# pr0g/ToyMeshPathTracer

Hardware: AMD Instinct MI355X
Metric: MRays/s on sponza.obj 1920x1080 64spp at 1/2/4/8 GPUs; %HBM roofline (higher is better)
Workload: dtype f32

## Files before the change

### include/tmpt.h

```cpp
#ifndef TMPT_H
#define TMPT_H

#include <stdint.h>

#ifdef __cplusplus
extern "C" {
#endif

#define TMPT_ABI_VERSION 9

typedef struct tmpt_scene tmpt_scene;

typedef struct {
    float origin[3], lower_left[3], horizontal[3], vertical[3], u[3], v[3], w[3];
    float lens_radius;
} tmpt_camera;

enum { TMPT_SEED_ROW = 0, TMPT_SEED_PIXEL = 1, TMPT_SEED_SAMPLE = 2 };

enum {
    TMPT_ENGINE_WAVEFRONT = 0,
    TMPT_ENGINE_MEGAKERNEL = 1,
    TMPT_ENGINE_PERSISTENT = 2
};

enum {
    TMPT_FLAG_OUT_DEVICE = 1,
    TMPT_FLAG_COUNT_VISITS = 2,
    TMPT_FLAG_WAIT_STREAM = 4,
    TMPT_FLAG_REQUIRE_RCCL = 8
};

typedef struct {
    int32_t width, height, spp;
    int32_t seed_mode;
    int32_t band_rows;
    int32_t shard, num_shards;
    int32_t engine;
    int32_t flags;
    int32_t spp_begin, spp_count;
    int32_t reserved0;
    uint64_t wait_stream;
    int32_t reserved[2];
} tmpt_render_desc;

typedef struct {
    double render_ms;
    double extend_ms, shadow_ms;
    uint64_t extend_rays, shadow_rays;
    int64_t extend_launches, shadow_launches, iterations;
    uint64_t node_visits, tri_tests;
    uint64_t shadow_node_visits, shadow_tri_tests;
    double build_ms;
    int32_t bvh_nodes, bvh_depth, n_tris, device;
    int32_t bvh4_nodes, bvh4_depth, leaf_max, builder_iters;
    int32_t octree_nodes, octree_leaves;
    int64_t octree_refs;
    double octree_build_ms;
    uint64_t tie_queries, root_misses;
    int32_t row_engine;
    int32_t stream_fallbacks;
    int32_t octree_depth;
    int32_t tie_rule;
    int64_t chain_pixels;
    int64_t redo_samples;
    int64_t redo_late;
    uint64_t crack_queries;
    int32_t octree_flat;
    int32_t redo_launches;
    double redo_ms;
    uint64_t redo_rays;
    int32_t tie_path;
    int32_t reserved_stats;
} tmpt_stats;

typedef struct {
    float    normal[3];
    float    depth;
    float    direct;
    int32_t  tri_id;
    uint32_t hits;
    uint32_t lit;
} tmpt_aov_pixel;

typedef struct {
    int32_t width, height, spp;
    int32_t levels;
    int32_t normal_exp;
    int32_t flags;
    float sigma_depth;
    float sigma_direct;
    uint64_t wait_stream;
    int32_t reserved[4];
} tmpt_denoise_desc;


int tmpt_load_obj(const char* path, float** out_tris, int32_t* out_n, float out_bmin[3],
                  float out_bmax[3]);
void tmpt_free(void* p);

int tmpt_camera_init(tmpt_camera* cam, const float look_from[3], const float look_at[3],
                     const float vup[3], float vfov, float aspect, float aperture,
                     float focus_dist);
int tmpt_camera_for_scene(tmpt_camera* cam, const float bmin[3], const float bmax[3],
                          int32_t width, int32_t height, int32_t is_sponza);


int tmpt_device_count(void);

int tmpt_scene_create(const float* tris, int32_t n, int32_t device, tmpt_scene** out);

int tmpt_scene_create_ex(const float* tris, int32_t n, int32_t device, const char* options, tmpt_scene** out);
int tmpt_scene_set_option(tmpt_scene* scene, const char* key, double value);
int tmpt_scene_get_option(const tmpt_scene* scene, const char* key, double* value);
int tmpt_scene_build_octree(tmpt_scene* scene, const float bmin[3], const float bmax[3]);
int tmpt_octree_bounds(const float bmin[3], const float bmax[3], float box[6]);
int tmpt_octree_digest(const float* tris, int32_t n, const float bmin[3], const float bmax[3], uint64_t out[5]);
int tmpt_octree_flags(const float* tris, int32_t n, const float bmin[3], const float bmax[3], const float* rays,
                      const float* t, const int32_t* ids, int64_t n_rays, uint8_t* flags, float grid[13]);
int tmpt_scene_destroy(tmpt_scene* scene);

int tmpt_scene_hit(const tmpt_scene* scene, const float* rays, int64_t n, float tmin, float tmax,
                   int32_t any_hit, float* hits, int32_t* ids);
int tmpt_scene_hit_ranged(const tmpt_scene* scene, const float* rays8, int64_t n, int32_t any_hit,
                          float* hits, int32_t* ids);

int tmpt_render(tmpt_scene* scene, const tmpt_camera* cam, const tmpt_render_desc* desc,
                uint8_t* rgba_out, uint64_t* ray_count);
int tmpt_render_aov(tmpt_scene* scene, const tmpt_camera* cam, const tmpt_render_desc* desc,
                    tmpt_aov_pixel* out, uint64_t* ray_count);
int tmpt_render_radiance(tmpt_scene* scene, const tmpt_camera* cam, const tmpt_render_desc* desc,
                         float* rgba32f_out, uint8_t* rgba8_out, uint64_t* ray_count);
int tmpt_denoise(tmpt_scene* scene, const tmpt_denoise_desc* desc, const float* rgba32f_in,
                 const tmpt_aov_pixel* aov, float* rgba32f_out, uint8_t* rgba8_out);
int tmpt_render_multi(const float* tris, int32_t n, const float* octree_box ,
                      const tmpt_camera* cam, const tmpt_render_desc* desc, const int32_t* devices,
                      int32_t ndevices, uint8_t* rgba_full, uint64_t* ray_count, double* seconds);

int32_t tmpt_tile_rows(const tmpt_render_desc* desc);
int32_t tmpt_tile_row_to_y(const tmpt_render_desc* desc, int32_t r);

int tmpt_get_stats(const tmpt_scene* scene, tmpt_stats* out);

int tmpt_write_png(const char* path, const uint8_t* rgba, int32_t width, int32_t height);

int tmpt_unit_sincos(int32_t device, uint32_t key0, uint32_t n, float* out);

int tmpt_fastdiv(uint32_t divisor, const uint32_t* x, uint64_t n, uint32_t* out, uint32_t mul_shift[2]);

int tmpt_scene_dump_bvh(const tmpt_scene* scene, int32_t layout, uint32_t* nodes, uint64_t node_words,
                        uint32_t* tris, uint64_t tri_words, int32_t info[8]);
int tmpt_radix_sort(const tmpt_scene* scene, uint32_t* keys, uint32_t* vals, int64_t n, int32_t bits);

const char* tmpt_last_error(void);
int tmpt_abi_version(void);

#ifdef __cplusplus
}
#endif
#endif
```

### toymeshpathtracer_amd/__init__.py

```python
from __future__ import annotations

import ctypes
import os
from dataclasses import dataclass
from typing import Optional, Tuple

import numpy as np

__all__ = [
    "Camera", "Scene", "Hit", "RenderStats", "load_scene", "write_png", "device_count",
    "SEED_ROW", "SEED_PIXEL", "SEED_SAMPLE", "ENGINE_WAVEFRONT", "ENGINE_MEGAKERNEL", "ENGINE_PERSISTENT", "lib_path", "TmptError",
    "tile_rows", "tile_row_to_y", "render_multi", "octree_bounds", "octree_digest", "octree_flags",
    "AOV_DTYPE",
]

SEED_ROW, SEED_PIXEL, SEED_SAMPLE = 0, 1, 2
ENGINE_WAVEFRONT, ENGINE_MEGAKERNEL, ENGINE_PERSISTENT = 0, 1, 2
FLAG_OUT_DEVICE, FLAG_COUNT_VISITS, FLAG_WAIT_STREAM, FLAG_REQUIRE_RCCL = 1, 2, 4, 8

AOV_DTYPE = np.dtype([("normal", np.float32, (3,)), ("depth", np.float32), ("direct", np.float32),
                      ("tri_id", np.int32), ("hits", np.uint32), ("lit", np.uint32)])

_HERE = os.path.dirname(os.path.abspath(__file__))
lib_path = os.environ.get("TMPT_LIB_PATH") or os.path.join(_HERE, "_lib", "libtmpt.so")


class TmptError(RuntimeError):
    pass


if not os.path.exists(lib_path):
    raise ImportError(
        f"libtmpt.so not built ({lib_path}); run `python -c 'import __graft_entry__ as g; g.build()'` "
        "or `make -C toymeshpathtracer_amd/csrc`. There is no CPU fallback.")

try:
    if os.environ.get("TMPT_NO_TORCH") == "1":
        raise ImportError("TMPT_NO_TORCH")
    import torch
except Exception:
    torch = None

_lib = ctypes.CDLL(lib_path)

_f32p = ctypes.POINTER(ctypes.c_float)
_i32p = ctypes.POINTER(ctypes.c_int32)
_u8p = ctypes.POINTER(ctypes.c_uint8)
_u64p = ctypes.POINTER(ctypes.c_uint64)


class _Camera(ctypes.Structure):
    _fields_ = [("origin", ctypes.c_float * 3), ("lower_left", ctypes.c_float * 3),
                ("horizontal", ctypes.c_float * 3), ("vertical", ctypes.c_float * 3),
                ("u", ctypes.c_float * 3), ("v", ctypes.c_float * 3), ("w", ctypes.c_float * 3),
                ("lens_radius", ctypes.c_float)]


class _Desc(ctypes.Structure):
    _fields_ = [("width", ctypes.c_int32), ("height", ctypes.c_int32), ("spp", ctypes.c_int32),
                ("seed_mode", ctypes.c_int32), ("band_rows", ctypes.c_int32),
                ("shard", ctypes.c_int32), ("num_shards", ctypes.c_int32),
                ("engine", ctypes.c_int32), ("flags", ctypes.c_int32),
                ("spp_begin", ctypes.c_int32), ("spp_count", ctypes.c_int32),
                ("reserved0", ctypes.c_int32), ("wait_stream", ctypes.c_uint64),
                ("reserved", ctypes.c_int32 * 2)]


class _DenoiseDesc(ctypes.Structure):
    _fields_ = [("width", ctypes.c_int32), ("height", ctypes.c_int32), ("spp", ctypes.c_int32),
                ("levels", ctypes.c_int32), ("normal_exp", ctypes.c_int32), ("flags", ctypes.c_int32),
                ("sigma_depth", ctypes.c_float), ("sigma_direct", ctypes.c_float),
                ("wait_stream", ctypes.c_uint64), ("reserved", ctypes.c_int32 * 4)]


class _Stats(ctypes.Structure):
    _fields_ = [("render_ms", ctypes.c_double), ("extend_ms", ctypes.c_double),
                ("shadow_ms", ctypes.c_double), ("extend_rays", ctypes.c_uint64),
                ("shadow_rays", ctypes.c_uint64), ("extend_launches", ctypes.c_int64),
                ("shadow_launches", ctypes.c_int64), ("iterations", ctypes.c_int64),
                ("node_visits", ctypes.c_uint64), ("tri_tests", ctypes.c_uint64),
                ("shadow_node_visits", ctypes.c_uint64), ("shadow_tri_tests", ctypes.c_uint64),
                ("build_ms", ctypes.c_double), ("bvh_nodes", ctypes.c_int32),
                ("bvh_depth", ctypes.c_int32), ("n_tris", ctypes.c_int32),
                ("device", ctypes.c_int32), ("bvh4_nodes", ctypes.c_int32),
                ("bvh4_depth", ctypes.c_int32), ("leaf_max", ctypes.c_int32),
                ("builder_iters", ctypes.c_int32), ("octree_nodes", ctypes.c_int32),
                ("octree_leaves", ctypes.c_int32), ("octree_refs", ctypes.c_int64),
                ("octree_build_ms", ctypes.c_double), ("tie_queries", ctypes.c_uint64),
                ("root_misses", ctypes.c_uint64), ("row_engine", ctypes.c_int32),
                ("stream_fallbacks", ctypes.c_int32), ("octree_depth", ctypes.c_int32),
                ("tie_rule", ctypes.c_int32), ("chain_pixels", ctypes.c_int64),
                ("redo_samples", ctypes.c_int64), ("redo_late", ctypes.c_int64),
                ("crack_queries", ctypes.c_uint64), ("octree_flat", ctypes.c_int32),
                ("redo_launches", ctypes.c_int32), ("redo_ms", ctypes.c_double),
                ("redo_rays", ctypes.c_uint64), ("tie_path", ctypes.c_int32), ("reserved_stats", ctypes.c_int32)]


def _sig(name, res, args):
    fn = getattr(_lib, name)
    fn.restype = res
    fn.argtypes = args
    return fn


_load_obj = _sig("tmpt_load_obj", ctypes.c_int, [ctypes.c_char_p, ctypes.POINTER(_f32p), _i32p, _f32p, _f32p])
_free = _sig("tmpt_free", None, [ctypes.c_void_p])
_cam_init = _sig("tmpt_camera_init", ctypes.c_int, [ctypes.POINTER(_Camera), _f32p, _f32p, _f32p,
                                                     ctypes.c_float, ctypes.c_float, ctypes.c_float,
                                                     ctypes.c_float])
_cam_scene = _sig("tmpt_camera_for_scene", ctypes.c_int, [ctypes.POINTER(_Camera), _f32p, _f32p,
                                                          ctypes.c_int32, ctypes.c_int32, ctypes.c_int32])
_dev_count = _sig("tmpt_device_count", ctypes.c_int, [])
_scene_create = _sig("tmpt_scene_create", ctypes.c_int, [_f32p, ctypes.c_int32, ctypes.c_int32,
                                                         ctypes.POINTER(ctypes.c_void_p)])
_scene_create_ex = _sig("tmpt_scene_create_ex", ctypes.c_int, [_f32p, ctypes.c_int32, ctypes.c_int32,
                                                               ctypes.c_char_p, ctypes.POINTER(ctypes.c_void_p)])
_set_option = _sig("tmpt_scene_set_option", ctypes.c_int, [ctypes.c_void_p, ctypes.c_char_p, ctypes.c_double])
_get_option = _sig("tmpt_scene_get_option", ctypes.c_int, [ctypes.c_void_p, ctypes.c_char_p,
                                                           ctypes.POINTER(ctypes.c_double)])
_scene_destroy = _sig("tmpt_scene_destroy", ctypes.c_int, [ctypes.c_void_p])
_scene_hit = _sig("tmpt_scene_hit", ctypes.c_int, [ctypes.c_void_p, _f32p, ctypes.c_int64,
                                                   ctypes.c_float, ctypes.c_float, ctypes.c_int32,
                                                   _f32p, _i32p])
_scene_hit_ranged = _sig("tmpt_scene_hit_ranged", ctypes.c_int, [ctypes.c_void_p, _f32p, ctypes.c_int64,
                                                                 ctypes.c_int32, _f32p, _i32p])
_render = _sig("tmpt_render", ctypes.c_int, [ctypes.c_void_p, ctypes.POINTER(_Camera),
                                             ctypes.POINTER(_Desc), ctypes.c_void_p, _u64p])
_render_aov = _sig("tmpt_render_aov", ctypes.c_int, [ctypes.c_void_p, ctypes.POINTER(_Camera),
                                                     ctypes.POINTER(_Desc), ctypes.c_void_p, _u64p])
_render_radiance = _sig("tmpt_render_radiance", ctypes.c_int, [ctypes.c_void_p, ctypes.POINTER(_Camera),
                                                               ctypes.POINTER(_Desc), ctypes.c_void_p,
                                                               ctypes.c_void_p, _u64p])
_denoise = _sig("tmpt_denoise", ctypes.c_int, [ctypes.c_void_p, ctypes.POINTER(_DenoiseDesc), ctypes.c_void_p,
                                               ctypes.c_void_p, ctypes.c_void_p, ctypes.c_void_p])
_build_octree = _sig("tmpt_scene_build_octree", ctypes.c_int, [ctypes.c_void_p, _f32p, _f32p])
_octree_bounds = _sig("tmpt_octree_bounds", ctypes.c_int, [_f32p, _f32p, _f32p])
_octree_digest = _sig("tmpt_octree_digest", ctypes.c_int, [_f32p, ctypes.c_int32, _f32p, _f32p, _u64p])
_octree_flags = _sig("tmpt_octree_flags", ctypes.c_int, [_f32p, ctypes.c_int32, _f32p, _f32p, _f32p, _f32p, _i32p,
                                                         ctypes.c_int64, ctypes.c_void_p, _f32p])
_render_multi = _sig("tmpt_render_multi", ctypes.c_int,
                     [_f32p, ctypes.c_int32, _f32p, ctypes.POINTER(_Camera), ctypes.POINTER(_Desc),
                      ctypes.POINTER(ctypes.c_int32), ctypes.c_int32, ctypes.c_void_p, _u64p,
                      ctypes.POINTER(ctypes.c_double)])
_tile_rows = _sig("tmpt_tile_rows", ctypes.c_int32, [ctypes.POINTER(_Desc)])
_tile_row_to_y = _sig("tmpt_tile_row_to_y", ctypes.c_int32, [ctypes.POINTER(_Desc), ctypes.c_int32])
_stats = _sig("tmpt_get_stats", ctypes.c_int, [ctypes.c_void_p, ctypes.POINTER(_Stats)])
_write_png = _sig("tmpt_write_png", ctypes.c_int, [ctypes.c_char_p, _u8p, ctypes.c_int32, ctypes.c_int32])
_last_error = _sig("tmpt_last_error", ctypes.c_char_p, [])
_abi = _sig("tmpt_abi_version", ctypes.c_int, [])
_unit_sincos = _sig("tmpt_unit_sincos", ctypes.c_int, [ctypes.c_int32, ctypes.c_uint32, ctypes.c_uint32,
                                                       ctypes.c_void_p])
EXPORTS = ("tmpt_load_obj", "tmpt_free", "tmpt_camera_init", "tmpt_camera_for_scene",
           "tmpt_device_count", "tmpt_scene_create", "tmpt_scene_create_ex", "tmpt_scene_set_option",
           "tmpt_scene_get_option", "tmpt_scene_destroy", "tmpt_scene_hit", "tmpt_scene_hit_ranged",
           "tmpt_render", "tmpt_render_multi", "tmpt_tile_rows", "tmpt_tile_row_to_y", "tmpt_get_stats",
           "tmpt_write_png", "tmpt_last_error", "tmpt_abi_version", "tmpt_unit_sincos",
           "tmpt_scene_build_octree", "tmpt_octree_bounds", "tmpt_octree_digest",
           "tmpt_octree_flags", "tmpt_render_aov", "tmpt_render_radiance", "tmpt_denoise", "tmpt_fastdiv",
           "tmpt_scene_dump_bvh", "tmpt_radix_sort")


def _check(rc: int, what: str) -> None:
    if rc != 0:
        raise TmptError(f"{what} failed ({rc}): {_last_error().decode(errors='replace')}")


def _fp(a: np.ndarray):
    return a.ctypes.data_as(_f32p)


def unit_sincos(key0: int, n: int, device: int = 0) -> np.ndarray:
    out = np.empty((n, 2), dtype=np.float32)
    _check(_unit_sincos(device, key0, n, out.ctypes.data), "tmpt_unit_sincos")
    return out


def fastdiv(divisor: int, x: np.ndarray):
    fn = _sig("tmpt_fastdiv", ctypes.c_int, [ctypes.c_uint32, ctypes.c_void_p, ctypes.c_uint64, ctypes.c_void_p,
                                             ctypes.c_void_p])
    x = np.ascontiguousarray(x, dtype=np.uint32)
    out = np.empty_like(x)
    ms = np.zeros(2, dtype=np.uint32)
    _check(fn(divisor, x.ctypes.data, x.size, out.ctypes.data, ms.ctypes.data), "tmpt_fastdiv")
    return out, (int(ms[0]), int(ms[1]))


def device_count() -> int:
    return int(_dev_count())


def abi_version() -> int:
    return int(_abi())


def load_scene(path: str) -> Tuple[np.ndarray, np.ndarray, np.ndarray]:
    p = _f32p()
    n = ctypes.c_int32()
    bmin = np.zeros(3, np.float32)
    bmax = np.zeros(3, np.float32)
    _check(_load_obj(path.encode(), ctypes.byref(p), ctypes.byref(n), _fp(bmin), _fp(bmax)),
           f"load_scene({path!r})")
    try:
        tris = np.ctypeslib.as_array(p, shape=(n.value * 9,)).copy().reshape(n.value, 3, 3)
    finally:
        _free(p)
    return tris, bmin, bmax


def octree_bounds(bmin, bmax) -> Tuple[np.ndarray, np.ndarray]:
    lo, hi = np.asarray(bmin, np.float32), np.asarray(bmax, np.float32)
    box = np.zeros(6, np.float32)
    _check(_octree_bounds(_fp(lo), _fp(hi), _fp(box)), "octree_bounds")
    return box[:3].copy(), box[3:].copy()


def octree_digest(tris: np.ndarray, box_min, box_max) -> dict:
    t = np.ascontiguousarray(np.asarray(tris, np.float32).reshape(-1, 9))
    lo, hi = np.asarray(box_min, np.float32), np.asarray(box_max, np.float32)
    out = (ctypes.c_uint64 * 5)()
    _check(_octree_digest(_fp(t), t.shape[0], _fp(lo), _fp(hi), out), "octree_digest")
    return dict(zip(("nodes", "leaves", "refs", "depth", "digest"), (int(v) for v in out)))


def octree_flags(tris: np.ndarray, box_min, box_max, rays, t, ids):
    tr = np.ascontiguousarray(np.asarray(tris, np.float32).reshape(-1, 9))
    lo, hi = np.asarray(box_min, np.float32), np.asarray(box_max, np.float32)
    r = np.ascontiguousarray(np.asarray(rays, np.float32)[:, :6])
    tt = np.ascontiguousarray(np.asarray(t, np.float32))
    ii = np.ascontiguousarray(np.asarray(ids, np.int32))
    out = np.zeros(r.shape[0], np.uint8)
    grid = np.zeros(13, np.float32)
    _check(_octree_flags(_fp(tr), tr.shape[0], _fp(lo), _fp(hi), _fp(r), _fp(tt), ii.ctypes.data_as(_i32p),
                         r.shape[0], out.ctypes.data, _fp(grid)), "octree_flags")
    return out, grid


@dataclass
class Camera:
    origin: np.ndarray
    lower_left: np.ndarray
    horizontal: np.ndarray
    vertical: np.ndarray
    u: np.ndarray
    v: np.ndarray
    w: np.ndarray
    lens_radius: float

    @staticmethod
    def _from_c(c: _Camera) -> "Camera":
        a = lambda f: np.array(list(f), np.float32)
        return Camera(a(c.origin), a(c.lower_left), a(c.horizontal), a(c.vertical), a(c.u),
                      a(c.v), a(c.w), float(c.lens_radius))

    def _to_c(self) -> _Camera:
        c = _Camera()
        for name in ("origin", "lower_left", "horizontal", "vertical", "u", "v", "w"):
            getattr(c, name)[:] = [float(x) for x in np.asarray(getattr(self, name), np.float32)]
        c.lens_radius = self.lens_radius
        return c

    @staticmethod
    def create(look_from, look_at, vup, vfov: float, aspect: float, aperture: float,
               focus_dist: float) -> "Camera":
        c = _Camera()
        lf, la, up = (np.asarray(x, np.float32) for x in (look_from, look_at, vup))
        _check(_cam_init(ctypes.byref(c), _fp(lf), _fp(la), _fp(up), vfov, aspect, aperture,
                         focus_dist), "Camera")
        return Camera._from_c(c)

    @staticmethod
    def for_scene(bmin, bmax, width: int, height: int, is_sponza: bool = False) -> "Camera":
        c = _Camera()
        lo, hi = np.asarray(bmin, np.float32), np.asarray(bmax, np.float32)
        _check(_cam_scene(ctypes.byref(c), _fp(lo), _fp(hi), width, height, int(is_sponza)),
               "Camera.for_scene")
        return Camera._from_c(c)

    def as_array(self) -> np.ndarray:
        return np.concatenate([self.origin, self.lower_left, self.horizontal, self.vertical,
                               self.u, self.v, self.w, [self.lens_radius]]).astype(np.float32)


@dataclass
class Hit:
    pos: np.ndarray
    normal: np.ndarray
    t: float


@dataclass
class RenderStats:
    render_ms: float
    extend_ms: float
    shadow_ms: float
    extend_rays: int
    shadow_rays: int
    extend_launches: int
    shadow_launches: int
    iterations: int
    node_visits: int
    tri_tests: int
    shadow_node_visits: int
    shadow_tri_tests: int
    build_ms: float
    bvh_nodes: int
    bvh_depth: int
    n_tris: int
    device: int
    bvh4_nodes: int
    bvh4_depth: int
    leaf_max: int
    builder_iters: int
# ... 96 lines not shown
    def __exit__(self, *exc):
        self.close()

    def hit_scene_batch(self, rays: np.ndarray, t_min: Optional[float] = None, t_max: Optional[float] = None,
                        any_hit: bool = False) -> Tuple[np.ndarray, np.ndarray]:
        rays = np.asarray(rays, np.float32)
        if (t_min is None) != (t_max is None):
            raise ValueError("hit_scene_batch: give both t_min and t_max, or neither (ranged rays [n,8])")
        ranged = t_min is None and t_max is None
        rays = np.ascontiguousarray(rays.reshape(-1, 8 if ranged else 6))
        n = rays.shape[0]
        hits = np.zeros((n, 7), np.float32)
        ids = np.full(n, -1, np.int32)
        if ranged:
            _check(_scene_hit_ranged(self._h, _fp(rays), n, int(any_hit), _fp(hits), ids.ctypes.data_as(_i32p)),
                   "hit_scene")
        else:
            _check(_scene_hit(self._h, _fp(rays), n, t_min, t_max, int(any_hit), _fp(hits),
                              ids.ctypes.data_as(_i32p)), "hit_scene")
        return ids, hits

    def hit_scene(self, orig, direction, t_min: float, t_max: float) -> Tuple[int, Optional[Hit]]:
        ids, hits = self.hit_scene_batch(np.concatenate([orig, direction])[None], t_min, t_max)
        if ids[0] < 0:
            return -1, None
        h = hits[0]
        return 1, Hit(h[0:3].copy(), h[3:6].copy(), float(h[6]))

    def trace_image(self, camera: Camera, width: int, height: int, spp: int,
                    seed_mode: int = SEED_ROW, engine: int = ENGINE_PERSISTENT, band_rows: int = 0,
                    shard: int = 0, num_shards: int = 1, count_visits: bool = False,
                    out=None, spp_begin: int = 0, spp_count: int = 0,
                    wait_stream="current") -> Tuple[np.ndarray, int]:
        if out is None:
            ws = None
        elif isinstance(wait_stream, str):
            ws = _current_stream(self.device)
        else:
            ws = wait_stream
        d = _desc(width, height, spp, seed_mode, band_rows, shard, num_shards, engine,
                  (FLAG_COUNT_VISITS if count_visits else 0) | (FLAG_OUT_DEVICE if out is not None else 0),
                  spp_begin, spp_count, ws)
        rows = int(_tile_rows(ctypes.byref(d)))
        rays = ctypes.c_uint64()
        cam = camera._to_c()
        if out is not None:
            _check(_render(self._h, ctypes.byref(cam), ctypes.byref(d), ctypes.c_void_p(int(out)),
                           ctypes.byref(rays)), "trace_image")
            return None, int(rays.value)
        img = np.zeros((rows, width, 4), np.uint8)
        _check(_render(self._h, ctypes.byref(cam), ctypes.byref(d), img.ctypes.data_as(ctypes.c_void_p),
                       ctypes.byref(rays)), "trace_image")
        return img, int(rays.value)

    def trace_progressive(self, camera: Camera, width: int, height: int, spp: int, passes,
                          band_rows: int = 0, shard: int = 0, num_shards: int = 1, seed_mode: int = SEED_PIXEL):
        if isinstance(passes, int):
            passes = [min(passes, spp - b) for b in range(0, spp, passes)]
        if sum(passes) != spp or min(passes) < 1:
            raise ValueError("passes must be positive and sum to spp")
        done = 0
        for n in passes:
            img, rays = self.trace_image(camera, width, height, spp, seed_mode=seed_mode,
                                         engine=ENGINE_PERSISTENT, band_rows=band_rows, shard=shard,
                                         num_shards=num_shards, spp_begin=done, spp_count=n)
            done += n
            yield done, img, rays

    def trace_aov(self, camera: Camera, width: int, height: int, spp: int, band_rows: int = 0,
                  shard: int = 0, num_shards: int = 1, out=None, wait_stream="current"):
        if out is None:
            ws = None
        elif isinstance(wait_stream, str):
            ws = _current_stream(self.device)
        else:
            ws = wait_stream
        d = _desc(width, height, spp, SEED_SAMPLE, band_rows, shard, num_shards, ENGINE_PERSISTENT,
                  FLAG_OUT_DEVICE if out is not None else 0, 0, 0, ws)
        rows = int(_tile_rows(ctypes.byref(d)))
        rays = ctypes.c_uint64()
        cam = camera._to_c()
        if out is not None:
            _check(_render_aov(self._h, ctypes.byref(cam), ctypes.byref(d), ctypes.c_void_p(int(out)),
                               ctypes.byref(rays)), "trace_aov")
            return None, int(rays.value)
        rec = np.zeros((rows, width), AOV_DTYPE)
        _check(_render_aov(self._h, ctypes.byref(cam), ctypes.byref(d), rec.ctypes.data_as(ctypes.c_void_p),
                           ctypes.byref(rays)), "trace_aov")
        return rec, int(rays.value)

    def trace_radiance(self, camera: Camera, width: int, height: int, spp: int, seed_mode: int = SEED_SAMPLE,
                       band_rows: int = 0, shard: int = 0, num_shards: int = 1, out=None, wait_stream="current"):
        if out is None:
            ws = None
        elif isinstance(wait_stream, str):
            ws = _current_stream(self.device)
        else:
            ws = wait_stream
        d = _desc(width, height, spp, seed_mode, band_rows, shard, num_shards, ENGINE_PERSISTENT,
                  FLAG_OUT_DEVICE if out is not None else 0, 0, 0, ws)
        rows = int(_tile_rows(ctypes.byref(d)))
        rays = ctypes.c_uint64()
        cam = camera._to_c()
        if out is not None:
            f32, u8 = out if isinstance(out, (tuple, list)) else (out, None)
            _check(_render_radiance(self._h, ctypes.byref(cam), ctypes.byref(d), ctypes.c_void_p(int(f32)),
                                    None if u8 is None else ctypes.c_void_p(int(u8)), ctypes.byref(rays)),
                   "trace_radiance")
            return None, None, int(rays.value)
        rad = np.zeros((rows, width, 4), np.float32)
        img = np.zeros((rows, width, 4), np.uint8)
        _check(_render_radiance(self._h, ctypes.byref(cam), ctypes.byref(d), rad.ctypes.data_as(ctypes.c_void_p),
                                img.ctypes.data_as(ctypes.c_void_p), ctypes.byref(rays)), "trace_radiance")
        return rad, img, int(rays.value)

    def denoise(self, radiance, aov, spp: int, levels: int = 0, normal_exp: int = -1, sigma_depth: float = 0.0,
                sigma_direct: float = 0.0, out=None, width: Optional[int] = None, height: Optional[int] = None,
                wait_stream="current"):
        dev = isinstance(radiance, int)
        d = _DenoiseDesc()
        if dev:
            if width is None or height is None or out is None:
                raise ValueError("denoise: device pointers need width, height and out")
            h, w = int(height), int(width)
        else:
            radiance = np.ascontiguousarray(radiance, np.float32)
            aov = np.ascontiguousarray(aov, AOV_DTYPE)
            h, w = radiance.shape[:2]
            if radiance.shape != (h, w, 4) or aov.shape != (h, w):
                raise ValueError("denoise: radiance [h, w, 4] and aov [h, w] of one whole frame")
        d.width, d.height, d.spp, d.levels, d.normal_exp = w, h, spp, levels, normal_exp
        d.sigma_depth, d.sigma_direct = sigma_depth, sigma_direct
        if dev:
            d.flags = FLAG_OUT_DEVICE
            ws = _current_stream(self.device) if isinstance(wait_stream, str) else wait_stream
            if ws is not None:
                d.flags |= FLAG_WAIT_STREAM
                d.wait_stream = int(ws)
            f32, u8 = out
            _check(_denoise(self._h, ctypes.byref(d), ctypes.c_void_p(radiance), ctypes.c_void_p(int(aov)),
                            None if f32 is None else ctypes.c_void_p(int(f32)),
                            None if u8 is None else ctypes.c_void_p(int(u8))), "denoise")
            return None, None
        res = np.zeros((h, w, 4), np.float32) if out is None else out
        if not (isinstance(res, np.ndarray) and res.dtype == np.float32 and res.shape == (h, w, 4)
                and res.flags.c_contiguous):
            raise ValueError("denoise: out must be a contiguous float32 array [h, w, 4] (it may be radiance itself)")
        img = np.zeros((h, w, 4), np.uint8)
        _check(_denoise(self._h, ctypes.byref(d), radiance.ctypes.data_as(ctypes.c_void_p),
                        aov.ctypes.data_as(ctypes.c_void_p), res.ctypes.data_as(ctypes.c_void_p),
                        img.ctypes.data_as(ctypes.c_void_p)), "denoise")
        return res, img

    def dump_bvh(self, layout: str = "aos") -> dict:
        if layout not in ("aos", "soa"):
            raise ValueError("dump_bvh: layout is 'aos' or 'soa'")
        fn = _sig("tmpt_scene_dump_bvh", ctypes.c_int, [ctypes.c_void_p, ctypes.c_int32, ctypes.c_void_p,
                                                        ctypes.c_uint64, ctypes.c_void_p, ctypes.c_uint64, _i32p])
        info = np.zeros(8, np.int32)
        lay = int(layout == "soa")
        _check(fn(self._h, lay, None, 0, None, 0, info.ctypes.data_as(_i32p)), "dump_bvh")
        nodes = np.zeros((int(info[1]), 16), np.uint32)
        tris = np.zeros((int(info[0]) + 1, 12), np.uint32)
        _check(fn(self._h, lay, nodes.ctypes.data, nodes.size, tris.ctypes.data, tris.size,
                  info.ctypes.data_as(_i32p)), "dump_bvh")
        keys = ("n", "n_nodes4", "depth4", "leaf_max", "count_shift", "link_bits", "builder_iters", "soa")
        return {"nodes": nodes, "tris": tris, "info": dict(zip(keys, (int(v) for v in info)))}

    def radix_sort(self, keys, vals, bits: int = 32):
        fn = _sig("tmpt_radix_sort", ctypes.c_int, [ctypes.c_void_p, ctypes.c_void_p, ctypes.c_void_p,
                                                    ctypes.c_int64, ctypes.c_int32])
        k = np.array(keys, dtype=np.uint32).reshape(-1)
        v = np.array(vals, dtype=np.uint32).reshape(-1)
        if k.shape != v.shape:
            raise ValueError("radix_sort: keys and vals of one length")
        _check(fn(self._h, k.ctypes.data, v.ctypes.data, k.size, bits), "radix_sort")
        return k, v

    def stats(self) -> RenderStats:
        s = _Stats()
        _check(_stats(self._h, ctypes.byref(s)), "stats")
        return RenderStats(*[getattr(s, f) for f, _ in _Stats._fields_ if not f.startswith("reserved")])


def render_multi(tris: np.ndarray, camera: "Camera", width: int, height: int, spp: int, devices,
                 seed_mode: int = SEED_PIXEL, engine: int = ENGINE_PERSISTENT,
                 require_rccl: bool = False, bounds=None) -> Tuple[np.ndarray, int, float]:
    t = np.ascontiguousarray(np.asarray(tris, np.float32).reshape(-1, 9))
    devs = (ctypes.c_int32 * len(devices))(*devices)
    img = np.zeros((height, width, 4), np.uint8)
    rays = ctypes.c_uint64()
    secs = ctypes.c_double()
    d = _desc(width, height, spp, seed_mode, 0, 0, 1, engine, FLAG_REQUIRE_RCCL if require_rccl else 0)
    cam = camera._to_c()
    box = None if bounds is None else np.concatenate(octree_bounds(*bounds)).astype(np.float32)
    _check(_render_multi(t.ctypes.data_as(_f32p), t.shape[0], None if box is None else _fp(box),
                         ctypes.byref(cam), ctypes.byref(d), devs,
                         len(devices), img.ctypes.data_as(ctypes.c_void_p), ctypes.byref(rays),
                         ctypes.byref(secs)), "render_multi")
    return img, int(rays.value), float(secs.value)


def write_png(path: str, rgba: np.ndarray) -> None:
    rgba = np.ascontiguousarray(rgba, np.uint8)
    h, w = rgba.shape[:2]
    _check(_write_png(path.encode(), rgba.ctypes.data_as(_u8p), w, h), "write_png")
```

### toymeshpathtracer_amd/csrc/tmpt_api.cpp

```cpp
#include <dlfcn.h>
#include <hip/hip_runtime.h>
#include <rccl/rccl.h>
#include <string.h>

#include <algorithm>
#include <new>
#include <chrono>
#include <string>
#include <thread>
#include <vector>

#include "tmpt.h"
#include "tmpt_internal.h"
#include "tmpt_traverse.h"
#include "tmpt_render.h"

namespace tmpt {

static thread_local std::string g_last_error;
void set_error(const std::string& msg) { g_last_error = msg; }
const char* last_error() { return g_last_error.c_str(); }

int load_obj(const char* path, std::vector<float>& tris, f3& bmin, f3& bmax);
void camera_init(tmpt_camera* cam, f3 lookFrom, f3 lookAt, f3 vup, float vfov, float aspect,
                 float aperture, float focusDist);
void camera_for_scene(tmpt_camera* cam, f3 sceneMin, f3 sceneMax, int w, int h, bool sponza);
int write_png(const char* path, const uint8_t* rgba, int w, int h);
int render(Scene& s, const tmpt_camera* cam, const tmpt_render_desc* d, uint32_t* d_out,
           uint64_t* ray_count, float4* d_sums = nullptr);
int intersect_batch(Scene& s, const float* d_rays, int64_t n, float tmin, float tmax, bool any, bool ranged,
                    float* d_hits, int32_t* d_ids);

__global__ void k_unit_sincos(uint32_t key0, uint32_t n, float2* out)
{
    const uint32_t i = blockIdx.x * blockDim.x + threadIdx.x;
    if (i >= n) return;
    float c, s;
    glibc_sincosf_unit(unit_angle((key0 + i) & 0xFFFFFFu), c, s);
    out[i] = make_float2(c, s);
}

__global__ void k_assemble_rows(const uint32_t* __restrict__ gathered, int32_t nd, int32_t max_rows, int32_t W,
                                int32_t H, uint32_t* __restrict__ frame)
{
    const int64_t i = (int64_t)blockIdx.x * 256 + threadIdx.x;
    if (i >= (int64_t)W * H) return;
    const int32_t y = (int32_t)(i / W), x = (int32_t)(i - (int64_t)y * W);
    frame[i] = gathered[((int64_t)(y % nd) * max_rows + y / nd) * W + x];
}

struct Rccl {
    ncclResult_t (*comm_init_all)(ncclComm_t*, int, const int*) = nullptr;
    ncclResult_t (*comm_destroy)(ncclComm_t) = nullptr;
    ncclResult_t (*gather)(const void*, void*, size_t, ncclDataType_t, int, ncclComm_t, hipStream_t) = nullptr;
    ncclResult_t (*reduce)(const void*, void*, size_t, ncclDataType_t, ncclRedOp_t, int, ncclComm_t,
                           hipStream_t) = nullptr;
    ncclResult_t (*group_start)() = nullptr;
    ncclResult_t (*group_end)() = nullptr;
    const char* (*error_string)(ncclResult_t) = nullptr;
    bool ok = false;
};

const Rccl& rccl()
{
    static Rccl r = []() {
        Rccl x;
        void* h = dlopen("librccl.so.1", RTLD_NOW | RTLD_GLOBAL);
        if (!h) h = dlopen("/opt/rocm/lib/librccl.so.1", RTLD_NOW | RTLD_GLOBAL);
        if (!h) return x;
        x.comm_init_all = (decltype(x.comm_init_all))dlsym(h, "ncclCommInitAll");
        x.comm_destroy = (decltype(x.comm_destroy))dlsym(h, "ncclCommDestroy");
        x.gather = (decltype(x.gather))dlsym(h, "ncclGather");
        x.reduce = (decltype(x.reduce))dlsym(h, "ncclReduce");
        x.group_start = (decltype(x.group_start))dlsym(h, "ncclGroupStart");
        x.group_end = (decltype(x.group_end))dlsym(h, "ncclGroupEnd");
        x.error_string = (decltype(x.error_string))dlsym(h, "ncclGetErrorString");
        x.ok = x.comm_init_all && x.comm_destroy && x.gather && x.reduce && x.group_start && x.group_end &&
               x.error_string;
        return x;
    }();
    return r;
}

namespace {
struct OptionDef {
    const char* name;
    bool build;
    double lo, hi;
    int Options::*i;
    float Options::*f;
    double Options::*d;
};
const OptionDef kOptions[] = {
    {"builder", true, 0, 1, &Options::builder, nullptr, nullptr},
    {"layout", true, 0, 1, &Options::layout, nullptr, nullptr},
    {"leaf_max", true, 1, kLeafMaxTris, &Options::leaf_max, nullptr, nullptr},
    {"collapse", true, 0, 1, &Options::collapse, nullptr, nullptr},
    {"ploc_radius", true, 1, 256, &Options::ploc_radius, nullptr, nullptr},
    {"sah_c_leaf", true, 0, 1e6, nullptr, &Options::sah_c_leaf, nullptr},
    {"sah_c_tri", true, 0, 1e6, nullptr, &Options::sah_c_tri, nullptr},
    {"sample_block", false, 0, 1024, &Options::sample_block, nullptr, nullptr},
    {"sample_tail", false, -1, 64, &Options::sample_tail, nullptr, nullptr},
    {"sbuf_max", false, 0, 1e18, nullptr, nullptr, &Options::sbuf_max},
    {"sbuf_pair", false, 0, 1, &Options::sbuf_pair, nullptr, nullptr},
    {"pilot", false, -1, 512, &Options::pilot, nullptr, nullptr},
    {"help", false, -1, 1, &Options::help, nullptr, nullptr},
    {"pair", false, -1, 63, &Options::pair, nullptr, nullptr},
    {"balance", false, 0, 1, &Options::balance, nullptr, nullptr},
    {"dprio", false, 0, 1, &Options::dprio, nullptr, nullptr},
    {"wave_cap", false, 0, 64, &Options::wave_cap, nullptr, nullptr},
    {"pixel_chains", false, -1, 1024, &Options::pixel_chains, nullptr, nullptr},
    {"tie_defer", false, -1, 1, &Options::tie_defer, nullptr, nullptr},
    {"redo_cap", false, 0, 1 << 30, &Options::redo_cap, nullptr, nullptr},
    {"redo_inline", false, 0, 1, &Options::redo_inline, nullptr, nullptr},
    {"redo_lanes", false, 1, 64, &Options::redo_lanes, nullptr, nullptr},
    {"path_waves", false, 0, 5, &Options::path_waves, nullptr, nullptr},
    {"top_walk", false, -1, 8, &Options::top_walk, nullptr, nullptr},
    {"shadow_order", false, -1, 2, &Options::shadow_order, nullptr, nullptr},
    {"pop_cull", false, -1, 1, &Options::pop_cull, nullptr, nullptr},
    {"pop_key_cap", false, -1, kPopKeyMax, &Options::pop_key_cap, nullptr, nullptr},
    {"rowspec", false, 0, 1, &Options::rowspec, nullptr, nullptr},
    {"rowspec_wmax", false, 0, 16384, &Options::rowspec_wmax, nullptr, nullptr},
    {"rowspec_windows", false, 0, 32, &Options::rowspec_windows, nullptr, nullptr},
    {"rowspec_spread", false, -1, 100, nullptr, &Options::rowspec_spread, nullptr},
    {"rowspec_groups", false, 1, kRowSpecMaxGroups, &Options::rowspec_groups, nullptr, nullptr},
    {"rowspec_noshadow", false, 0, 1, &Options::rowspec_noshadow, nullptr, nullptr},
    {"rowspec_chase", false, 0, 1, &Options::rowspec_chase, nullptr, nullptr},
    {"rowspec_stream", false, 0, 1, &Options::rowspec_stream, nullptr, nullptr},
    {"rowstream_dynamic", false, 0, 1, &Options::rowstream_dynamic, nullptr, nullptr},
    {"row_flag_leaves", false, 0, 1, &Options::row_flag_leaves, nullptr, nullptr},
    {"row_occ", false, 0, 5, &Options::row_occ, nullptr, nullptr},
    {"wf_bins", false, 1, 8, &Options::wf_bins, nullptr, nullptr},
    {"rowstream_test_abort", false, 0, 1, &Options::rowstream_test_abort, nullptr, nullptr},
    {"tie_rule", false, 0, 1, &Options::tie_rule, nullptr, nullptr},
    {"aov_group", false, 0, 16, &Options::aov_group, nullptr, nullptr},
    {"denoise_lds", false, -1, 1, &Options::denoise_lds, nullptr, nullptr},
};

const OptionDef* find_option(const char* key)
{
    for (const OptionDef& d : kOptions)
        if (strcmp(d.name, key) == 0) return &d;
    return nullptr;
}
}

int options_set(Options& o, const char* key, double v, bool allow_build)
{
    const OptionDef* d = key ? find_option(key) : nullptr;
    if (!d) {
        set_error(std::string("unknown option '") + (key ? key : "(null)") + "'");
        return -22;
    }
    if (d->build && !allow_build) {
        set_error(std::string("option '") + key + "' is a build option: give it to tmpt_scene_create_ex");
        return -22;
    }
    if (!(v >= d->lo && v <= d->hi)) {
        set_error(std::string("option '") + key + "' out of range [" + std::to_string(d->lo) + ", " +
                  std::to_string(d->hi) + "]");
        return -22;
    }
    if (d->i) {
        if (v != (double)(long long)v) {
            set_error(std::string("option '") + key + "' takes an integer");
            return -22;
        }
        if ((strcmp(key, "row_occ") == 0 || strcmp(key, "path_waves") == 0) && v != 0 && v != 4 && v != 5) {
            set_error(std::string("option '") + key + "' takes 0 (auto), 4 or 5");
            return -22;
        }
        if (strcmp(key, "aov_group") == 0 && v > 0 && ((long long)v & ((long long)v - 1)) != 0) {
            set_error(std::string("option '") + key + "' out of range: 0 (auto), 1, 2, 4, 8 or 16");
            return -22;
        }
        if ((strcmp(key, "sample_block") == 0 || strcmp(key, "wf_bins") == 0) && v > 0 &&
            ((long long)v & ((long long)v - 1)) != 0) {
            set_error(std::string("option '") + key + "' must be a power of two");
            return -22;
        }
        o.*(d->i) = (int)v;
    } else if (d->f) {
        o.*(d->f) = (float)v;
    } else {
        o.*(d->d) = v;
    }
    return 0;
}

int options_get(const Options& o, const char* key, double* v)
{
    const OptionDef* d = key ? find_option(key) : nullptr;
    if (!d) {
        set_error(std::string("unknown option '") + (key ? key : "(null)") + "'");
        return -22;
    }
    *v = d->i ? (double)(o.*(d->i)) : d->f ? (double)(o.*(d->f)) : o.*(d->d);
    return 0;
}

int options_parse(Options& o, const char* text, bool allow_build)
{
    if (!text) return 0;
    std::string t(text);
    size_t pos = 0;
    while (pos <= t.size()) {
        size_t end = t.find(',', pos);
        if (end == std::string::npos) end = t.size();
        std::string item = t.substr(pos, end - pos);
        pos = end + 1;
        item.erase(0, item.find_first_not_of(" \t"));
        item.erase(item.find_last_not_of(" \t") + 1);
        if (item.empty()) continue;
        const size_t eq = item.find('=');
        if (eq == std::string::npos) {
            set_error("option '" + item + "' has no value (key=value)");
            return -22;
        }
        std::string key = item.substr(0, eq), val = item.substr(eq + 1);
        key.erase(key.find_last_not_of(" \t") + 1);
        val.erase(0, val.find_first_not_of(" \t"));
        if (key == "builder" && (val == "ploc" || val == "lbvh")) val = val == "lbvh" ? "1" : "0";
        if (key == "collapse" && (val == "greedy" || val == "sah")) val = val == "sah" ? "1" : "0";
        if (key == "tie_rule" && (val == "visit" || val == "index")) val = val == "index" ? "1" : "0";
        if (key == "layout" && (val == "aos" || val == "soa")) val = val == "soa" ? "1" : "0";
        char* endp = nullptr;
        const double v = strtod(val.c_str(), &endp);
        if (val.empty() || !endp || *endp != '\0') {
            set_error("option '" + key + "': bad value '" + val + "'");
            return -22;
        }
        if (int rc = options_set(o, key.c_str(), v, allow_build)) return rc;
    }
    return 0;
}

}

struct tmpt_scene {
    tmpt::Scene s;
};

using namespace tmpt;

#define TMPT_GUARD_BEGIN try {
#define TMPT_GUARD_END                                  \
    }                                                   \
    catch (const std::bad_alloc&) {                     \
        set_error("out of host memory");                \
        return -1;                                      \
    }                                                   \
    catch (...) {                                       \
        set_error("unexpected C++ exception");          \
        return -1;                                      \
    }

namespace {
// ... 17 lines not shown
    if (n == 0) return 0;
    if (device < 0) {
        for (uint32_t i = 0; i < n; ++i)
            glibc_sincosf_unit(unit_angle((key0 + i) & 0xFFFFFFu), out[2 * (size_t)i], out[2 * (size_t)i + 1]);
        return 0;
    }
    int ndev = 0;
    TMPT_HIP(hipGetDeviceCount(&ndev));
    if (device >= ndev) return bad("tmpt_unit_sincos: no such device");
    TMPT_HIP(hipSetDevice(device));
    float2* d = nullptr;
    TMPT_HIP(hipMalloc(&d, sizeof(float2) * (size_t)n));
    k_unit_sincos<<<(n + 255u) / 256u, 256>>>(key0, n, d);
    hipError_t e = hipGetLastError();
    if (e == hipSuccess) e = hipMemcpy(out, d, sizeof(float2) * (size_t)n, hipMemcpyDeviceToHost);
    (void)hipFree(d);
    if (e != hipSuccess) {
        set_error(std::string("tmpt_unit_sincos: ") + hipGetErrorString(e));
        return -1;
    }
    return 0;
    TMPT_GUARD_END
}

int tmpt_fastdiv(uint32_t divisor, const uint32_t* x, uint64_t n, uint32_t* out, uint32_t mul_shift[2])
{
    TMPT_GUARD_BEGIN
    if (divisor == 0u || divisor >= (1u << 31)) return bad("tmpt_fastdiv: divisor out of range (1 .. 2^31 - 1)");
    if ((!x || !out) && n) return bad("tmpt_fastdiv: null argument");
    const FastDiv f = fastdiv_make(divisor);
    if (mul_shift) {
        mul_shift[0] = f.mul;
        mul_shift[1] = f.shift;
    }
    for (uint64_t i = 0; i < n; ++i) {
        if (x[i] >= (1u << 31)) return bad("tmpt_fastdiv: dividend out of range (below 2^31)");
        out[i] = fastdiv(x[i], f);
    }
    return 0;
    TMPT_GUARD_END
}

int tmpt_load_obj(const char* path, float** out_tris, int32_t* out_n, float out_bmin[3],
                  float out_bmax[3])
{
    TMPT_GUARD_BEGIN
    if (!path || !out_tris || !out_n) return bad("tmpt_load_obj: null argument");
    std::vector<float> tris;
    f3 bmin, bmax;
    int rc = load_obj(path, tris, bmin, bmax);
    if (rc) return rc;
    float* p = (float*)malloc(tris.size() * sizeof(float));
    if (!p) return bad("tmpt_load_obj: out of memory");
    memcpy(p, tris.data(), tris.size() * sizeof(float));
    *out_tris = p;
    *out_n = (int32_t)(tris.size() / 9);
    if (out_bmin) { out_bmin[0] = bmin.x; out_bmin[1] = bmin.y; out_bmin[2] = bmin.z; }
    if (out_bmax) { out_bmax[0] = bmax.x; out_bmax[1] = bmax.y; out_bmax[2] = bmax.z; }
    return 0;
    TMPT_GUARD_END
}

int tmpt_camera_init(tmpt_camera* cam, const float lf[3], const float la[3], const float up[3],
                     float vfov, float aspect, float aperture, float focus_dist)
{
    if (!cam || !lf || !la || !up) return bad("tmpt_camera_init: null argument");
    camera_init(cam, mk(lf[0], lf[1], lf[2]), mk(la[0], la[1], la[2]), mk(up[0], up[1], up[2]),
                vfov, aspect, aperture, focus_dist);
    return 0;
}

int tmpt_camera_for_scene(tmpt_camera* cam, const float bmin[3], const float bmax[3],
                          int32_t width, int32_t height, int32_t is_sponza)
{
    if (!cam || !bmin || !bmax) return bad("tmpt_camera_for_scene: null argument");
    if (width < 1 || height < 1) return bad("tmpt_camera_for_scene: bad size");
    camera_for_scene(cam, mk(bmin[0], bmin[1], bmin[2]), mk(bmax[0], bmax[1], bmax[2]), width,
                     height, is_sponza != 0);
    return 0;
}

int tmpt_device_count(void)
{
    int n = 0;
    if (hipGetDeviceCount(&n) != hipSuccess) return 0;
    return n;
}

int tmpt_scene_create(const float* tris, int32_t n, int32_t device, tmpt_scene** out)
{
    return tmpt_scene_create_ex(tris, n, device, nullptr, out);
}

int tmpt_scene_create_ex(const float* tris, int32_t n, int32_t device, const char* options, tmpt_scene** out)
{
    TMPT_GUARD_BEGIN
    if (!out || n < 0 || (n > 0 && !tris)) return bad("tmpt_scene_create: bad arguments");
    *out = nullptr;
    (void)hipGetLastError();
    Options opt;
    if (int rc = options_parse(opt, options, true)) {
        set_error(std::string("tmpt_scene_create: ") + last_error());
        return rc;
    }
    int ndev = 0;
    TMPT_HIP(hipGetDeviceCount(&ndev));
    if (device < 0 || device >= ndev) return bad("tmpt_scene_create: no such device");
    TMPT_HIP(hipSetDevice(device));
    tmpt_scene* h = new tmpt_scene();
    Scene& s = h->s;
    s.opt = opt;
    s.device = device;
    s.n = n;
    auto fail = [&](int rc) {
        tmpt_scene_destroy(h);
        return rc;
    };
    if (hipStreamCreateWithFlags(&s.stream, hipStreamNonBlocking) != hipSuccess)
        return fail((set_error("hipStreamCreate failed"), -1));
    float* d_tris = nullptr;
    if (n > 0) {
        if (hipMalloc(&d_tris, sizeof(float) * 9 * (size_t)n) != hipSuccess)
            return fail((set_error("tmpt_scene_create: out of device memory"), -1));
        if (hipMemcpy(d_tris, tris, sizeof(float) * 9 * (size_t)n, hipMemcpyHostToDevice) != hipSuccess) {
            (void)hipFree(d_tris);
            return fail((set_error("tmpt_scene_create: upload failed"), -1));
        }
    }
    s.tris_host.assign(tris, tris + 9 * (size_t)n);
    int rc = build_lbvh(s, d_tris);
    if (d_tris) (void)hipFree(d_tris);
    if (rc) return fail(rc);
    *out = h;
    return 0;
    TMPT_GUARD_END
}

int tmpt_scene_destroy(tmpt_scene* h)
{
    if (!h) return 0;
    Scene& s = h->s;
    (void)hipSetDevice(s.device);
    if (s.stream) (void)hipStreamSynchronize(s.stream);
    for (auto& st : s.rs_stream)
        if (st) (void)hipStreamSynchronize(st);
    if (s.nodes4) (void)hipFree(s.nodes4);
    if (s.oct) (void)hipFree(s.oct);
    if (s.oct_refs) (void)hipFree(s.oct_refs);
    if (s.oct_view) (void)hipFree(s.oct_view);
    if (s.soa_buf) (void)hipFree(s.soa_buf);
    if (s.prog) (void)hipFree(s.prog);
    if (s.jt) (void)hipFree(s.jt);
    if (s.sbuf) (void)hipFree(s.sbuf);
    if (s.redo) (void)hipFree(s.redo);
    if (s.redo_state) (void)hipFree(s.redo_state);
    if (s.jt2) (void)hipFree(s.jt2);
    if (s.rs_buf) (void)hipFree(s.rs_buf);
    for (auto& st : s.rs_stream)
        if (st) (void)hipStreamDestroy(st);
    for (auto& ev : s.rs_event)
        if (ev) (void)hipEventDestroy(ev);
    if (s.rs_host) (void)hipHostFree(s.rs_host);
    if (s.rs_list) (void)hipFree(s.rs_list);
    if (s.rss_buf) (void)hipFree(s.rss_buf);
    if (s.rss_tab) (void)hipFree(s.rss_tab);
    if (s.rss_host) (void)hipHostFree(s.rss_host);
    if (s.wait_ev) (void)hipEventDestroy(s.wait_ev);
    if (s.counters) (void)hipFree(s.counters);
    if (s.chk) (void)hipFree(s.chk);
    if (s.counters_host) (void)hipHostFree(s.counters_host);
    for (auto e : s.render_ev)
        if (e) (void)hipEventDestroy(e);
    if (s.tri_pre) (void)hipFree(s.tri_pre);
    if (s.tri_orig) (void)hipFree(s.tri_orig);
    if (s.ws) (void)hipFree(s.ws);
    for (auto e : s.path_ev)
        if (e) (void)hipEventDestroy(e);
    if (s.stream) (void)hipStreamDestroy(s.stream);
    delete h;
    return 0;
}

int tmpt_scene_build_octree(tmpt_scene* h, const float bmin[3], const float bmax[3])
{
    TMPT_GUARD_BEGIN
    if (!h || !bmin || !bmax) return bad("tmpt_scene_build_octree: null argument");
    Scene& s = h->s;
    if ((int64_t)s.tris_host.size() != 9 * (int64_t)s.n) return bad("tmpt_scene_build_octree: no triangle copy");
    TMPT_HIP(hipSetDevice(s.device));
    const auto t0 = std::chrono::steady_clock::now();
    OctreeHost t;
    build_octree(s.tris_host.data(), s.n, bmin, bmax, t);
    if (t.refs.size() >= (size_t)INT32_MAX || t.nodes.size() >= (size_t)INT32_MAX)
        return bad("tmpt_scene_build_octree: octree too large");
    OctNode* d_nodes = nullptr;
    int32_t* d_refs = nullptr;
    const size_t nb = t.nodes.size() * sizeof(OctNode), rb = std::max<size_t>(1, t.refs.size()) * sizeof(int32_t);
    if (hipMalloc(&d_nodes, nb) != hipSuccess || hipMalloc(&d_refs, rb) != hipSuccess ||
        hipMemcpy(d_nodes, t.nodes.data(), nb, hipMemcpyHostToDevice) != hipSuccess ||
        (t.refs.size() && hipMemcpy(d_refs, t.refs.data(), t.refs.size() * sizeof(int32_t), hipMemcpyHostToDevice) !=
                              hipSuccess)) {
        if (d_nodes) (void)hipFree(d_nodes);
        if (d_refs) (void)hipFree(d_refs);
        return (set_error("tmpt_scene_build_octree: out of device memory"), -1);
    }
    if (ensure_counters(s)) {
        (void)hipFree(d_nodes);
        (void)hipFree(d_refs);
        return -1;
    }
    if (s.stream) (void)hipStreamSynchronize(s.stream);
    if (!s.oct_view && hipMalloc(&s.oct_view, sizeof(OctView)) != hipSuccess) {
        (void)hipFree(d_nodes);
        (void)hipFree(d_refs);
        return (set_error("tmpt_scene_build_octree: out of device memory"), -1);
    }
    OctGrid grid;
    octree_grid(t, bmin, bmax, grid);
    std::vector<uint8_t> flat;
    const int32_t n_flat = octree_flat_triangles(s.tris_host.data(), s.n, grid, flat);
    if (mark_flat_triangles(s, flat)) {
        (void)hipFree(d_nodes);
        (void)hipFree(d_refs);
        return -1;
    }
    const OctView ov{d_nodes, d_refs, (int32_t)t.nodes.size(), n_flat, s.ties, grid, (int64_t)t.refs.size()};
    if (hipMemcpy(s.oct_view, &ov, sizeof(ov), hipMemcpyHostToDevice) != hipSuccess) {
        (void)hipFree(d_nodes);
        (void)hipFree(d_refs);
        std::vector<uint8_t> old_flat((size_t)s.n, 0);
        if (s.oct) (void)octree_flat_triangles(s.tris_host.data(), s.n, s.oct_grid, old_flat);
        (void)mark_flat_triangles(s, old_flat);
        return (set_error("tmpt_scene_build_octree: upload failed"), -1);
    }
    if (s.oct) (void)hipFree(s.oct);
    if (s.oct_refs) (void)hipFree(s.oct_refs);
    s.oct = d_nodes;
    s.oct_refs = d_refs;
    s.n_oct = (int32_t)t.nodes.size();
    s.n_oct_refs = (int64_t)t.refs.size();
    s.oct_leaves = t.leaves;
    s.oct_depth = t.depth;
    s.oct_flat = n_flat;
    s.oct_grid = grid;
    for (int c = 0; c < 3; ++c) {
        s.oct_lo[c] = bmin[c];
        s.oct_hi[c] = bmax[c];
    }
    s.oct_build_ms = std::chrono::duration<double, std::milli>(std::chrono::steady_clock::now() - t0).count();
    return 0;
    TMPT_GUARD_END
}

int tmpt_octree_bounds(const float bmin[3], const float bmax[3], float box[6])
{
    if (!bmin || !bmax || !box) return bad("tmpt_octree_bounds: null argument");
    const f3 lo = mk(bmin[0], bmin[1], bmin[2]), hi = mk(bmax[0], bmax[1], bmax[2]);
    const f3 extra = (hi - lo) * 0.7f;
    const f3 a = lo - extra, b = hi + extra;
    box[0] = a.x, box[1] = a.y, box[2] = a.z, box[3] = b.x, box[4] = b.y, box[5] = b.z;
    return 0;
}

int tmpt_octree_digest(const float* tris, int32_t n, const float bmin[3], const float bmax[3], uint64_t out[5])
{
    TMPT_GUARD_BEGIN
    if (n < 0 || (n > 0 && !tris) || !bmin || !bmax || !out) return bad("tmpt_octree_digest: bad arguments");
    OctreeHost t;
    build_octree(tris, n, bmin, bmax, t);
    out[0] = t.nodes.size();
    out[1] = (uint64_t)t.leaves;
    out[2] = t.refs.size() - (uint64_t)t.leaves;
    out[3] = (uint64_t)t.depth;
    out[4] = octree_digest(t);
    return 0;
    TMPT_GUARD_END
}

int tmpt_octree_flags(const float* tris, int32_t n, const float bmin[3], const float bmax[3], const float* rays,
                      const float* t, const int32_t* ids, int64_t n_rays, uint8_t* flags, float grid[13])
{
    TMPT_GUARD_BEGIN
    if (n < 0 || (n > 0 && !tris) || !bmin || !bmax || n_rays < 0 || (n_rays > 0 && (!rays || !t || !ids || !flags)))
        return bad("tmpt_octree_flags: bad arguments");
    OctreeHost oh;
    build_octree(tris, n, bmin, bmax, oh);
    OctGrid g;
    octree_grid(oh, bmin, bmax, g);
    std::vector<uint8_t> flat;
    octree_flat_triangles(tris, n, g, flat);
    for (int64_t i = 0; i < n_rays; ++i) {
        const float* r = rays + 6 * i;
        const int32_t id = ids[i];
        uint8_t f = 0;
        if (id >= 0 && id < n)
            f = (uint8_t)(flat[(size_t)id] | (octree_crack(g, mk(r[0], r[1], r[2]), mk(r[3], r[4], r[5]), t[i]) ? 2 : 0));
        flags[i] = f;
    }
    if (grid) {
        for (int k = 0; k < 3; ++k) {
            grid[k] = g.r0[k];
            grid[3 + k] = g.inv_cell[k];
            grid[6 + k] = g.cell[k];
            grid[9 + k] = g.band[k];
        }
        grid[12] = g.reach;
    }
    return 0;
    TMPT_GUARD_END
}

int tmpt_scene_set_option(tmpt_scene* h, const char* key, double value)
{
    TMPT_GUARD_BEGIN
    if (!h) return bad("tmpt_scene_set_option: null scene");
    return options_set(h->s.opt, key, value, false);
    TMPT_GUARD_END
}

int tmpt_scene_get_option(const tmpt_scene* h, const char* key, double* value)
{
    TMPT_GUARD_BEGIN
    if (!h || !value) return bad("tmpt_scene_get_option: null argument");
    if (key && strcmp(key, "pop_key_bits") == 0) {
        *value = (double)pop_key_bits(h->s.link_bits, h->s.opt.pop_key_cap);
        return 0;
    }
    return options_get(h->s.opt, key, value);
    TMPT_GUARD_END
}

namespace {
int scene_hit(const tmpt_scene* hc, const float* rays, int64_t n, float tmin, float tmax, bool ranged,
              int32_t any_hit, float* hits, int32_t* ids)
{
    if (!hc || n < 0 || (n > 0 && (!rays || !hits || !ids))) return bad("tmpt_scene_hit: bad arguments");
    if (n == 0) return 0;
    const size_t rs = ranged ? 32 : 24;
    Scene& s = const_cast<tmpt_scene*>(hc)->s;
    TMPT_HIP(hipSetDevice(s.device));
    float *d_rays = nullptr, *d_hits = nullptr;
    int32_t* d_ids = nullptr;
    auto cleanup = [&]() {
        if (d_rays) (void)hipFree(d_rays);
        if (d_hits) (void)hipFree(d_hits);
        if (d_ids) (void)hipFree(d_ids);
    };
    if (hipMalloc(&d_rays, rs * (size_t)n) != hipSuccess || hipMalloc(&d_hits, 28 * (size_t)n) != hipSuccess ||
        hipMalloc(&d_ids, 4 * (size_t)n) != hipSuccess) {
        cleanup();
        return bad("tmpt_scene_hit: out of device memory");
    }
    int rc = 0;
    if (hipMemcpy(d_rays, rays, rs * (size_t)n, hipMemcpyHostToDevice) != hipSuccess ||
        hipMemcpy(d_hits, hits, 28 * (size_t)n, hipMemcpyHostToDevice) != hipSuccess)
        rc = (set_error("tmpt_scene_hit: upload failed"), -1);
    if (!rc) rc = intersect_batch(s, d_rays, n, tmin, tmax, any_hit != 0, ranged, d_hits, d_ids);
    if (!rc && (hipStreamSynchronize(s.stream) != hipSuccess ||
                hipMemcpy(hits, d_hits, 28 * (size_t)n, hipMemcpyDeviceToHost) != hipSuccess ||
                hipMemcpy(ids, d_ids, 4 * (size_t)n, hipMemcpyDeviceToHost) != hipSuccess))
        rc = (set_error("tmpt_scene_hit: kernel or readback failed"), -1);
    if (!rc) {
        s.tie_queries = s.counters_host[kTieCounter];
        s.root_misses = s.counters_host[kTieCounter + 1];
        s.crack_queries = s.counters_host[kCrackCounter];
    }
    if (!rc) rc = check_report(s, "tmpt_scene_hit");
    cleanup();
    return rc;
}
}

int tmpt_scene_hit(const tmpt_scene* hc, const float* rays, int64_t n, float tmin, float tmax,
                   int32_t any_hit, float* hits, int32_t* ids)
{
    TMPT_GUARD_BEGIN
    return scene_hit(hc, rays, n, tmin, tmax, false, any_hit, hits, ids);
    TMPT_GUARD_END
}

int tmpt_scene_hit_ranged(const tmpt_scene* hc, const float* rays8, int64_t n, int32_t any_hit, float* hits,
                          int32_t* ids)
{
    TMPT_GUARD_BEGIN
    return scene_hit(hc, rays8, n, 0.0f, 0.0f, true, any_hit, hits, ids);
    TMPT_GUARD_END
}

int32_t tmpt_tile_rows(const tmpt_render_desc* d)
{
    if (!d || d->height < 1) return 0;
    int band = d->band_rows > 0 ? d->band_rows : d->height;
    int ns = d->num_shards > 1 ? d->num_shards : 1;
    int sh = ns > 1 ? d->shard : 0;
    int nbands = (d->height + band - 1) / band;
    int rows = 0;
    for (int b = sh; b < nbands; b += ns) rows += std::min(band, d->height - b * band);
    return rows;
}

int32_t tmpt_tile_row_to_y(const tmpt_render_desc* d, int32_t r)
{
    int band = d->band_rows > 0 ? d->band_rows : d->height;
    int ns = d->num_shards > 1 ? d->num_shards : 1;
    int sh = ns > 1 ? d->shard : 0;
    int lb = r / band;
    return (lb * ns + sh) * band + (r - lb * band);
}

int tmpt_render(tmpt_scene* h, const tmpt_camera* cam, const tmpt_render_desc* d,
                uint8_t* rgba_out, uint64_t* ray_count)
{
    TMPT_GUARD_BEGIN
    if (!h || !cam || !d || !rgba_out) return bad("tmpt_render: null argument");
    if (d->width < 1 || d->width > 10000) return bad("tmpt_render: invalid width");
    if (d->height < 1 || d->height > 10000) return bad("tmpt_render: invalid height");
    if (d->spp < 1 || d->spp > 1024) return bad("tmpt_render: invalid samplesPerPixel");
    if (d->seed_mode != TMPT_SEED_ROW && d->seed_mode != TMPT_SEED_PIXEL && d->seed_mode != TMPT_SEED_SAMPLE)
        return bad("tmpt_render: invalid seed_mode");
    if (d->engine != TMPT_ENGINE_WAVEFRONT && d->engine != TMPT_ENGINE_MEGAKERNEL &&
        d->engine != TMPT_ENGINE_PERSISTENT)
        return bad("tmpt_render: invalid engine");
    if (d->num_shards > 1 && (d->shard < 0 || d->shard >= d->num_shards))
        return bad("tmpt_render: invalid shard");
    if (d->spp_begin < 0 || d->spp_begin >= d->spp || d->spp_count < 0 ||
        d->spp_count > d->spp - d->spp_begin)
        return bad("tmpt_render: invalid spp_begin / spp_count");
    const bool progressive = d->spp_begin > 0 || (d->spp_count > 0 && d->spp_count < d->spp);
    if (progressive && (d->engine != TMPT_ENGINE_PERSISTENT || d->seed_mode == TMPT_SEED_ROW))
        return bad("tmpt_render: progressive spp needs the persistent engine and pixel or sample seeding");
    (void)hipGetLastError();
    Scene& s = h->s;
    TMPT_HIP(hipSetDevice(s.device));
    const int32_t rows = tmpt_tile_rows(d);
    const size_t bytes = (size_t)rows * (size_t)d->width * 4;
    const bool dev_out = (d->flags & TMPT_FLAG_OUT_DEVICE) != 0;
    uint32_t* d_out = nullptr;
    if (dev_out) d_out = (uint32_t*)rgba_out;
    else if (bytes && hipMalloc(&d_out, bytes) != hipSuccess) return bad("tmpt_render: out of device memory");
    int rc = render(s, cam, d, d_out, ray_count);
    if (!rc) rc = check_report(s, "tmpt_render");
    if (!rc && !dev_out && bytes) {
        if (hipMemcpy(rgba_out, d_out, bytes, hipMemcpyDeviceToHost) != hipSuccess)
            rc = (set_error("tmpt_render: readback failed"), -1);
    }
    if (!dev_out && d_out) (void)hipFree(d_out);
    return rc;
    TMPT_GUARD_END
}

int tmpt_render_aov(tmpt_scene* h, const tmpt_camera* cam, const tmpt_render_desc* d, tmpt_aov_pixel* out,
                    uint64_t* ray_count)
{
    TMPT_GUARD_BEGIN
    if (!h || !cam || !d || !out) return bad("tmpt_render_aov: null argument");
    if (d->width < 1 || d->width > 10000) return bad("tmpt_render_aov: invalid width");
    if (d->height < 1 || d->height > 10000) return bad("tmpt_render_aov: invalid height");
    if (d->spp < 1 || d->spp > 1024) return bad("tmpt_render_aov: invalid samplesPerPixel");
    if (d->seed_mode != TMPT_SEED_SAMPLE)
        return bad("tmpt_render_aov: seed_mode must be TMPT_SEED_SAMPLE (the only seeding where a camera ray is a "
                   "function of pixel and sample)");
    if (d->spp_begin != 0 || d->spp_count != 0)
        return bad("tmpt_render_aov: spp_begin / spp_count must be 0 (the pass is not progressive)");
    if (d->flags & TMPT_FLAG_COUNT_VISITS) return bad("tmpt_render_aov: TMPT_FLAG_COUNT_VISITS is not supported");
    if (d->num_shards > 1 && (d->shard < 0 || d->shard >= d->num_shards))
        return bad("tmpt_render_aov: invalid shard");
    const bool dev_out = (d->flags & TMPT_FLAG_OUT_DEVICE) != 0;
    if (dev_out && (reinterpret_cast<uintptr_t>(out) & 15u) != 0)
        return bad("tmpt_render_aov: a device output must be 16-byte aligned");
    (void)hipGetLastError();
    Scene& s = h->s;
    TMPT_HIP(hipSetDevice(s.device));
    const size_t bytes = (size_t)tmpt_tile_rows(d) * (size_t)d->width * sizeof(tmpt_aov_pixel);
    tmpt_aov_pixel* d_out = nullptr;
    if (dev_out) d_out = out;
    else if (bytes && hipMalloc(&d_out, bytes) != hipSuccess) return bad("tmpt_render_aov: out of device memory");
    int rc = render_aov(s, cam, d, d_out, ray_count);
    if (!rc) rc = check_report(s, "tmpt_render_aov");
    if (!rc && !dev_out && bytes) {
        if (hipMemcpy(out, d_out, bytes, hipMemcpyDeviceToHost) != hipSuccess)
            rc = (set_error("tmpt_render_aov: readback failed"), -1);
    }
    if (!dev_out && d_out) (void)hipFree(d_out);
    return rc;
    TMPT_GUARD_END
}

int tmpt_render_radiance(tmpt_scene* h, const tmpt_camera* cam, const tmpt_render_desc* d, float* rgba32f_out,
                         uint8_t* rgba8_out, uint64_t* ray_count)
{
    TMPT_GUARD_BEGIN
    if (!h || !cam || !d || !rgba32f_out) return bad("tmpt_render_radiance: null argument");
    if (d->width < 1 || d->width > 10000) return bad("tmpt_render_radiance: invalid width");
    if (d->height < 1 || d->height > 10000) return bad("tmpt_render_radiance: invalid height");
    if (d->spp < 1 || d->spp > 1024) return bad("tmpt_render_radiance: invalid samplesPerPixel");
    if (d->seed_mode != TMPT_SEED_PIXEL && d->seed_mode != TMPT_SEED_SAMPLE)
        return bad("tmpt_render_radiance: seed_mode must be TMPT_SEED_PIXEL or TMPT_SEED_SAMPLE (row seeding keeps no "
                   "float sum per pixel)");
    if (d->engine != TMPT_ENGINE_PERSISTENT)
        return bad("tmpt_render_radiance: engine must be TMPT_ENGINE_PERSISTENT");
    if (d->spp_begin != 0 || d->spp_count != 0)
        return bad("tmpt_render_radiance: spp_begin / spp_count must be 0 (whole renders only)");
    if (d->flags & TMPT_FLAG_COUNT_VISITS)
        return bad("tmpt_render_radiance: TMPT_FLAG_COUNT_VISITS is not supported");
    if (d->num_shards > 1 && (d->shard < 0 || d->shard >= d->num_shards))
        return bad("tmpt_render_radiance: invalid shard");
    const bool dev_out = (d->flags & TMPT_FLAG_OUT_DEVICE) != 0;
    if (dev_out && (reinterpret_cast<uintptr_t>(rgba32f_out) & 15u) != 0)
        return bad("tmpt_render_radiance: a device rgba32f_out must be 16-byte aligned");
    (void)hipGetLastError();
    Scene& s = h->s;
    TMPT_HIP(hipSetDevice(s.device));
    const size_t px = (size_t)tmpt_tile_rows(d) * (size_t)d->width;
    float4* d_f = dev_out ? reinterpret_cast<float4*>(rgba32f_out) : nullptr;
    uint32_t* d_8 = dev_out ? reinterpret_cast<uint32_t*>(rgba8_out) : nullptr;
    void *own_f = nullptr, *own_8 = nullptr;
    auto cleanup = [&]() {
        if (own_f) (void)hipFree(own_f);
        if (own_8) (void)hipFree(own_8);
    };
    if (px && ((!d_f && hipMalloc(&own_f, px * sizeof(float4)) != hipSuccess) ||
               (!d_8 && hipMalloc(&own_8, px * 4) != hipSuccess))) {
        cleanup();
        return bad("tmpt_render_radiance: out of device memory");
    }
    if (own_f) d_f = static_cast<float4*>(own_f);
    if (own_8) d_8 = static_cast<uint32_t*>(own_8);
    int rc = render(s, cam, d, d_8, ray_count, d_f);
    if (!rc) rc = check_report(s, "tmpt_render_radiance");
    if (!rc && !dev_out && px) {
        if (hipMemcpy(rgba32f_out, d_f, px * sizeof(float4), hipMemcpyDeviceToHost) != hipSuccess ||
            (rgba8_out && hipMemcpy(rgba8_out, d_8, px * 4, hipMemcpyDeviceToHost) != hipSuccess))
            rc = (set_error("tmpt_render_radiance: readback failed"), -1);
    }
    cleanup();
    return rc;
    TMPT_GUARD_END
}

int tmpt_denoise(tmpt_scene* h, const tmpt_denoise_desc* d, const float* rgba32f_in, const tmpt_aov_pixel* aov,
                 float* rgba32f_out, uint8_t* rgba8_out)
{
    TMPT_GUARD_BEGIN
    if (!d) return bad("tmpt_denoise: null descriptor");
    if (d->width < 1 || d->width > 10000) return bad("tmpt_denoise: invalid width");
    if (d->height < 1 || d->height > 10000) return bad("tmpt_denoise: invalid height");
    if (d->spp < 1 || d->spp > 1024) return bad("tmpt_denoise: invalid samplesPerPixel");
    if (d->levels < 0 || d->levels > 6) return bad("tmpt_denoise: levels out of range (1..6, 0 = 5)");
    if (d->normal_exp < -1 || d->normal_exp > 8) return bad("tmpt_denoise: normal_exp out of range (0..8, -1 = 5)");
    if (!(d->sigma_depth >= 0.0f) || !(d->sigma_depth <= 3.0e38f))
        return bad("tmpt_denoise: sigma_depth must be finite and not negative (0 = auto)");
    if (!(d->sigma_direct >= 0.0f) || !(d->sigma_direct <= 3.0e38f))
        return bad("tmpt_denoise: sigma_direct must be finite and not negative (0 = default)");
    if (d->flags & ~(TMPT_FLAG_OUT_DEVICE | TMPT_FLAG_WAIT_STREAM)) return bad("tmpt_denoise: unknown flag");
    if (!rgba32f_out && !rgba8_out) return bad("tmpt_denoise: no output (rgba32f_out and rgba8_out are both null)");
    if (!h || !rgba32f_in || !aov) return bad("tmpt_denoise: null argument");
    const bool dev = (d->flags & TMPT_FLAG_OUT_DEVICE) != 0;
    if (dev && (((reinterpret_cast<uintptr_t>(rgba32f_in) | reinterpret_cast<uintptr_t>(aov) |
                  reinterpret_cast<uintptr_t>(rgba32f_out)) & 15u) != 0 ||
                (reinterpret_cast<uintptr_t>(rgba8_out) & 3u) != 0))
        return bad("tmpt_denoise: device pointers must be 16-byte aligned (rgba8_out: 4)");
    tmpt_denoise_desc r = *d;
    if (r.levels == 0) r.levels = 5;
    if (r.normal_exp < 0) r.normal_exp = 5;
    if (r.sigma_depth == 0.0f) r.sigma_depth = 1.0f / (float)r.height;
    if (r.sigma_direct == 0.0f) r.sigma_direct = 0.05f;
    (void)hipGetLastError();
    Scene& s = h->s;
    TMPT_HIP(hipSetDevice(s.device));
    const size_t n = (size_t)r.width * (size_t)r.height;
    const float4* d_in = reinterpret_cast<const float4*>(rgba32f_in);
    const tmpt_aov_pixel* d_aov = aov;
    float4* d_o32 = reinterpret_cast<float4*>(rgba32f_out);
    uint32_t* d_o8 = reinterpret_cast<uint32_t*>(rgba8_out);
    void *own_in = nullptr, *own_aov = nullptr, *own_8 = nullptr;
    auto cleanup = [&]() {
        if (own_in) (void)hipFree(own_in);
        if (own_aov) (void)hipFree(own_aov);
        if (own_8) (void)hipFree(own_8);
    };
    if (!dev) {
        if (hipMalloc(&own_in, n * sizeof(float4)) != hipSuccess ||
            hipMalloc(&own_aov, n * sizeof(tmpt_aov_pixel)) != hipSuccess ||
            (rgba8_out && hipMalloc(&own_8, n * 4) != hipSuccess)) {
            cleanup();
            return bad("tmpt_denoise: out of device memory");
        }
        if (hipMemcpy(own_in, rgba32f_in, n * sizeof(float4), hipMemcpyHostToDevice) != hipSuccess ||
            hipMemcpy(own_aov, aov, n * sizeof(tmpt_aov_pixel), hipMemcpyHostToDevice) != hipSuccess) {
            cleanup();
            return (set_error("tmpt_denoise: upload failed"), -1);
        }
        d_in = static_cast<const float4*>(own_in);
        d_aov = static_cast<const tmpt_aov_pixel*>(own_aov);
        d_o32 = rgba32f_out ? static_cast<float4*>(own_in) : nullptr;
        d_o8 = static_cast<uint32_t*>(own_8);
    }
    int rc = denoise(s, &r, d_in, d_aov, d_o32, d_o8);
    if (!rc && !dev) {
        if ((rgba32f_out && hipMemcpy(rgba32f_out, d_o32, n * sizeof(float4), hipMemcpyDeviceToHost) != hipSuccess) ||
            (rgba8_out && hipMemcpy(rgba8_out, d_o8, n * 4, hipMemcpyDeviceToHost) != hipSuccess))
            rc = (set_error("tmpt_denoise: readback failed"), -1);
    }
    cleanup();
    return rc;
    TMPT_GUARD_END
}

int tmpt_render_multi(const float* tris, int32_t n, const float* octree_box, const tmpt_camera* cam,
                      const tmpt_render_desc* desc, const int32_t* devices, int32_t ndevices, uint8_t* rgba_full,
                      uint64_t* ray_count, double* seconds)
{
    TMPT_GUARD_BEGIN
    if (!cam || !desc || !devices || ndevices < 1 || !rgba_full || (n > 0 && !tris))
        return bad("tmpt_render_multi: bad arguments");
    if (desc->width < 1 || desc->width > 10000 || desc->height < 1 || desc->height > 10000)
        return bad("tmpt_render_multi: invalid width / height");
    const int nd = ndevices;
    const int W = desc->width, H = desc->height;
    bool unique = true;
    for (int g = 0; g < nd; ++g)
        for (int k = 0; k < g; ++k) unique = unique && devices[g] != devices[k];
    const bool use_rccl = unique && rccl().ok;
    if ((desc->flags & TMPT_FLAG_REQUIRE_RCCL) && !use_rccl)
        return bad(unique ? "tmpt_render_multi: RCCL (librccl.so.1) not available"
                          : "tmpt_render_multi: RCCL needs distinct devices (a device is listed twice)");
    std::vector<tmpt_scene*> scenes((size_t)nd, nullptr);
    std::vector<int> rcs((size_t)nd, 0);
    std::vector<std::string> errs((size_t)nd);
    const int max_rows = (H + nd - 1) / nd;
    const size_t tile_bytes = (size_t)max_rows * (size_t)W * 4;
    std::vector<uint8_t*> d_tile((size_t)nd, nullptr);
    std::vector<uint64_t*> d_rays((size_t)nd, nullptr);
    std::vector<hipStream_t> streams((size_t)nd, nullptr);
    uint8_t* d_gather = nullptr;
    uint32_t* d_frame = nullptr;
    uint64_t* d_total = nullptr;
// ... 223 lines not shown
```

### toymeshpathtracer_amd/csrc/tmpt_internal.h

```cpp
#pragma once

#include <hip/hip_runtime.h>
#include <stdint.h>

#include <string>
#include <vector>

#include "tmpt_math.h"

namespace tmpt {

struct alignas(16) Bvh4Node {
    float4 a;
    uint4 b;
    uint4 c;
    int4 d;
};
static_assert(sizeof(Bvh4Node) == 64, "BVH4Q node is one half cache line");

constexpr int kLeafMaxTris = 16;

constexpr int kPopKeyMin = 9;
constexpr int kPopKeyMax = 16;
TMPT_HD constexpr int bits_for(uint32_t v)
// ... 24 lines not shown
{
    return 0x80000000u | ((count - 1u) << count_shift) | first;
}
TMPT_HD constexpr uint32_t leaf_first(uint32_t link, int count_shift) { return link & ((1u << count_shift) - 1u); }
TMPT_HD constexpr uint32_t leaf_count(uint32_t link, int count_shift)
{
    return ((link >> count_shift) & (uint32_t)(kLeafMaxTris - 1)) + 1u;
}
TMPT_HD constexpr uint32_t entry_pack(uint32_t link, uint32_t key_f32, uint32_t key_mask)
{
    return (key_f32 & key_mask) | link;
}
TMPT_HD constexpr uint32_t entry_key(uint32_t e, uint32_t key_mask) { return e & key_mask; }
TMPT_HD constexpr uint32_t entry_link(uint32_t e, uint32_t key_mask) { return e ^ (e & key_mask); }

namespace link_checks {
constexpr LinkLayout kBench = link_layout(66453u, 2, 16700u);
static_assert(kBench.count_shift == 17 && kBench.link_bits == 18, "bench scene: 18-bit links");
static_assert(pop_key_bits(kBench.link_bits, -1) == 13 && pop_key_mask(13) == 0x7FFC0000u, "bench scene: bits 30..18");
static_assert(pop_key_bits(kBench.link_bits, 9) == 9 && pop_key_mask(9) == 0x7FC00000u, "capped key");
static_assert(pop_key_bits(kBench.link_bits, 0) == 0 && pop_key_bits(kBench.link_bits, 8) == 0 &&
                  pop_key_mask(0) == 0u, "no key below 9 bits");
static_assert(link_layout(66453u, 16, 9000u).link_bits == 21 && pop_key_bits(21, -1) == 10, "leaf_max 16");
static_assert(link_layout(1u << 21, 2, 1u << 20).link_bits == 23 && pop_key_bits(23, -1) == 0, "2^21 triangles");
static_assert(link_layout(1u << 21, 1, 1u << 21).link_bits == 22 && pop_key_bits(22, -1) == 9, "2^21, leaf_max 1");
static_assert(pop_key_bits(link_layout(12u, 2, 5u).link_bits, -1) == 16 && pop_key_mask(16) == 0x7FFF8000u, "cap 16");
static_assert(link_layout(3u, 1, 1000u).link_bits == 10, "node index decides");
static_assert(link_layout((1u << 27) - 1u, 16, 1u << 26).link_bits == 31, "2^27 - 1 triangles still fit");
constexpr uint32_t kLeaf = leaf_link(2u, 66452u, kBench.count_shift), kMask = pop_key_mask(13);
constexpr uint32_t kTn = 0x4129999Au;
static_assert(leaf_first(kLeaf, kBench.count_shift) == 66452u && leaf_count(kLeaf, kBench.count_shift) == 2u,
              "leaf decode");
static_assert(entry_link(entry_pack(kLeaf, kTn, kMask), kMask) == kLeaf, "leaf link survives its key");
static_assert(entry_link(entry_pack(16699u, kTn, kMask), kMask) == 16699u, "node link survives its key");
static_assert(entry_key(entry_pack(kLeaf, kTn, kMask), kMask) == 0x41280000u, "key = tn truncated (10.5 <= 10.6)");
static_assert(entry_key(entry_pack(kLeaf, 0x7F800000u, kMask), kMask) == 0x7F800000u, "+inf stays +inf");
static_assert(entry_pack(kLeaf, kTn, 0u) == kLeaf && entry_key(kLeaf, 0u) == 0u, "no key field: plain links");
}

struct FastDiv {
    uint32_t mul, shift;
};
inline FastDiv fastdiv_make(uint32_t d)
{
    const uint32_t l = (uint32_t)bits_for(d > 1u ? d - 1u : 0u);
    const uint64_t p = 1ull << (31u + l);
    return FastDiv{(uint32_t)((p + d - 1u) / d), l};
}
TMPT_HD uint32_t fastdiv(uint32_t x, FastDiv f)
{
#if defined(__HIP_DEVICE_COMPILE__)
    return __umulhi(x << 1, f.mul) >> f.shift;
#else
    return (uint32_t)(((uint64_t)(x << 1) * f.mul) >> 32) >> f.shift;
#endif
}

constexpr int kTopNodes = 120;
constexpr int kTopNodes5 = 80;

struct alignas(16) TriPre {
    float4 a;
    float4 b;
    float4 c;
};
struct alignas(16) TriOrig {
    float4 a;
    float4 b;
    float4 c;
};

struct alignas(16) OctNode {
    float4 lo;
    float4 hi;
};
static_assert(sizeof(OctNode) == 32, "octree node: two dwordx4 loads");

struct OctGrid {
    float reach;
    float drift[3];
    float r0[3];
    float inv_cell[3];
    float cell[3];
    float band[3];
};

struct OctView {
    const OctNode* nodes;
    const int32_t* refs;
    int32_t n;
    int32_t flat;
    unsigned long long* ties;
    OctGrid grid;
    int64_t n_refs;
};

constexpr uint32_t kChkNode = 1u, kChkLeaf = 2u, kChkStack = 4u, kChkOctSkip = 8u, kChkOctRef = 16u,
                   kChkTri = 32u;
constexpr int kCheckError = -30;

struct OctreeHost {
    std::vector<OctNode> nodes;
    std::vector<int32_t> refs;
    int32_t leaves = 0, depth = 0;
};

void build_octree(const float* tris9, int32_t n, const float bmin[3], const float bmax[3], OctreeHost& out);
uint64_t octree_digest(const OctreeHost& t);
void octree_grid(const OctreeHost& t, const float bmin[3], const float bmax[3], OctGrid& g);
int32_t octree_flat_triangles(const float* tris9, int32_t n, const OctGrid& g, std::vector<uint8_t>& flat);

struct SoaScene {
    const uint4* __restrict__ na = nullptr;
    const uint4* __restrict__ nb = nullptr;
    const uint2* __restrict__ nc = nullptr;
    const int4* __restrict__ nd = nullptr;
    const float4* __restrict__ ta = nullptr;
    const float4* __restrict__ tb = nullptr;
    const float2* __restrict__ tc = nullptr;
};

constexpr float kBoxPadRel = 1e-5f;
constexpr float kTfarSlack = 1.00001f;

constexpr int kStackTotal = 128;

constexpr int kShadowOrderDefault = 2;
constexpr int kPopCullSample = 1, kPopCullPixel = 1, kPopCullRow = 1;

constexpr int kRowSpecMaxGroups = 8;
constexpr int kRenderCounters = 48;
constexpr int kWalkCounter = 42;
constexpr int kCamCounter = 44;
constexpr int kTopCounter = 32;
constexpr int kTieCounter = 24;
constexpr int kCrackCounter = 30;
constexpr int kRedoRaysCounter = 31;
constexpr int kRedoCounter = 26;

struct Options {
    int builder = 0;
    int layout = 0;
    int leaf_max = 2;
    int collapse = 0;
    int ploc_radius = 32;
    float sah_c_leaf = 0.7f, sah_c_tri = 0.5f;
    int sample_block = 0;
    int rowstream_dynamic = 1;
    int row_flag_leaves = 1;
    int row_occ = 0;
    int sample_tail = -1;
    double sbuf_max = 0.0;
    int sbuf_pair = 1;
    int pilot = -1;
    int help = -1;
    int pair = -1;
    int balance = 1;
    int dprio = 1;
    int wave_cap = 0;
    int pixel_chains = -1;
    int rowspec = 1;
    int rowspec_wmax = 0;
    int rowspec_windows = 0;
    float rowspec_spread = -1.0f;
    int rowspec_groups = 2;
    int rowspec_noshadow = 1;
    int rowspec_chase = 1;
    int rowspec_stream = 1;
    int rowstream_test_abort = 0;
    int wf_bins = 1;
    int tie_rule = 0;
    int tie_defer = -1;
    int redo_cap = 0;
    int redo_lanes = 4;
    int path_waves = 0;
    int redo_inline = 1;
    int top_walk = -1;
    int shadow_order = -1;
    int pop_cull = -1;
    int pop_key_cap = -1;
    int aov_group = 0;
    int denoise_lds = -1;
};
int options_parse(Options& o, const char* text, bool allow_build);
int options_set(Options& o, const char* key, double value, bool allow_build);
int options_get(const Options& o, const char* key, double* value);

struct Scene {
    int device = 0;
    int32_t n = 0;
    int32_t n_nodes = 0;
    int32_t max_depth = 0;
    Bvh4Node* nodes4 = nullptr;
    int32_t n_nodes4 = 0, depth4 = 0, leaf_max = 0, ploc_iters = 0;
    int32_t count_shift = 0, link_bits = 31;
    TriPre* tri_pre = nullptr;
    TriOrig* tri_orig = nullptr;
    void* soa_buf = nullptr;
    SoaScene soa;
    std::vector<float> tris_host;
    OctNode* oct = nullptr;
    int32_t* oct_refs = nullptr;
    OctView* oct_view = nullptr;
    int32_t n_oct = 0, oct_leaves = 0, oct_depth = 0;
    int32_t oct_flat = 0;
    OctGrid oct_grid{};
    int64_t n_oct_refs = 0;
    double oct_build_ms = 0.0;
    float oct_lo[3] = {0, 0, 0}, oct_hi[3] = {0, 0, 0};
    unsigned long long* ties = nullptr;
    uint64_t tie_queries = 0, root_misses = 0, crack_queries = 0;
    int32_t row_engine = 0, stream_fallbacks = 0;
    int64_t chain_pixels = 0;
    Options opt;
    hipEvent_t wait_ev = nullptr;
    unsigned long long* counters = nullptr;
    unsigned long long* counters_host = nullptr;
    uint32_t* chk = nullptr;
    hipEvent_t render_ev[2] = {nullptr, nullptr};
    hipStream_t stream = nullptr;
    double build_ms = 0.0;
    void* ws = nullptr;
    size_t ws_bytes = 0;
    float4* prog = nullptr;
    size_t prog_slots = 0;
    int32_t prog_key[7] = {0, 0, 0, 0, 0, 0, -1};
    uint64_t prog_cam = 0;
    uint32_t* jt = nullptr;
    int32_t jt_spp = 0;
    float4* sbuf = nullptr;
    size_t sbuf_bytes = 0;
    uint2* redo = nullptr;
    uint32_t redo_cap = 0;
    float4* redo_state = nullptr;
    int64_t redo_samples = 0;
    int64_t redo_late = 0;
    int32_t redo_launches = 0;
    int32_t tie_path = 0;
    bool row_render = false;
    bool pixel_render = false;
    double redo_ms = 0.0;
    uint64_t redo_rays = 0;
    uint32_t* jt2 = nullptr;
    int32_t jt2_n = 0;
    void* rs_buf = nullptr;
    size_t rs_bytes = 0;
    hipStream_t rs_stream[kRowSpecMaxGroups] = {};
    hipEvent_t rs_event[kRowSpecMaxGroups + 1] = {};
    uint32_t* rs_host = nullptr;
    void* rs_list = nullptr;
    size_t rs_list_bytes = 0;
    void* rss_buf = nullptr;
    size_t rss_bytes = 0;
    uint32_t* rss_tab = nullptr;
    uint32_t* rss_host = nullptr;
    int path_launches = 1;
    hipEvent_t path_ev[4] = {nullptr, nullptr, nullptr, nullptr};
    double render_ms = 0.0;
    double extend_ms = 0.0;
    double shadow_ms = 0.0;
    uint64_t extend_rays = 0, shadow_rays = 0;
    int64_t extend_launches = 0, shadow_launches = 0, iterations = 0;
    uint64_t node_visits = 0, tri_tests = 0;
    uint64_t shadow_node_visits = 0, shadow_tri_tests = 0;
};

void set_error(const std::string& msg);
const char* last_error();

#define TMPT_HIP(call)                                                                  \
    do {                                                                                \
        hipError_t e_ = (call);                                                         \
        if (e_ != hipSuccess) {                                                         \
            ::tmpt::set_error(std::string(#call) + ": " + hipGetErrorString(e_));       \
            return -1;                                                                  \
        }                                                                               \
    } while (0)

int build_lbvh(Scene& s, const float* d_tris9);
int build_soa(Scene& s);
int mark_flat_triangles(Scene& s, const std::vector<uint8_t>& flat);
int ensure_counters(Scene& s);
int check_report(Scene& s, const char* what);
void sample_jump_tables(int32_t spp, std::vector<uint32_t>& tab);
int radix_sort_pairs(uint32_t* keys, uint32_t* vals, uint32_t* tkeys, uint32_t* tvals, int32_t n,
                     int bits, uint32_t* hist, hipStream_t st);
size_t radix_sort_hist_words(int32_t n);
constexpr int32_t kRadixSortHookMax = 1 << 22;
int dump_bvh(Scene& s, bool soa, uint32_t* nodes, uint32_t* tris);
int radix_sort_host(Scene& s, uint32_t* keys, uint32_t* vals, int32_t n, int bits);

TMPT_HD float4 f4(float x, float y, float z, float w) { return make_float4(x, y, z, w); }

}
```

### toymeshpathtracer_amd/csrc/tmpt_path.h

```cpp
#pragma once

#include "tmpt_render.h"

namespace tmpt {

#ifndef TMPT_RSS_T
#define TMPT_RSS_T 8
#endif
constexpr int kRssT = TMPT_RSS_T;
static_assert(kRssT >= 4 && kRssT <= 31, "the worker's pick key holds the slot in 5 bits");
constexpr uint32_t kRssM24 = 0xFFFFFFu;
struct RsStream {
    unsigned long long* __restrict__ slots;
    unsigned long long* __restrict__ res;
    unsigned long long* __restrict__ chainpos;
    uint32_t* __restrict__ list;
    uint32_t* __restrict__ rowrays;
    uint32_t* __restrict__ lo;
    uint32_t* __restrict__ ctl;
    const uint32_t* __restrict__ anchors;
    const uint32_t* __restrict__ t1;
    const uint32_t* __restrict__ t2;
    uint32_t na, R, rmask;
    uint32_t jlimit;
    int nrows, nchase, nw;
    float spread;
    float room_lanes;
    uint32_t dyn;
    uint32_t watchdog;
    int test_abort;
};

__device__ __forceinline__ uint32_t rss_state(const RsStream& S, int row, uint32_t j)
{
    uint32_t s = S.anchors[(size_t)row * S.na + (j >> 14)];
    s = sample_seed(S.t2, (j >> 7) & 127u, s);
    return sample_seed(S.t1, j & 127u, s);
}

struct PathCtl {
    uint32_t* heads;
    uint32_t nchunks;
    uint32_t* simd_reg;
    uint32_t* claim;
    uint32_t nsimd, wps;
    int64_t P;
    const uint32_t* __restrict__ order;
    uint32_t* __restrict__ cost_out;
    float dprio[3];
    const uint32_t* __restrict__ dprio_cost;
    uint32_t lane_cap;
    uint32_t chunk;
    uint32_t nblk, blk;
    FastDiv div_nblk, div_blk;
    uint32_t blk0;
    uint32_t ua;
    float4* __restrict__ sbuf;
    uint32_t sb_ss, sb_sp;
    uint32_t pair;
    const uint32_t* __restrict__ upix;
    const uint32_t* __restrict__ ustate;
    float4* __restrict__ rs_out;
    uint32_t* __restrict__ rs_end;
    const uint32_t* __restrict__ p_dev;
    int rs_noshadow;
    const uint32_t* __restrict__ uslot;
    RsStream rss;
    uint2* __restrict__ redo;
    float4* __restrict__ redo_state;
    uint32_t redo_cap;
    uint32_t redo_inline;
    uint32_t redo_lanes;
    uint32_t oct_shadow;
    uint32_t top_walk;
};

struct PathVariant {
    bool count;
    int sl, steps, shade_min, occ;
    int prof;
    int help;
    int samp;
    bool soa;
    int ties;
    bool sums;
};

constexpr int kPathSL = 16, kPathSL5 = 12;

#ifndef TMPT_PATH_STEPS
#define TMPT_PATH_STEPS 16
#endif
#ifndef TMPT_PIX_STEPS
#define TMPT_PIX_STEPS 24
#endif
#ifndef TMPT_ROW_STEPS
#define TMPT_ROW_STEPS 16
#endif
#ifndef TMPT_ROW_SHADE_MIN
#define TMPT_ROW_SHADE_MIN 24
#endif
#ifndef TMPT_SHADE_MIN
#define TMPT_SHADE_MIN 16
#endif
#ifndef TMPT_SPARSE
#define TMPT_SPARSE 2
#endif
#ifndef TMPT_RS_OCC
#define TMPT_RS_OCC 5
#endif
constexpr int kSampleSteps = TMPT_PATH_STEPS, kShadeMin = TMPT_SHADE_MIN, kSparse = TMPT_SPARSE;
constexpr int kPixSteps = TMPT_PIX_STEPS;
constexpr int kRowSteps = TMPT_ROW_STEPS, kRowShadeMin = TMPT_ROW_SHADE_MIN;
constexpr int kRowIterSteps = 16, kRowIterShadeMin = 16;
constexpr int kRsOcc3 = TMPT_RS_OCC;
constexpr int path_tail(int samp) { return samp <= 1 ? kSparse : 2; }

using PathFn = void (*)(SceneView, RenderArgs, PathCtl, uint32_t*, uint32_t*, unsigned long long*);

PathFn path_kernel(const PathVariant& v);
int find_path_kernel(const PathVariant& v, const char* who, PathFn& fn);

struct PixelChains {
    const uint32_t* cpix;
    const float4* cinit;
    int n, smp0, cspp;
};

uint32_t top_walk_cap(const Options& o, int seeding);
uint32_t oct_shadow_check(const Scene& s);

void launch_resolve_px(hipStream_t stream, const float4* sbuf, int64_t P, int32_t spp, float spp_recip,
                       uint32_t* out);

#ifdef TMPT_EXP_WAVETIME
constexpr int kWaveTimeMax = 16384;
bool wavetime_get(unsigned long long* w);
bool rowtime_get(unsigned long long* r, unsigned long long* cl);
void wavetime_put(const unsigned long long* w);
void rowtime_put(const unsigned long long* r);
#endif

}
```

### toymeshpathtracer_amd/csrc/tmpt_render.hip

```cpp
#include <hip/hip_runtime.h>

#include <stdio.h>
#include <stdlib.h>
#include <string.h>

#include <algorithm>
#include <chrono>
#include <cmath>
#include <string>
#include <utility>
#include <vector>

#include "tmpt_lane_path.h"
#include "tmpt_path.h"

namespace tmpt {

#ifdef TMPT_EXP_WAVETIME
__device__ unsigned long long g_wavetime[3 * kWaveTimeMax];
__device__ unsigned long long g_rowtime[kWaveTimeMax];
__device__ unsigned long long g_claimtime[kWaveTimeMax];
bool wavetime_get(unsigned long long* w)
{
    return hipMemcpyFromSymbol(w, HIP_SYMBOL(g_wavetime), 3 * kWaveTimeMax * 8) == hipSuccess;
// ... 203 lines not shown
                               ((hw >> 8) & 15u)) * 4u) + ((hw >> 4) & 3u);
        r = hw & 15u;
        if (atomicAdd(&reg[2 * key], 1u) == 0) {
            d = atomicAdd(&reg[2 * kSimdKeys], 1u);
            __hip_atomic_store(&reg[2 * key + 1], d + 1u, __ATOMIC_RELAXED, __HIP_MEMORY_SCOPE_AGENT);
        } else {
            uint32_t v;
            while ((v = __hip_atomic_load(&reg[2 * key + 1], __ATOMIC_RELAXED, __HIP_MEMORY_SCOPE_AGENT)) == 0u)
                __builtin_amdgcn_s_sleep(2);
            d = v - 1u;
        }
    }
    return make_uint2((uint32_t)__shfl((int)r, 0), (uint32_t)__shfl((int)d, 0));
}

__device__ __forceinline__ unsigned long long rss_ld(const unsigned long long* p)
{
    return __hip_atomic_load(p, __ATOMIC_RELAXED, __HIP_MEMORY_SCOPE_AGENT);
}
__device__ __forceinline__ uint32_t rss_ld32(const uint32_t* p)
{
    return __hip_atomic_load(p, __ATOMIC_RELAXED, __HIP_MEMORY_SCOPE_AGENT);
}
__device__ __forceinline__ unsigned long long rss_win(uint32_t p, uint32_t q, uint32_t hi)
{
    return ((unsigned long long)(p + 1u) << 48) | ((unsigned long long)q << 24) | hi;
}

template <int BLOCK>
__device__ void rss_chaser(const RenderArgs& a, const RsStream& S, int wave)
{
    const int row = wave * 64 + lane_id();
    const bool mine = row < S.nrows;
    const uint32_t W = (uint32_t)a.W, spp = (uint32_t)a.spp, T = (uint32_t)kRssT;
    uint32_t c = 0, x = 0, k = 0, pdraws = 0, rays = 0, erays = 0, planned = 0;
    uint32_t n_wait = 0, n_ext = 0, n_pre = 0, n_sweep = 0;
    uint32_t stuck = 0;
    float mean = 17.0f;
    float spread = S.spread;
    uint32_t nw = (uint32_t)S.nw;
    bool done = !mine, err = false;
    unsigned long long* slot = S.slots + (size_t)(mine ? row : 0) * (T + 1u);
    uint32_t* lo = S.lo + (size_t)(mine ? row : 0) * T;
    const unsigned long long* res = S.res + (size_t)(mine ? row : 0) * T * S.R;
    const uint32_t cap_span = S.R - 64u;
    auto plan = [&](uint32_t q) {
        const float E = (float)spp * mean * 0.5f, rest = (float)(spp - k) * mean * 0.5f;
        const float i = (float)(q - x);
        const float P = (float)c + rest + (i - 1.0f) * E;
        const float lo_f = fmaxf((float)c, P - spread * sqrtf(i) * E);
        const float hi_f = P + E + spread * sqrtf(i + 1.0f) * E + 2.0f;
        const uint32_t l = (uint32_t)lo_f, h = min((uint32_t)hi_f, c + cap_span);
        lo[q % T] = l;
        __hip_atomic_exchange(&slot[q % T], rss_win(q, min(l, h), h), __ATOMIC_RELAXED, __HIP_MEMORY_SCOPE_AGENT);
    };
    if (mine) {
        const float E = (float)spp * mean * 0.5f;
        const uint32_t h = min((uint32_t)(E + S.spread * E) + 2u, cap_span);
        lo[0] = 0;
        __hip_atomic_exchange(&slot[0], rss_win(0, 0, h), __ATOMIC_RELAXED, __HIP_MEMORY_SCOPE_AGENT);
        planned = 0;
        while (planned + 1u < min(W, (uint32_t)S.nw)) plan(++planned);
    }
    for (;;) {
        bool moved = false;
        if (!done) {
            for (int it = 0; it < 64; ++it) {
                const unsigned long long w = rss_ld(res + (size_t)(x % T) * S.R + (c & S.rmask));
                if ((w >> 28) != (((unsigned long long)(x + 1u) << 24) | c)) {
                    if (++stuck < 3u) break;
                    stuck = 0;
                    const unsigned long long sw = rss_ld(&slot[x % T]);
                    const uint32_t q = (uint32_t)(sw >> 24) & kRssM24, hi = (uint32_t)sw & kRssM24;
                    const uint32_t l = lo[x % T];
                    const uint32_t rest = (uint32_t)((float)(spp - k) * mean * 0.65f) + 16u;
                    ++n_wait;
                    if (c < l) {
                        ++n_pre;
                        __hip_atomic_exchange(&slot[T], rss_win(x, c, min(l, c + cap_span)), __ATOMIC_RELAXED,
                                              __HIP_MEMORY_SCOPE_AGENT);
                        lo[x % T] = c;
                    } else if (c >= hi) {
                        ++n_ext;
                        __hip_atomic_exchange(&slot[x % T], rss_win(x, c, c + min(rest, cap_span)),
                                              __ATOMIC_RELAXED, __HIP_MEMORY_SCOPE_AGENT);
                    }
                    (void)q;
                    break;
                }
                stuck = 0;
                const uint32_t draws = (uint32_t)w & 0x3FFFu;
                rays += (uint32_t)(w >> 14) & 31u;
                erays += (uint32_t)(w >> 19) & 15u;
                pdraws += draws;
                S.list[((size_t)row * W + x) * spp + k] = c;
                c += draws >> 1;
                moved = true;
                if (c + cap_span >= S.jlimit) {
                    err = true;
                    done = true;
                    break;
                }
                if (++k == spp) {
                    mean = (float)pdraws / (float)k;
                    k = 0;
                    pdraws = 0;
                    if (++x == W) {
                        done = true;
                        break;
                    }
                    if (S.dyn) {
                        const uint32_t live = (uint32_t)S.nrows - min((uint32_t)S.nrows, rss_ld32(&S.ctl[0]));
                        const float room = S.room_lanes / (float)max(live, 1u);
                        if (S.dyn & 1u)
                            nw = (uint32_t)min((int)kRssT - 1, max(2, (int)rintf(2.6f + 1.5f * __logf(fmaxf(room, 1e-3f)))));
                        if (S.dyn & 2u) spread = fminf(0.25f, fmaxf(0.0f, 0.055f * room - 0.015f));
                    }
                    while (planned + 1u < W && planned < x + nw - 1u) plan(++planned);
                }
            }
            if (moved) __hip_atomic_store(&S.chainpos[row], ((unsigned long long)x << 32) | c, __ATOMIC_RELAXED,
                                          __HIP_MEMORY_SCOPE_AGENT);
            if (done) {
#ifdef TMPT_EXP_WAVETIME
                if (row < kWaveTimeMax) g_rowtime[row] = __builtin_amdgcn_s_memrealtime();
#endif
                S.rowrays[2 * row] = rays;
                S.rowrays[2 * row + 1] = erays;
                if (err) {
                    atomicExch(&S.ctl[3], 1u);
                    atomicExch(&S.ctl[1], 1u);
                }
                __threadfence();
                atomicAdd(&S.ctl[0], 1u);
            }
        }
        const uint64_t mv = wballot(moved);
        if (lane_id() == 0 && mv) atomicAdd(&S.ctl[2], 1u);
        ++n_sweep;
        if (!wany(!done)) break;
        if (rss_ld32(&S.ctl[1]) != 0u) break;
        if (!mv) __builtin_amdgcn_s_sleep(8);
    }
    if (mine) {
        atomicAdd(&S.ctl[8], n_wait);
        atomicAdd(&S.ctl[9], n_ext);
        atomicAdd(&S.ctl[10], n_pre);
    }
    if (lane_id() == 0) atomicAdd(&S.ctl[11], n_sweep);
}


template <bool COUNT, int BLOCK, int SL, int STEPS, int SHADE_MIN, int OCC = 1, int TAIL = 0, int PROF = 0,
          int HELP = 0, int SAMP = 0, bool SOA = false, int TIES = 0, bool SUMS = false>
__global__ void __launch_bounds__(BLOCK, OCC) k_path(SceneView sv, RenderArgs a, PathCtl pc,
                                                uint32_t* __restrict__ out,
                                                uint32_t* __restrict__ ovf,
                                                unsigned long long* __restrict__ counters)
{
    constexpr bool DEFER = TIES == 1, FLAG = TIES != 0;
    static_assert(!SUMS || SAMP == 1, "SUMS: the sample kernel's float sums");
    __shared__ uint32_t s_stack[SL * BLOCK];
    __shared__ float s_light[SAMP >= 3 ? 1 : kMaxDepth * BLOCK];
    constexpr bool NEXT3 = OCC >= 5;
    __shared__ float s_next[SAMP >= 3 ? 1 : (NEXT3 ? 3 : 6) * BLOCK];
    if (SAMP == 4) {
        __shared__ uint32_t s_ticket;
        if (threadIdx.x == 0) s_ticket = atomicAdd(&pc.rss.ctl[12], 1u);
        __syncthreads();
        const uint32_t ticket = s_ticket;
        if ((int)ticket < pc.rss.nchase) {
            if (!pc.rss.test_abort) rss_chaser<BLOCK>(a, pc.rss, (int)(ticket * (BLOCK / 64) + threadIdx.x / 64));
            return;
        }
    }
    const int64_t gtid = (int64_t)blockIdx.x * BLOCK + threadIdx.x;
    TravStack<BLOCK, SL> st{&s_stack[threadIdx.x], ovf + gtid * (kStackTotal - SL)};
    constexpr uint32_t LS = BLOCK;
    float* light = &s_light[threadIdx.x];
    float* nxt = &s_next[threadIdx.x];
    __shared__ uint8_t s_pair[HELP ? BLOCK : 1];
    {
        constexpr int kTop = OCC >= 5 ? kTopNodes5 : (HELP ? kTopNodes - 4 : kTopNodes);
        __shared__ uint4 s_top[kTop * 4];
        const uint32_t ntop = (uint32_t)min(kTop, sv.n_nodes4);
        const uint4* g = reinterpret_cast<const uint4*>(sv.nodes4);
        for (uint32_t i = threadIdx.x; i < ntop * 4; i += BLOCK) s_top[i] = g[i];
        __syncthreads();
        st.top = (const lds_u4*)s_top;
        st.ntop = ntop;
    }
    constexpr bool kFull = !SAMP;
    float dp0 = kFull ? pc.dprio[0] : 0.0f, dp1 = kFull ? pc.dprio[1] : 0.0f, dp2 = kFull ? pc.dprio[2] : 0.0f;
    if (kFull && pc.dprio_cost && pc.order && a.smp_begin > 0) {
        const float sc = (float)pc.dprio_cost[pc.order[0]] * (float)(a.smp_end - a.smp_begin) / (float)a.smp_begin;
        dp0 *= sc;
        dp1 *= sc;
        dp2 *= sc;
    }
    TravCount cnt, cnt_s;
    uint32_t rays_e = 0, rays_s = 0;
    const f3 ldir = light_dir();
    const uint64_t lt = (1ull << lane_id()) - 1ull;
    uint32_t seg = (uint32_t)(gtid >> 6) % kSeg, walked = 0;
    uint32_t res = 0, res_end = 0;
    if (SAMP == 2 || SAMP == 3) {
        pc.P = *pc.p_dev;
        pc.nchunks = (uint32_t)((pc.P + pc.chunk - 1) / pc.chunk);
    }
    bool exhausted = SAMP == 4 ? false : pc.P == 0;
    uint32_t crow = SAMP == 4 ? (uint32_t)((gtid >> 6) % (int64_t)max(1, pc.rss.nrows)) : 0u;
    uint32_t srow = 0, spx = 0, wd_tick = 0, n_claim = 0, n_miss = 0, n_cas = 0;
    uint32_t crow_rng = (uint32_t)(gtid >> 6) * 2654435761u + 1u;
    uint64_t wd_time = 0;
    if (kFull && pc.simd_reg && !exhausted) {
        const uint2 rd = simd_rank(pc.simd_reg);
        if (rd.x < pc.wps && rd.y < pc.nsimd) {
            const uint32_t c = rd.x * pc.nsimd + ((rd.x & 1u) ? pc.nsimd - 1u - rd.y : rd.y);
            uint32_t got = 0;
            if (c < pc.nchunks && lane_id() == 0) got = atomicExch(&pc.claim[c], 1u) == 0u;
            if (__shfl((int)got, 0)) {
                res = c * pc.chunk;
                res_end = (uint32_t)min<int64_t>((int64_t)res + pc.chunk, pc.P);
            } else if (c < pc.nchunks && lane_id() == 0) {
                atomicAdd(&counters[21], 1ull);
            }
        } else if (lane_id() == 0) {
            atomicAdd(&counters[20 + (rd.x >= pc.wps ? 2 : 3)], 1ull);
        }
        if (res >= res_end)
            for (int k = 0; k < 6; ++k) __builtin_amdgcn_s_sleep(127);
    }
#ifdef TMPT_EXP_WAVETIME
    const int wt_id = (int)(gtid >> 6);
    if (lane_id() == 0 && wt_id < kWaveTimeMax) g_wavetime[3 * wt_id] = __builtin_amdgcn_s_memrealtime();
#endif
    bool has_pix = false, in_query = false, qany = false;
    bool helper = false, waiting = false;
    uint32_t hown = 0;
    uint32_t pix = 0, rng = 0, smp = 0, depth = 0;
    uint32_t pf0 = 0, pf1 = 0, pf2 = 0, pf3 = 0, pf_smp = 0xFFFFFFFFu, pf_pix = 0;
    uint32_t cur_unit = 0, re0 = 0, rs0 = 0, ndraw = 0;
    bool single = false;
    uint32_t psteps = 0;
    uint64_t rs_nr = 0, rs_nl = 0, rs_lr = 0, rs_ll = 0, rs_sr = 0, rs_sl = 0, rs_st = 0;
    uint64_t pt_shade = 0, pt_node = 0, pt_leaf = 0, pt_t = PROF ? stamp() : 0;
    uint64_t ps_fetch = 0, ps_shade = 0, ps_cam = 0, ps_start = 0;
    uint64_t pc_sr = 0, pc_cr = 0, pc_cl = 0;
    uint64_t tv_n = 0, tv_lead = 0, tv_mix = 0, tv_only = 0, tw_r = 0, tw_l = 0;
    uint64_t pt_top = 0, pt_node_g = 0, pn_g = 0, pn_all = 0;
    bool lead = false;
    f3 col = mk(0.0f, 0.0f, 0.0f);
    TravRay r;
    TravState ts;
    trav_init(ts, kMaxT);

    for (;;) {
        const bool wants = has_pix ? !in_query : (HELP && helper ? !in_query : !exhausted);
        const uint64_t need = wballot(wants);
        const uint64_t trav = wballot(in_query);
        int shade_min = SHADE_MIN;
        if (TAIL > 0) {
            const int act = __popcll(wballot(has_pix));
            shade_min = max(1, min(SHADE_MIN, act / TAIL));
        }
        if (need != 0 && (__popcll(need) >= shade_min || trav == 0)) {
            if (COUNT || PROF >= 3) {
                ++rs_sr;
                rs_sl += (uint64_t)__popcll(need);
                rs_st += (uint64_t)__popcll(trav);
            }
            bool cam = false, start = false, sany = false;
            f3 so = mk(0.0f, 0.0f, 0.0f), sd = so;
            const uint64_t nopix = wballot(!has_pix && !(HELP && helper) && !exhausted);
            if (SAMP == 4 && nopix != 0 && res >= res_end && !exhausted) {
                const RsStream& S = pc.rss;
                const uint32_t T = (uint32_t)kRssT;
                const int natt = wany(has_pix) ? 1 : 4;
                for (int att = 0; att < natt && res >= res_end; ++att) {
                    const uint32_t x = (uint32_t)(rss_ld(&S.chainpos[crow]) >> 32);
                    bool moved_on = true;
                    if (x < (uint32_t)a.W) {
                        unsigned long long* sl = S.slots + (size_t)crow * (T + 1u);
                        const uint32_t ln = (uint32_t)lane_id();
                        unsigned long long w = 0;
                        if (ln <= T) w = rss_ld(&sl[ln]);
                        const uint32_t p1 = (uint32_t)(w >> 48), q = (uint32_t)(w >> 24) & kRssM24;
                        const uint32_t hi = (uint32_t)w & kRssM24;
                        const bool valid = ln <= T && p1 > x && p1 <= (uint32_t)a.W && q < hi;
                        uint32_t key = valid ? (((ln == T ? 0u : p1 - x) << 5) | ln) : 0xFFFFFFFFu;
                        for (int off = 1; off < 64; off <<= 1) key = min(key, (uint32_t)__shfl_xor((int)key, off));
                        if (key != 0xFFFFFFFFu) {
                            moved_on = false;
                            const int pick = (int)(key & 31u);
                            uint32_t got = 0, gq = 0, gp = 0;
                            if (ln == (uint32_t)pick) {
                                const uint32_t n = min((uint32_t)__popcll(nopix), hi - q);
                                const unsigned long long old = atomicAdd(&sl[ln], (unsigned long long)n << 24);
                                const uint32_t op = (uint32_t)(old >> 48), oq = (uint32_t)(old >> 24) & kRssM24;
                                const uint32_t ohi = (uint32_t)old & kRssM24;
                                if (op != 0u && oq < ohi) {
                                    got = min(n, ohi - oq);
                                    gq = oq;
                                    gp = op - 1u;
                                }
                            }
                            got = (uint32_t)__shfl((int)got, pick);
                            if (!got) ++n_cas;
                            if (got) {
                                ++n_claim;
#ifdef TMPT_EXP_WAVETIME
                                if (lane_id() == 0 && wt_id < kWaveTimeMax)
                                    g_claimtime[wt_id] = __builtin_amdgcn_s_memrealtime();
#endif
                                res = (uint32_t)__shfl((int)gq, pick);
                                res_end = res + got;
                                srow = crow;
                                spx = (uint32_t)__shfl((int)gp, pick);
                            }
                        }
                    }
                    if (moved_on) {
                        ++n_miss;
                        crow_rng ^= crow_rng << 13;
                        crow_rng ^= crow_rng >> 17;
                        crow_rng ^= crow_rng << 5;
                        crow = crow_rng % (uint32_t)S.nrows;
                    }
                }
                if (res >= res_end && (rss_ld32(&S.ctl[0]) >= (uint32_t)S.nrows || rss_ld32(&S.ctl[1]) != 0u))
                    exhausted = true;
            }
            if (nopix != 0) {
                while (SAMP != 4 && res >= res_end && !exhausted) {
                    const uint32_t c = seg < pc.nchunks ? (pc.nchunks - 1u - seg) / (uint32_t)kSeg + 1u : 0u;
                    uint32_t b = c;
                    if (c != 0) {
                        if (lane_id() == 0) b = atomicAdd(&pc.heads[seg * kCtr], 1u);
                        b = (uint32_t)__shfl((int)b, 0);
                    }
                    if (b < c && kFull && pc.claim) {
                        uint32_t got = 0;
                        if (lane_id() == 0) got = atomicExch(&pc.claim[seg + b * (uint32_t)kSeg], 1u) == 0u;
                        if (!__shfl((int)got, 0)) continue;
                    }
                    if (b < c) {
                        res = (seg + b * (uint32_t)kSeg) * pc.chunk;
                        res_end = (uint32_t)min<int64_t>((int64_t)res + pc.chunk, pc.P);
                    } else {
                        seg = (seg + 1) & 63u;
                        if (++walked == kSeg) exhausted = true;
                    }
                }
                uint32_t take = min((uint32_t)__popcll(nopix), res_end - res);
                if (pc.lane_cap < 64u)
                    take = min(take, pc.lane_cap - min(pc.lane_cap, (uint32_t)__popcll(wballot(has_pix))));
                const uint32_t k = (uint32_t)__popcll(nopix & lt);
                if (!has_pix && ((nopix >> lane_id()) & 1ull) && k < take) {
                    uint32_t smp0 = (uint32_t)a.smp_begin;
                    if (SAMP == 4) {
                        cur_unit = res + k;
                        pix = srow * (uint32_t)a.W + spx;
                        re0 = rays_e;
                        rs0 = rays_s;
                    } else if (SAMP >= 2) {
                        cur_unit = res + k;
                        pix = pc.upix ? pc.upix[cur_unit] : cur_unit / (uint32_t)a.spp;
                        if (pc.uslot) smp0 = pc.uslot[cur_unit];
                        else if (!pc.upix) smp0 = cur_unit - pix * (uint32_t)a.spp;
                        re0 = rays_e;
                        rs0 = rays_s;
                    } else if (SAMP && pc.nblk > 1) {
                        const uint32_t unit = res + k;
                        uint32_t q = unit, sub = 0u;
                        single = unit >= pc.ua;
                        if (single) {
                            const uint32_t v = unit - pc.ua, qv = fastdiv(v, pc.div_blk);
                            q = pc.ua + qv;
                            sub = v - qv * pc.blk;
                        }
                        pix = fastdiv(q, pc.div_nblk);
                        smp0 = (q - pix * pc.nblk + pc.blk0) * pc.blk + sub;
                    } else {
                        pix = (kFull && pc.order) ? pc.order[res + k] : res + k;
                    }
                    psteps = 0;
                    has_pix = true;
                    const int lr = (int)fastdiv(pix, a.div_w);
                    const int x = (int)(pix - (uint32_t)lr * (uint32_t)a.W);
                    if (SAMP == 4) {
                        rng = rss_state(pc.rss, (int)srow, cur_unit);
                    } else if (SAMP >= 2) {
                        rng = pc.ustate[cur_unit];
                    } else if (!kFull || a.smp_begin == 0) {
                        rng = pixel_seed((uint32_t)x, (uint32_t)tile_row_to_y_fd(a, lr), (uint32_t)a.W);
                        col = mk(0.0f, 0.0f, 0.0f);
                    } else {
                        const float4 pv = a.prog[pix];
                        col = mk(pv.x, pv.y, pv.z);
                        rng = __float_as_uint(pv.w);
                    }
                    smp = smp0;
                    depth = 0;
                    cam = true;
                }
                res += take;
            }
            if (HELP && helper && !in_query) {
                float* ol = &s_light[(threadIdx.x & ~63u) + (hown >> 4) + (hown & 15u) * BLOCK];
                const float v = *ol;
                *ol = ts.best >= 0 ? 0.0f : -v;
                helper = false;
            }
            if (HELP) __atomic_signal_fence(__ATOMIC_SEQ_CST);
            uint64_t ps_t = 0;
            if (PROF >= 2) {
                ps_t = stamp();
                ps_fetch += ps_t - pt_t;
            }
            bool settled = false;
            if (!DEFER && SAMP < 2) {
                const bool fin = has_pix && !in_query && !cam && !(HELP && waiting) && (!qany || pc.oct_shadow);
                uint64_t T = wballot(fin && octree_flag(sv, r, ts));
                if (T != 0) {
                    const OctView* ov = sv.oct;
                    do {
                        const int l = (int)__builtin_ctzll(T);
                        T &= T - 1;
                        const f3 qo = mk(rlane(r.o.x, l), rlane(r.o.y, l), rlane(r.o.z, l));
                        const f3 qd = mk(rlane(r.d.x, l), rlane(r.d.y, l), rlane(r.d.z, l));
                        const OctHit h = octree_walk_wave(ov->nodes, ov->refs, ov->n, sv.tri_orig, qo, qd, kMinT, kMaxT,
                                                          rlane(qany ? -INFINITY : ts.bt, l) TMPT_CHK_ARGS(sv));
                        if (lane_id() == l) {
                            octree_count(ov, ts.best);
                            ts.best = h.best;
                            ts.bt = h.t;
                            ts.bu = h.u;
                            ts.bv = h.v;
                            settled = true;
                        }
                    } while (T != 0);
                }
            }
            bool finish = false, want_off = false;
            f3 color = mk(0.0f, 0.0f, 0.0f);
            if (has_pix && !in_query && !cam) {
                if (HELP && waiting) {
                    finish = true;
                    if (depth < (uint32_t)kMaxDepth) color = sky(r.d);
                } else if (!qany) {
                    bool drop = false;
                    if (DEFER) {
                        drop = octree_flag(sv, r, ts);
                        if (wany(drop)) {
                            if (drop) {
                                const unsigned long long slot = atomicAdd(&counters[kRedoCounter], 1ull);
                                if (slot < (unsigned long long)pc.redo_cap) {
                                    redo_state_put(pc.redo_state + (size_t)slot * kRedoState4, r.o, r.d, rng, light,
                                                   depth, LS);
                                    __builtin_amdgcn_fence(__ATOMIC_RELEASE, "agent");
                                    redo_put(pc.redo + slot, pix, smp | (depth << 16));
                                }
                                rays_e -= 1u;
                                depth = 0;
                                ts.best = -1;
                            }
                        }
                        ts.best >>= 1;
                    } else if (SAMP >= 2) {
                        const bool tie = octree_flag(sv, r, ts);
                        if (wany(tie)) {
                            if (tie) settle_closest<BLOCK, SL, true, SOA, false>(sv, r, 0.0f, kMinT, kMaxT, ts, st);
                        }
                        if (!tie) ts.best >>= 1;
                    } else if (!settled) {
                        ts.best >>= 1;
                    }
                    if (ts.best >= 0) {
                        const float4* hp = reinterpret_cast<const float4*>(sv.tri_orig + ts.best);
                        float4 ha = hp[0], hb = hp[1], hc = hp[2];
                        f3 rnd = random_unit_vector(rng);
                        materialize(ha, hb, hc);
                        const f3 nrm = mk(hc.y, hc.z, hc.w);
                        const f3 pos = hit_pos(mk(ha.x, ha.y, ha.z), mk(ha.w, hb.x, hb.y), mk(hb.z, hb.w, hc.x),
                                               ts.bu, ts.bv);
                        const float lc = light_cosine(nrm, r.d);
                        if (SAMP < 3) light[depth * LS] = lc;
                        f3 target = pos + nrm + rnd;
                        f3 nd = normalize(target - pos);
                        ++depth;
                        if (SAMP < 3 && lc > 0.0f && !(SAMP == 2 && pc.rs_noshadow)) {
                            if (NEXT3) {
                                nxt[0] = nd.x; nxt[LS] = nd.y; nxt[2 * LS] = nd.z;
                            } else {
                                nxt[0] = pos.x; nxt[LS] = pos.y; nxt[2 * LS] = pos.z;
                                nxt[3 * LS] = nd.x; nxt[4 * LS] = nd.y; nxt[5 * LS] = nd.z;
                            }
                            start = true;
                            sany = true;
                            so = pos;
                            sd = ldir;
                            want_off = HELP != 0;
                        } else {
                            ++rays_s;
                            if (depth < (uint32_t)kMaxDepth) {
                                start = true;
                                so = pos;
                                sd = nd;
                            } else {
                                finish = true;
                            }
                        }
                    } else {
                        color = sky(r.d);
                        if (DEFER && drop) color.x = -1.0f;
                        finish = true;
                    }
                } else if (SAMP < 3) {
                    if (SAMP == 2 && pc.oct_shadow && octree_flag(sv, r, ts))
                        settle_any(sv, r, kMinT, kMaxT, ts);
                    if (ts.best >= 0) light[(depth - 1) * LS] = 0.0f;
                    if (depth < (uint32_t)kMaxDepth) {
                        start = true;
                        if (NEXT3) {
                            so = r.o;
                            sd = mk(nxt[0], nxt[LS], nxt[2 * LS]);
                        } else {
                            so = mk(nxt[0], nxt[LS], nxt[2 * LS]);
                            sd = mk(nxt[3 * LS], nxt[4 * LS], nxt[5 * LS]);
                        }
                    } else {
                        finish = true;
                    }
                }
            }
            if (HELP) {
                const uint64_t S = wballot(want_off);
                const uint64_t I = S ? wballot(!has_pix && !helper && !in_query) : 0ull;
                if (I != 0) {
                    const uint32_t n = min(__popcll(S), __popcll(I));
                    const uint32_t ks = (uint32_t)__popcll(S & lt), ki = (uint32_t)__popcll(I & lt);
                    const uint32_t wb = threadIdx.x & ~63u;
                    if (want_off && ks < n) s_pair[wb + ks] = (uint8_t)lane_id();
                    __atomic_signal_fence(__ATOMIC_SEQ_CST);
                    const bool idle = ((I >> lane_id()) & 1ull) != 0 && ki < n;
                    const int src = idle ? (int)s_pair[wb + ki] : (int)lane_id();
                    const float hx = __shfl(so.x, src), hy = __shfl(so.y, src), hz = __shfl(so.z, src);
                    const uint32_t hs = (uint32_t)__shfl((int)depth, src) - 1u;
                    if (want_off && ks < n) {
                        light[(depth - 1) * LS] = -light[(depth - 1) * LS];
                        sany = false;
                        if (depth < (uint32_t)kMaxDepth) {
                            sd = NEXT3 ? mk(nxt[0], nxt[LS], nxt[2 * LS]) : mk(nxt[3 * LS], nxt[4 * LS], nxt[5 * LS]);
                        } else {
                            start = false;
                            finish = true;
                        }
                    }
                    if (idle) {
                        helper = true;
                        hown = ((uint32_t)src << 4) | hs;
                        start = true;
                        sany = true;
                        so = mk(hx, hy, hz);
                        sd = ldir;
                    }
                }
            }
            if (finish) {
                bool pend = false;
                if (HELP)
                    for (int kk = 0; kk < (int)depth; ++kk) pend |= light[kk * LS] < 0.0f;
                waiting = pend;
                if (!pend) {
                    if (SAMP < 3)
                        for (int kk = (int)depth - 1; kk >= 0; --kk)
                            color = backward_step(color, light[kk * LS]);
                    if (SAMP == 2 && pc.sbuf) {
                        typedef float f32x4 __attribute__((ext_vector_type(4)));
                        __builtin_nontemporal_store((f32x4){color.x, color.y, color.z, 0.0f},
                                                    reinterpret_cast<f32x4*>(pc.sbuf + ((size_t)smp * pc.sb_ss +
                                                                                        (size_t)pix * pc.sb_sp)));
                    } else if (SAMP == 4) {
                        const uint32_t draws = ndraw + 2u * depth;
                        const uint32_t ne = rays_e - re0, nr = ne + rays_s - rs0;
                        const uint32_t row = pix / (uint32_t)a.W, p = pix - row * (uint32_t)a.W;
                        if (draws > 0x3FFFu) atomicExch(&pc.rss.ctl[3], 2u);
                        const unsigned long long word =
                            ((((unsigned long long)(p + 1u) << 24) | cur_unit) << 28) |
                            (unsigned long long)(min(draws, 0x3FFFu) | (nr << 14) | (ne << 19));
                        atomicMax(pc.rss.res + ((size_t)row * kRssT + p % kRssT) * pc.rss.R + (cur_unit & pc.rss.rmask),
                                  word);
                    } else if (SAMP >= 2) {
                        const uint32_t draws = ndraw + 2u * depth;
                        const uint32_t ne = rays_e - re0, nr = ne + rays_s - rs0;
                        pc.rs_out[cur_unit] =
                            make_float4(SAMP == 3 ? 0.0f : color.x, SAMP == 3 ? 0.0f : color.y, SAMP == 3 ? 0.0f : color.z,
                                        __uint_as_float(draws | (nr << 23) | (ne << 28)));
                        pc.rs_end[cur_unit] = rng;
                    } else if (SAMP && pc.sbuf) {
                        typedef float f32x4 __attribute__((ext_vector_type(4)));
                        f32x4* dst = reinterpret_cast<f32x4*>(pc.sbuf + ((size_t)smp * pc.sb_ss + (size_t)pix * pc.sb_sp));
                        const bool odd = (smp & 1u) != 0u;
                        if (pc.pair && !odd && !single && smp + 1u < (uint32_t)a.smp_end && ((smp + 1u) & a.bmask) != 0u) {
                            col = color;
                        } else {
                            if (pc.pair && odd && !single && (!DEFER || !(col.x < 0.0f)))
                                __builtin_nontemporal_store((f32x4){col.x, col.y, col.z, 0.0f}, dst - 1);
                            if (!DEFER || !(color.x < 0.0f))
                                __builtin_nontemporal_store((f32x4){color.x, color.y, color.z, 0.0f}, dst);
                        }
                    } else
                        col = col + color;
                    ++smp;
                    depth = 0;
                    if (smp < (uint32_t)a.smp_end && (!SAMP || ((smp & a.bmask) != 0u && !single))) {
                        cam = true;
                    } else {
                        if ((kFull || (SUMS && !pc.sbuf)) && a.prog)
                            a.prog[pix] = make_float4(col.x, col.y, col.z, __uint_as_float(rng));
                        if (kFull && pc.cost_out) pc.cost_out[pix] = psteps;
                        if (SAMP < 2 && (!SAMP || !pc.sbuf)) out[pix] = pack_pixel(col, a.out_recip);
                        has_pix = false;
                    }
                }
            }
            if (PROF >= 2) {
                const uint64_t t = stamp();
                ps_shade += t - ps_t;
                ps_t = t;
            }
            if (PROF >= 2) {
                const uint64_t cm = wballot(cam);
                ++pc_sr;
                if (cm != 0) {
                    ++pc_cr;
                    pc_cl += (uint64_t)__popcll(cm);
                }
            }
            if (cam) {
                const int lr = (int)fastdiv(pix, a.div_w);
                const int x = (int)(pix - (uint32_t)lr * (uint32_t)a.W);
                const uint32_t y = (uint32_t)tile_row_to_y_fd(a, lr);
                if (SAMP == 1) {
                    const uint32_t ps = pixel_seed((uint32_t)x, y, (uint32_t)a.W);
                    rng = (pf_smp == smp && pf_pix == pix) ? (pf0 ^ pf1 ^ pf2 ^ pf3) : sample_seed(a.jt, smp, ps);
                    const uint32_t* t = a.jt + (size_t)(smp + 1u) * 1024u;
                    const bool more = smp + 1u < (uint32_t)a.smp_end && ((smp + 1u) & a.bmask) != 0u && !single;
                    const uint32_t* tt = more ? t : a.jt;
                    pf0 = tt[ps & 255u];
                    pf1 = tt[256u + ((ps >> 8) & 255u)];
                    pf2 = tt[512u + ((ps >> 16) & 255u)];
                    pf3 = tt[768u + (ps >> 24)];
                    pf_smp = more ? smp + 1u : 0xFFFFFFFFu;
                    pf_pix = pix;
                }
                if (SAMP >= 2) {
                    ndraw = 0;
                    camera_sample(a.cam, (uint32_t)x, y, a.invW, a.invH, rng, so, sd, ndraw);
                } else {
                    camera_sample(a.cam, (uint32_t)x, y, a.invW, a.invH, rng, so, sd);
                }
                start = true;
            }
            if (PROF >= 2) {
                const uint64_t t = stamp();
                ps_cam += t - ps_t;
                ps_t = t;
            }
            if (start) {
                r = make_trav_ray(so, sd);
                trav_init(ts, kMaxT);
                qany = sany;
                if (sany) ++rays_s; else ++rays_e;
                in_query = sv.n > 0 && !ray_has_nan(so, sd);
                if (!DEFER && a.root_check && cam && in_query && !octree_root_hit(sv, so, sd, kMinT, kMaxT)) {
                    in_query = false;
                    atomicAdd(&sv.oct->ties[1], 1ull);
                }
            }
            if (PROF >= 2) ps_start += stamp() - ps_t;
            if (COUNT && start) lead = true;
            if (pc.top_walk) {
                uint64_t tw_t = 0;
                if (PROF) {
                    tw_t = stamp();
                    pt_shade += tw_t - pt_t;
                }
                for (uint32_t k = 0; k < pc.top_walk; ++k) {
                    const bool top = in_query && ts.node >= 0 && (uint32_t)ts.node < st.ntop;
                    const uint64_t tm = wballot(top);
                    if (tm == 0) break;
                    if (COUNT || PROF) {
                        ++tw_r;
                        tw_l += (uint64_t)__popcll(tm);
                    }
                    if (COUNT) {
                        tv_n += (uint64_t)__popcll(tm);
                        tv_lead += (uint64_t)__popcll(wballot(top && lead));
                    }
                    if (top) {
                        bool done;
                        if (!COUNT) {
                            done = trav_step4q2_mixed<false, BLOCK, SL, true, 1, SOA, false, FLAG, true>(sv, r, qany, ts, st,
                                                                                                        cnt);
                        } else {
                            TravCount c1;
                            done = trav_step4q2_mixed<COUNT, BLOCK, SL, true, 1, SOA, false, FLAG, true>(sv, r, qany, ts, st,
                                                                                                        c1);
                            (qany ? cnt_s : cnt).nodes += c1.nodes;
                            cnt.stale += c1.stale;
                            cnt.stale2 += c1.stale2;
                        }
                        if (done) in_query = false;
                        if ((kFull && pc.cost_out) || dp0 > 0.0f) ++psteps;
                    }
                }
                if (PROF) {
                    pt_t = stamp();
                    pt_top += pt_t - tw_t;
                }
            }
        }
        if (dp0 > 0.0f) {
            float rem = 0.0f;
            if (has_pix)
                rem = smp > (uint32_t)a.smp_begin
                          ? (float)psteps * (float)((uint32_t)a.smp_end - smp) *
                                __builtin_amdgcn_rcpf((float)(smp - (uint32_t)a.smp_begin))
                          : 3.0e38f;
            for (int o = 32; o > 0; o >>= 1) rem = fmaxf(rem, __shfl_xor(rem, o));
            if (rem >= dp0) __builtin_amdgcn_s_setprio(3);
            else if (rem >= dp1) __builtin_amdgcn_s_setprio(2);
            else if (rem >= dp2) __builtin_amdgcn_s_setprio(1);
            else __builtin_amdgcn_s_setprio(0);
        }
        if (PROF) {
            const uint64_t t = stamp();
            pt_shade += t - pt_t;
            pt_t = t;
        }
        if (!wany(in_query)) {
            if (exhausted && !wany(has_pix)) break;
            if (SAMP == 4 && !wany(has_pix)) {
                const uint32_t tick = rss_ld32(&pc.rss.ctl[2]);
                const uint64_t now = __builtin_amdgcn_s_memrealtime();
                if (tick != wd_tick || wd_time == 0) {
                    wd_tick = tick;
                    wd_time = now;
                } else if (now - wd_time > (uint64_t)pc.rss.watchdog) {
                    if (lane_id() == 0) atomicExch(&pc.rss.ctl[1], 1u);
                    exhausted = true;
                }
                __builtin_amdgcn_s_sleep(32);
            }
            continue;
        }
        for (int k = 0; k < STEPS; ++k) {
            const uint64_t q = wballot(in_query);
            const uint64_t at_leaf = q & wballot(ts.node < 0);
            const uint64_t at_node = q & ~at_leaf;
            if (q == 0) break;
            const uint32_t n_leaf = (uint32_t)__builtin_popcount((uint32_t)at_leaf) +
                                    (uint32_t)__builtin_popcount((uint32_t)(at_leaf >> 32));
            const uint32_t n_node = (uint32_t)__builtin_popcount((uint32_t)at_node) +
                                    (uint32_t)__builtin_popcount((uint32_t)(at_node >> 32));
            const bool leaf_round = n_leaf > n_node;
            if (COUNT || PROF >= 3) {
                if (!leaf_round) { ++rs_nr; rs_nl += (uint64_t)__popcll(at_node); }
                if (leaf_round) { ++rs_lr; rs_ll += (uint64_t)__popcll(at_leaf); }
            }
            uint64_t top_m = 0;
            if ((COUNT || PROF) && !leaf_round) top_m = at_node & wballot(ts.node >= 0 && (uint32_t)ts.node < st.ntop);
            if (COUNT) {
                tv_n += (uint64_t)__popcll(top_m);
                tv_lead += (uint64_t)__popcll(top_m & wballot(lead));
                if (top_m != 0) ++((at_node & ~top_m) != 0 ? tv_mix : tv_only);
                if (in_query && (ts.node < 0) == leaf_round && !((top_m >> lane_id()) & 1ull)) lead = false;
            }
            if (!COUNT) {
                const bool stepping = in_query && ((ts.node < 0) == leaf_round);
                bool done = false;
                if (leaf_round) {
                    if (stepping) done = trav_step4q2_mixed<false, BLOCK, SL, true, 2, SOA, false, FLAG>(sv, r, qany, ts, st, cnt);
                } else {
                    if (stepping) done = trav_step4q2_mixed<false, BLOCK, SL, true, 1, SOA, false, FLAG>(sv, r, qany, ts, st, cnt);
                }
                if (done) in_query = false;
                if (stepping && ((kFull && pc.cost_out) || dp0 > 0.0f)) ++psteps;
            } else if (in_query && (ts.node < 0) == leaf_round) {
                TravCount c1;
                if (trav_step4q2_mixed<COUNT, BLOCK, SL, true, 0, SOA, false, FLAG>(sv, r, qany, ts, st, c1)) in_query = false;
                TravCount& dst = qany ? cnt_s : cnt;
                dst.nodes += c1.nodes;
                dst.tris += c1.tris;
                dst.stale += c1.stale;
                dst.stale2 += c1.stale2;
                if ((kFull && pc.cost_out) || dp0 > 0.0f) ++psteps;
            }
            if (PROF) {
                const uint64_t t = stamp();
                (leaf_round ? pt_leaf : pt_node) += t - pt_t;
                if (!leaf_round) {
                    ++pn_all;
                    if ((at_node & ~top_m) != 0) {
                        ++pn_g;
                        pt_node_g += t - pt_t;
                    }
                }
                pt_t = t;
            }
        }
    }
#ifdef TMPT_EXP_WAVETIME
    if (lane_id() == 0 && wt_id < kWaveTimeMax) g_wavetime[3 * wt_id + 1] = __builtin_amdgcn_s_memrealtime();
#endif
    if (DEFER && pc.redo_inline) {
        constexpr uint64_t kRedoGuard = 2000000;
        const unsigned long long waves = (unsigned long long)gridDim.x * (BLOCK / 64);
        uint32_t t = 0;
        if (lane_id() == 0) {
            atomicAdd(&counters[kRedoWaves], 1ull);
            t = (uint32_t)atomicAdd(&counters[kRedoTaken], (unsigned long long)pc.redo_lanes);
        }
        t = lane_id() < pc.redo_lanes ? (uint32_t)__shfl((int)t, 0) + lane_id() : 0xFFFFFFFFu;
        unsigned long long seen = ~0ull;
        uint64_t since = 0;
        for (;;) {
            const unsigned long long listed =
                __hip_atomic_load(&counters[kRedoCounter], __ATOMIC_RELAXED, __HIP_MEMORY_SCOPE_AGENT);
            const uint32_t lim = (uint32_t)min(listed, (unsigned long long)pc.redo_cap);
            uint2 e = make_uint2(kRedoEmpty, 0u);
            if (t < lim) e = redo_load(pc.redo + t);
            const bool have = e.x < kRedoDone;
            if (wany(have)) {
                if (have) {
                    __builtin_amdgcn_fence(__ATOMIC_ACQUIRE, "agent");
                    redo_sample<BLOCK, SL>(sv, a, e.x, e.y, pc.redo_state + (size_t)t * kRedoState4, pc.sbuf, pc.sb_ss,
                                           pc.sb_sp, rays_e, rays_s, st, light);
                    redo_mark(pc.redo + t);
                    atomicAdd(&counters[kRedoTraced], 1ull);
                    t = (uint32_t)atomicAdd(&counters[kRedoTaken], 1ull);
                }
                since = 0;
                continue;
            }
            const unsigned long long past =
                __hip_atomic_load(&counters[kRedoWaves], __ATOMIC_RELAXED, __HIP_MEMORY_SCOPE_AGENT);
            if (past >= waves && !wany(t < lim)) break;
            const uint64_t now = __builtin_amdgcn_s_memrealtime();
            const unsigned long long sig = (past << 40) ^ listed;
            if (sig != seen || since == 0) {
                seen = sig;
                since = now;
            } else if (now - since > kRedoGuard) {
                break;
            }
            __builtin_amdgcn_s_sleep(16);
        }
    }
#ifdef TMPT_EXP_WAVETIME
    if (lane_id() == 0 && wt_id < kWaveTimeMax) g_wavetime[3 * wt_id + 2] = __builtin_amdgcn_s_memrealtime();
#endif
    if (SAMP == 4 && lane_id() == 0) {
        atomicAdd(&pc.rss.ctl[5], n_claim);
        atomicAdd(&pc.rss.ctl[6], n_miss);
        atomicAdd(&pc.rss.ctl[7], n_cas);
    }
    uint32_t re = wave_sum(rays_e), rs = wave_sum(rays_s);
    uint32_t nv = COUNT ? wave_sum(cnt.nodes) : 0u;
    uint32_t nt = COUNT ? wave_sum(cnt.tris) : 0u;
    uint32_t nvs = COUNT ? wave_sum(cnt_s.nodes) : 0u;
    uint32_t nts = COUNT ? wave_sum(cnt_s.tris) : 0u;
    uint32_t nst = COUNT ? wave_sum(cnt.stale) : 0u;
    uint32_t nst2 = COUNT ? wave_sum(cnt.stale2) : 0u;
    if (lane_id() == 0) {
        atomicAdd(&counters[0], (unsigned long long)(re + rs));
        atomicAdd(&counters[3], (unsigned long long)re);
        if (COUNT) {
            atomicAdd(&counters[kWalkCounter], (unsigned long long)nst);
            atomicAdd(&counters[kWalkCounter + 1], (unsigned long long)nst2);
            atomicAdd(&counters[1], (unsigned long long)nv);
            atomicAdd(&counters[2], (unsigned long long)nt);
            atomicAdd(&counters[4], (unsigned long long)nvs);
            atomicAdd(&counters[5], (unsigned long long)nts);
        }
        if (COUNT || PROF >= 3) {
            atomicAdd(&counters[6], (unsigned long long)rs_nr);
            atomicAdd(&counters[7], (unsigned long long)rs_nl);
            atomicAdd(&counters[8], (unsigned long long)rs_lr);
            atomicAdd(&counters[9], (unsigned long long)rs_ll);
            atomicAdd(&counters[10], (unsigned long long)rs_sr);
            atomicAdd(&counters[11], (unsigned long long)rs_sl);
            atomicAdd(&counters[12], (unsigned long long)rs_st);
        }
        if (PROF) {
            atomicAdd(&counters[13], (unsigned long long)pt_shade);
            atomicAdd(&counters[14], (unsigned long long)pt_node);
            atomicAdd(&counters[15], (unsigned long long)pt_leaf);
        }
        if (PROF >= 2) {
            atomicAdd(&counters[16], (unsigned long long)ps_fetch);
            atomicAdd(&counters[17], (unsigned long long)ps_shade);
            atomicAdd(&counters[18], (unsigned long long)ps_cam);
            atomicAdd(&counters[19], (unsigned long long)ps_start);
            atomicAdd(&counters[kCamCounter], (unsigned long long)pc_sr);
            atomicAdd(&counters[kCamCounter + 1], (unsigned long long)pc_cr);
            atomicAdd(&counters[kCamCounter + 2], (unsigned long long)pc_cl);
        }
        if (COUNT) {
            atomicAdd(&counters[kTopCounter], (unsigned long long)tv_n);
            atomicAdd(&counters[kTopCounter + 1], (unsigned long long)tv_lead);
            atomicAdd(&counters[kTopCounter + 2], (unsigned long long)tv_mix);
            atomicAdd(&counters[kTopCounter + 3], (unsigned long long)tv_only);
        }
        if (COUNT || PROF) {
            atomicAdd(&counters[kTopCounter + 4], (unsigned long long)tw_r);
            atomicAdd(&counters[kTopCounter + 5], (unsigned long long)tw_l);
        }
        if (PROF) {
            atomicAdd(&counters[kTopCounter + 6], (unsigned long long)pt_top);
            atomicAdd(&counters[kTopCounter + 7], (unsigned long long)pt_node_g);
            atomicAdd(&counters[kTopCounter + 8], (unsigned long long)pn_g);
            atomicAdd(&counters[kTopCounter + 9], (unsigned long long)pn_all);
        }
    }
}

namespace {
constexpr bool F = false, T = true;
constexpr PathVariant kPathVariants[] = {
    {F, kPathSL, kSampleSteps, kShadeMin, 4, 0, 0, 1, F, 0, F},
    {F, kPathSL, kSampleSteps, kShadeMin, 4, 0, 0, 1, F, 2, F},
    {F, kPathSL, kSampleSteps, kShadeMin, 4, 0, 0, 1, F, 1, F},
    {F, kPathSL, kSampleSteps, kShadeMin, 4, 0, 0, 1, F, 0, T},
    {F, kPathSL, kSampleSteps, kShadeMin, 4, 0, 0, 1, F, 2, T},
    {T, kPathSL, kSampleSteps, kShadeMin, 4, 0, 0, 1, F, 0, F},
    {F, kPathSL, kSampleSteps, kShadeMin, 4, 0, 0, 1, T, 0, F},
    {F, kPathSL, kSampleSteps, kShadeMin, 4, 0, 0, 1, T, 0, T},
    {T, kPathSL, kSampleSteps, kShadeMin, 4, 0, 0, 1, T, 0, F},
    {F, kPathSL5, kSampleSteps, kShadeMin, 5, 0, 0, 1, F, 0, F},
    {F, kPathSL5, kSampleSteps, kShadeMin, 5, 0, 0, 1, F, 2, F},
    {F, kPathSL5, kSampleSteps, kShadeMin, 5, 0, 0, 1, F, 1, F},
    {F, kPathSL5, kSampleSteps, kShadeMin, 5, 0, 0, 1, F, 0, T},
    {F, kPathSL5, kSampleSteps, kShadeMin, 5, 0, 0, 1, F, 2, T},
    {F, kPathSL, kPixSteps, kShadeMin, 4, 0, 0, 0, F, 0, F},
    {F, kPathSL, kPixSteps, kShadeMin, 4, 0, 0, 0, F, 2, F},
    {F, kPathSL, kPixSteps, kShadeMin, 4, 0, 1, 0, F, 0, F},
    {F, kPathSL, kPixSteps, kShadeMin, 4, 0, 1, 0, F, 2, F},
    {T, kPathSL, kPixSteps, kShadeMin, 4, 0, 0, 0, F, 0, F},
    {F, kPathSL5, kPixSteps, kShadeMin, 5, 0, 0, 0, F, 0, F},
    {F, kPathSL5, kPixSteps, kShadeMin, 5, 0, 0, 0, F, 2, F},
    {F, kPathSL5, kPixSteps, kShadeMin, 5, 0, 1, 0, F, 0, F},
    {F, kPathSL5, kPixSteps, kShadeMin, 5, 0, 1, 0, F, 2, F},
    {F, kPathSL, kRowIterSteps, kRowIterShadeMin, 4, 0, 0, 2, F, 0, F},
    {F, kPathSL, kRowIterSteps, kRowIterShadeMin, kRsOcc3, 0, 0, 3, F, 0, F},
    {F, kPathSL, kRowSteps, kRowShadeMin, 4, 0, 0, 2, F, 0, F},
    {F, kPathSL, kRowSteps, kRowShadeMin, 4, 0, 0, 2, F, 2, F},
    {F, kPathSL5, kRowSteps, kRowShadeMin, 5, 0, 0, 2, F, 0, F},
    {F, kPathSL5, kRowSteps, kRowShadeMin, 5, 0, 0, 2, F, 2, F},
    {F, kPathSL, kRowSteps, kRowShadeMin, 4, 0, 0, 4, F, 0, F},
    {F, kPathSL, kRowSteps, kRowShadeMin, 4, 0, 0, 4, F, 2, F},
    {F, kPathSL, kRowSteps, kRowShadeMin, kRsOcc3, 0, 0, 4, F, 0, F},
    {F, kPathSL, kRowSteps, kRowShadeMin, kRsOcc3, 0, 0, 4, F, 2, F},
#ifdef TMPT_DIAG
    {F, kPathSL, kPixSteps, kShadeMin, 1, 1, 0, 0, F, 0, F},
    {F, kPathSL, kPixSteps, kShadeMin, 1, 2, 0, 0, F, 0, F},
    {F, kPathSL, kPixSteps, kShadeMin, 1, 3, 0, 0, F, 0, F},
    {F, kPathSL, kSampleSteps, kShadeMin, 1, 1, 0, 1, F, 0, F},
    {F, kPathSL, kSampleSteps, kShadeMin, 1, 2, 0, 1, F, 0, F},
    {F, kPathSL5, kSampleSteps, kShadeMin, 5, 2, 0, 1, F, 0, F},
#endif
};
constexpr size_t kNumPathVariants = sizeof(kPathVariants) / sizeof(kPathVariants[0]);

constexpr bool same_variant(const PathVariant& a, const PathVariant& b)
{
    return a.count == b.count && a.sl == b.sl && a.steps == b.steps && a.shade_min == b.shade_min && a.occ == b.occ &&
           a.prof == b.prof && a.help == b.help && a.samp == b.samp && a.soa == b.soa && a.ties == b.ties &&
           a.sums == b.sums;
}

template <size_t I>
constexpr PathFn variant_kernel()
{
    constexpr PathVariant v = kPathVariants[I];
    return k_path<v.count, kBlk, v.sl, v.steps, v.shade_min, v.occ, path_tail(v.samp), v.prof, v.help, v.samp, v.soa,
                  v.ties, v.sums>;
}

template <size_t... I>
PathFn kernel_at(size_t i, std::index_sequence<I...>)
{
    static const PathFn fns[] = {variant_kernel<I>()...};
    return fns[i];
}
}

PathFn path_kernel(const PathVariant& v)
{
    for (size_t i = 0; i < kNumPathVariants; ++i)
        if (same_variant(v, kPathVariants[i])) return kernel_at(i, std::make_index_sequence<kNumPathVariants>{});
    return nullptr;
}

int find_path_kernel(const PathVariant& v, const char* who, PathFn& fn)
{
    fn = path_kernel(v);
    if (fn) return 0;
    set_error(std::string(who) + ": no k_path kernel for count " + std::to_string(v.count) + ", sl " +
              std::to_string(v.sl) + ", steps " + std::to_string(v.steps) + ", shade_min " +
              std::to_string(v.shade_min) + ", occ " + std::to_string(v.occ) + ", prof " + std::to_string(v.prof) +
              ", help " + std::to_string(v.help) + ", samp " + std::to_string(v.samp) + ", soa " +
              std::to_string(v.soa) + ", ties " + std::to_string(v.ties) + ", sums " + std::to_string(v.sums));
    return -22;
}

__global__ void __launch_bounds__(256) k_pair_order(const uint32_t* __restrict__ order, int64_t P, int32_t h,
                                                     uint32_t* __restrict__ paired)
{
    const int64_t r = (int64_t)blockIdx.x * 256 + threadIdx.x;
    if (r >= P) return;
    const int64_t full = P / 64, c = r / 64, i = r - c * 64;
    const int64_t m = c < full ? 64 : P - full * 64;
    const int64_t hc = c < full ? h : (m * h + 63) / 64;
    const int64_t src = i < hc ? c * h + i : P - 1 - (c * (64 - h) + (i - hc));
    paired[r] = order[src];
}

__global__ void __launch_bounds__(256) k_order_keys(const uint32_t* __restrict__ cost, int32_t W,
                                                     int32_t rows, uint32_t* __restrict__ keys,
                                                     uint32_t* __restrict__ vals)
{
    const int64_t i = (int64_t)blockIdx.x * 256 + threadIdx.x;
    if (i >= (int64_t)W * rows) return;
    const int y = (int)(i / W), x = (int)(i - (int64_t)y * W);
    uint32_t sum = 0;
    for (int dy = -1; dy <= 1; ++dy) {
        const int yy = y + dy;
        if (yy < 0 || yy >= rows) continue;
        for (int dx = -1; dx <= 1; ++dx) {
            const int xx = x + dx;
            if (xx >= 0 && xx < W) sum += cost[(int64_t)yy * W + xx];
        }
    }
    keys[i] = 65535u - min(sum, 65535u);
    vals[i] = (uint32_t)i;
}

__global__ void __launch_bounds__(64) k_resolve_px(const float4* __restrict__ sbuf, int64_t P, int32_t spp,
                                                    float spp_recip, uint32_t* __restrict__ out,
                                                    int32_t s_begin = 0, int32_t s_end = -1,
                                                    float4* __restrict__ prog = nullptr)
{
    constexpr int kC = 16;
    __shared__ float4 tile[64][kC + 1];
    const int64_t p0 = (int64_t)blockIdx.x * 64;
    const int t = threadIdx.x;
    const int np = (int)min<int64_t>(64, P - p0);
    if (s_end < 0) s_end = spp;
    f3 col = mk(0.0f, 0.0f, 0.0f);
    if (prog && s_begin > 0 && t < np) {
        const float4 c = prog[p0 + t];
        col = mk(c.x, c.y, c.z);
    }
    for (int32_t s0 = s_begin; s0 < s_end; s0 += kC) {
        const int nc = min(kC, s_end - s0);
        for (int e = t; e < 64 * kC; e += 64) {
            const int i = e / kC, j = e - i * kC;
            if (i < np && j < nc) tile[i][j] = sbuf[(size_t)(p0 + i) * (size_t)spp + (size_t)(s0 + j)];
        }
        __syncthreads();
        if (t < np)
            for (int j = 0; j < nc; ++j) col = col + mk(tile[t][j].x, tile[t][j].y, tile[t][j].z);
        __syncthreads();
    }
    if (t < np) {
        if (prog) prog[p0 + t] = make_float4(col.x, col.y, col.z, 0.0f);
        out[p0 + t] = pack_pixel(col, spp_recip);
    }
}

void launch_resolve_px(hipStream_t stream, const float4* sbuf, int64_t P, int32_t spp, float spp_recip,
                       uint32_t* out)
{
    k_resolve_px<<<(unsigned)((P + 63) / 64), 64, 0, stream>>>(sbuf, P, spp, spp_recip, out);
}

int occupancy_grid(const void* fn, int block, size_t dyn_lds, int device)
{
    int per_cu = 0, cus = 0;
    if (hipOccupancyMaxActiveBlocksPerMultiprocessor(&per_cu, fn, block, dyn_lds) != hipSuccess ||
        per_cu < 1)
        per_cu = 1;
    if (hipDeviceGetAttribute(&cus, hipDeviceAttributeMultiprocessorCount, device) != hipSuccess ||
        cus < 1)
        cus = 256;
    return per_cu * cus;
}

int ensure_ws(Scene& s, size_t bytes)
{
    if (s.ws_bytes >= bytes) return 0;
    if (s.ws) (void)hipFree(s.ws);
    s.ws = nullptr;
    s.ws_bytes = 0;
    TMPT_HIP(hipMalloc(&s.ws, bytes));
    s.ws_bytes = bytes;
    return 0;
}

static float shadow_order_weight(const Options& o, bool row)
{
    const int order = o.shadow_order >= 0 ? o.shadow_order : row ? 0 : kShadowOrderDefault;
    return order == 0 ? 0.0f : order == 1 ? -1.0f : -1024.0f;
}

static bool pop_cull_on(const Scene& s)
{
    if (s.opt.pop_cull >= 0) return s.opt.pop_cull != 0;
    return (s.row_render ? kPopCullRow : s.pixel_render ? kPopCullPixel : kPopCullSample) != 0;
}

SceneView view(const Scene& s)
{
    SceneView v{s.nodes4, s.tri_pre, s.tri_orig, s.n, s.n_nodes4};
    v.soa = s.soa;
    v.any_w = shadow_order_weight(s.opt, s.row_render);
    v.count_shift = (uint32_t)s.count_shift;
    v.key_mask = pop_cull_on(s) ? pop_key_mask(pop_key_bits(s.link_bits, s.opt.pop_key_cap)) : 0u;
#ifdef TMPT_CHECK
    v.chk = s.chk;
    if (const char* e = getenv("TMPT_CHECK_SELFTEST"))
        if (atoi(e) == 1) v.n_nodes4 = std::min(v.n_nodes4, 1);
#endif
    if (s.oct && s.opt.tie_rule == 0) {
        v.oct = s.oct_view;
        const OctGrid& g = s.oct_grid;
        v.crack = make_float4(g.reach, g.drift[0], g.drift[1], g.drift[2]);
    }
    return v;
}

namespace {

void gf2_mul(const uint32_t* x, const uint32_t* y, uint32_t* out)
{
    uint32_t t[32];
    for (int j = 0; j < 32; ++j) {
        uint32_t r = 0;
        for (int i = 0; i < 32; ++i)
            if ((y[j] >> i) & 1u) r ^= x[i];
        t[j] = r;
    }
    memcpy(out, t, sizeof t);
}

void xorshift_power(uint64_t n, uint32_t* acc)
{
    uint32_t m[32];
    for (int j = 0; j < 32; ++j) {
        uint32_t v = 1u << j;
        m[j] = xorshift32(v);
        acc[j] = 1u << j;
    }
    for (; n; n >>= 1) {
        if (n & 1u) gf2_mul(m, acc, acc);
        gf2_mul(m, m, m);
    }
}

}

void jump_tables(uint64_t stride_steps, int32_t count, std::vector<uint32_t>& tab)
{
    uint32_t stride[32], J[32];
    xorshift_power(stride_steps, stride);
    for (int j = 0; j < 32; ++j) J[j] = 1u << j;
    tab.assign((size_t)count * 1024u, 0u);
    for (int32_t i = 0; i < count; ++i) {
        uint32_t* t = tab.data() + (size_t)i * 1024u;
        for (int k = 0; k < 4; ++k)
            for (uint32_t b = 1; b < 256; ++b)
                t[256 * k + b] = t[256 * k + (b & (b - 1u))] ^ J[8 * k + __builtin_ctz(b)];
        gf2_mul(stride, J, J);
    }
}

void sample_jump_tables(int32_t spp, std::vector<uint32_t>& tab) { jump_tables(kSampleStride, spp, tab); }

RenderArgs make_args(const tmpt_camera* c, const tmpt_render_desc* d)
{
    RenderArgs a;
    a.cam.origin = mk(c->origin[0], c->origin[1], c->origin[2]);
    a.cam.lower_left = mk(c->lower_left[0], c->lower_left[1], c->lower_left[2]);
    a.cam.horizontal = mk(c->horizontal[0], c->horizontal[1], c->horizontal[2]);
    a.cam.vertical = mk(c->vertical[0], c->vertical[1], c->vertical[2]);
    a.cam.u = mk(c->u[0], c->u[1], c->u[2]);
    a.cam.v = mk(c->v[0], c->v[1], c->v[2]);
    a.cam.w = mk(c->w[0], c->w[1], c->w[2]);
    a.cam.lens_radius = c->lens_radius;
    a.W = d->width;
    a.H = d->height;
    a.spp = d->spp;
    a.seed_mode = d->seed_mode;
    a.band_rows = d->band_rows > 0 ? d->band_rows : d->height;
    a.shard = d->num_shards > 1 ? d->shard : 0;
    a.nshards = d->num_shards > 1 ? d->num_shards : 1;
    a.tile_rows = tmpt_tile_rows(d);
    a.invW = 1.0f / (float)d->width;
    a.invH = 1.0f / (float)d->height;
    a.spp_recip = 1.0f / (float)d->spp;
    a.slots = (int64_t)a.tile_rows * a.W;
    a.smp_begin = d->spp_begin;
    a.smp_end = d->spp_count > 0 ? d->spp_begin + d->spp_count : d->spp;
    a.out_recip = a.smp_end == d->spp ? a.spp_recip : 1.0f / (float)a.smp_end;
    a.prog = nullptr;
    a.jt = nullptr;
    a.bmask = 2047u;
    a.row_lanes = 1;
    a.root_check = 0;
    a.div_w = fastdiv_make((uint32_t)a.W);
    a.div_band = fastdiv_make((uint32_t)a.band_rows);
    return a;
}

constexpr int kTopWalkSample = 4, kTopWalkPixel = 0, kTopWalkRow = 4;
uint32_t top_walk_cap(const Options& o, int seeding)
{
    if (o.top_walk >= 0) return (uint32_t)o.top_walk;
    return (uint32_t)(seeding == 0 ? kTopWalkSample : seeding == 1 ? kTopWalkPixel : kTopWalkRow);
}

uint32_t oct_shadow_check(const Scene& s)
{
    if (!s.oct_view || s.opt.tie_rule != 0) return 0u;
    if (s.oct_flat > 0) return 1u;
    const f3 ld = light_dir();
    const float l[3] = {fabsf(ld.x), fabsf(ld.y), fabsf(ld.z)};
    for (int k = 0; k < 3; ++k)
        if (l[k] * fminf(kMinT, s.oct_grid.reach) <= s.oct_grid.drift[k]) return 1u;
    return 0u;
}

int render_persistent(Scene& s, const RenderArgs& a, uint32_t* d_out, bool count,
                      unsigned long long* d_counters)
{
    const Options& o = s.opt;
    if (!s.path_ev[0])
        for (auto& e : s.path_ev) TMPT_HIP(hipEventCreate(&e));
    const bool jt = a.jt != nullptr;
    const bool oct = s.oct_view && o.tie_rule == 0;
    int prof = 0;
#ifdef TMPT_DIAG
    if (const char* pe = getenv("TMPT_PROF")) prof = count ? 0 : atoi(pe);
#endif
    const int prof_level = !prof ? 0 : prof >= 3 && !jt ? 3 : prof >= 2 ? 2 : 1;
    const bool soa = s.soa.na != nullptr;
    const bool soa_kernel = jt && soa && !prof;
    const bool prof5 = prof == 2 && jt && !soa && o.path_waves != 4;
    const bool waves5 = jt && !count && (!prof || prof5) && !soa && o.path_waves != 4;
    const bool flag = oct && !count && !prof && !soa_kernel;
    auto variant = [&](bool w5, int help, int ties, bool sums) {
        PathVariant v{};
        v.count = count;
        v.sl = w5 ? kPathSL5 : kPathSL;
        v.steps = jt ? kSampleSteps : kPixSteps;
        v.shade_min = kShadeMin;
        v.occ = w5 ? 5 : prof ? 1 : 4;
        v.prof = prof_level;
        v.help = help;
        v.samp = jt ? 1 : 0;
        v.soa = soa_kernel;
        v.ties = ties;
        v.sums = sums;
        return v;
    };
    PathVariant probe5{};
    probe5.sl = kPathSL5;
    probe5.steps = kSampleSteps;
    probe5.shade_min = kShadeMin;
    probe5.occ = 5;
    probe5.samp = 1;
    probe5.ties = 1;
    PathFn fn_base, fn_probe5;
    if (int rc = find_path_kernel(variant(prof5, 0, 0, false), "tmpt_render", fn_base)) return rc;
    if (int rc = find_path_kernel(probe5, "tmpt_render", fn_probe5)) return rc;
    const int grid4 = occupancy_grid((const void*)fn_base, kBlk, 0, s.device);
    const int grid5 = occupancy_grid((const void*)fn_probe5, kBlk, 0, s.device);
    const bool waves5p = !jt && !count && !prof &&
                         (o.path_waves == 5 || (o.path_waves == 0 && a.slots >= 3 * (int64_t)grid4 * kBlk));
    const int grid = waves5 || waves5p ? grid5 : grid4;
    uint32_t blk = 1u, nblk = 1u, blk0 = 0u;
    const bool pass = a.jt && (a.smp_begin > 0 || a.smp_end < a.spp);
    const int64_t s0 = a.smp_begin, s1 = a.smp_end;
    if (a.jt) {
        const int64_t kUnitsPerLane = waves5 ? 12 : 15;
        const int64_t lanes0 = (int64_t)grid * kBlk;
        blk = 1u;
        while ((int64_t)blk * 2 <= 8 && blk * 2u <= (uint32_t)(s1 - s0) &&
               a.slots * ((s1 - s0 + blk * 2 - 1) / (blk * 2)) >= kUnitsPerLane * lanes0)
            blk *= 2u;
        if (o.sample_block > 0) blk = (uint32_t)o.sample_block;
        while (a.slots * ((s1 - s0 + blk - 1) / blk) >= (1ll << 31)) blk *= 2u;
        while (s0 % blk) blk /= 2u;
        if (a.slots * ((s1 - s0 + blk - 1) / blk) >= (1ll << 31)) {
            set_error("tmpt_render: this progressive pass (samples " + std::to_string(s0) + ".." +
                      std::to_string(s1) + " of " + std::to_string(a.slots) +
                      " pixels) needs more than 2^31 sample units at the block size its first sample allows (" +
                      std::to_string(blk) + "): start passes at a multiple of a larger power of two, or render "
                      "the frame in one call");
            return -22;
        }
        blk0 = (uint32_t)(s0 / blk);
        nblk = (uint32_t)((s1 + blk - 1) / blk - blk0);
        if (nblk > 1 || pass) {
            const size_t need = sizeof(float4) * (size_t)a.spp * (size_t)a.slots;
            size_t fr = 0, tot = 0;
            size_t budget = hipMemGetInfo(&fr, &tot) == hipSuccess ? fr / 4 * 3 : 0;
            budget += s.sbuf_bytes;
            if (o.sbuf_max > 0.0) budget = std::min(budget, (size_t)o.sbuf_max);
            if (need > budget) {
                if (pass) {
                    set_error("tmpt_render: progressive passes in sample seeding need the per-sample colour buffer (" +
                              std::to_string(need >> 20) + " MiB), which does not fit: render the frame in one call");
                    return -12;
                }
                while (blk < (uint32_t)a.spp) blk *= 2u;
                nblk = 1u;
            }
        }
    }
    int64_t P = a.slots * (int64_t)nblk;
    uint32_t ua = 0xFFFFFFFFu;
    int64_t tail_blocks = o.sample_tail;
    if (tail_blocks < 0) {
        const int64_t spl = a.slots * (s1 - s0) / std::max<int64_t>(1, (int64_t)grid * kBlk);
        const int64_t b = std::max<uint32_t>(1u, blk);
        tail_blocks = std::max<int64_t>(1, (std::min<int64_t>(64, spl / 4) + b - 1) / b);
    }
    if (a.jt && nblk > 1 && blk >= 2u && tail_blocks > 0 && (s1 - s0) % blk == 0) {
        int64_t nb = std::min<int64_t>(P, tail_blocks * grid * kBlk);
        while (nb > 0 && (P - nb) + nb * (int64_t)blk >= (1ll << 31)) nb /= 2;
        if (nb > 0) {
            ua = (uint32_t)(P - nb);
            P = (P - nb) + nb * (int64_t)blk;
        }
    }
    int pilot = 2 * P <= 5 * (int64_t)grid * kBlk ? 2 : 4;
    if (o.pilot >= 0) pilot = o.pilot;
    const bool ordered = pilot > 0 && !count && !a.jt && a.smp_begin == 0 && a.smp_end == a.spp &&
                         a.spp >= 2 * pilot && P < (1ll << 31);
    const int64_t lanes = (int64_t)grid * kBlk;
    int help = ordered && !prof && 2 * P <= 9 * lanes ? 1 : 0;
    if (o.help >= 0) help = o.help != 0 && !count && !prof && !jt;
    const uint32_t oct_shadow = oct_shadow_check(s);
    if (oct_shadow) help = 0;
    int pair = help && ordered ? (2 * P <= 3 * lanes ? 52 : 56) : 0;
    if (o.pair >= 0) pair = o.pair;
    const bool w5 = jt ? waves5 : waves5p;
    const size_t ovf_words = std::max((size_t)grid4 * (kStackTotal - kPathSL),
                                      (size_t)std::max(grid4, grid5) * (kStackTotal - kPathSL5)) * kBlk;
    const size_t head_words = (size_t)kSeg * kCtr;
    const size_t hist_words = ordered ? radix_sort_hist_words((int32_t)P) : 0;
    const size_t reg_words = ordered ? 2 * (size_t)kSimdKeys + 64 + (size_t)P : 0;
    const size_t extra_words = ordered ? (size_t)P * (4 + 5) + hist_words + reg_words : 0;
    if (ensure_ws(s, (ovf_words + head_words + extra_words) * 4)) return -1;
    uint32_t* heads = (uint32_t*)s.ws + ovf_words;
    TMPT_HIP(hipMemsetAsync(heads, 0, head_words * 4, s.stream));
    PathCtl pc;
    memset(&pc, 0, sizeof(pc));
    pc.heads = heads;
    pc.oct_shadow = oct_shadow;
    pc.top_walk = top_walk_cap(o, a.jt ? 0 : 1);
    pc.P = P;
    pc.nblk = nblk;
    pc.blk = blk;
    pc.div_nblk = fastdiv_make(nblk);
    pc.div_blk = fastdiv_make(blk);
    pc.blk0 = blk0;
    pc.ua = ua;
    RenderArgs as = a;
    if (a.jt) {
        as.bmask = nblk > 1 ? blk - 1u : 2047u;
        if (nblk > 1 || pass) {
            const size_t need = sizeof(float4) * (size_t)a.spp * (size_t)a.slots;
            if (s.sbuf_bytes < need) {
                if (s.sbuf) (void)hipFree(s.sbuf);
                s.sbuf = nullptr;
                s.sbuf_bytes = 0;
                TMPT_HIP(hipMalloc(&s.sbuf, need));
                s.sbuf_bytes = need;
            }
            pc.sbuf = s.sbuf;
        }
    }
    pc.sb_ss = 1u;
    pc.sb_sp = (uint32_t)a.spp;
    pc.pair = pc.sbuf && blk >= 2u && a.spp % 2 == 0 && o.sbuf_pair ? 1u : 0u;
    {
        const int64_t waves = std::max<int64_t>(1, (int64_t)grid * (kBlk / 64));
        int64_t c = P <= waves * 16 ? 32 : 64;
        if (o.wave_cap > 0) c = o.wave_cap;
        pc.lane_cap = (uint32_t)std::max<int64_t>(1, std::min<int64_t>(64, c));
    }
    pc.chunk = std::min<uint32_t>(kChunk, pc.lane_cap);
    pc.nchunks = (uint32_t)((P + pc.chunk - 1) / pc.chunk);
    if (!ordered) {
        const bool defer = jt && !count && !prof && !soa && pc.sbuf && a.root_check == 0 && o.tie_defer != 0 &&
                           !oct_shadow &&
                           (o.tie_defer > 0 || a.slots * (int64_t)a.spp >= (waves5 ? 48 : 192) * lanes);
        bool redo = defer && oct;
        if (redo && o.redo_cap > 0 && s.redo_cap != (uint32_t)o.redo_cap) free_redo(s);
        if (redo && s.redo_cap == 0) {
            int64_t cap = std::min<int64_t>(1ll << 31, std::max<int64_t>(1 << 16, a.slots * (int64_t)a.spp / 128));
            if (o.redo_cap > 0) cap = o.redo_cap;
            (void)alloc_redo(s, cap);
        }
        const bool redo_nomem = redo && s.redo_cap == 0;
        if (redo_nomem) redo = false;
        const bool sums = jt && a.prog && !pc.sbuf;
        if (sums && (count || prof)) {
            set_error("tmpt_render_radiance: no instrumented kernel stores the float sums");
            return -22;
        }
        PathVariant v_main = variant(w5, help, flag ? (redo ? 1 : 2) : 0, sums);
        PathFn fn_main;
        if (int rc = find_path_kernel(v_main, "tmpt_render", fn_main)) return rc;
        int grid_main = occupancy_grid((const void*)fn_main, kBlk, 0, s.device);
        if ((size_t)grid_main * kBlk * (kStackTotal - kPathSL5) > ovf_words) {
            set_error("tmpt_render: internal: stack spill area sized for fewer lanes");
            return -1;
        }
        s.tie_path = !oct ? 0 : redo ? 2 : redo_nomem ? 3 : 1;
        s.path_launches = 1;
        for (int attempt = 0;; ++attempt) {
            pc.redo = redo ? s.redo : nullptr;
            pc.redo_state = redo ? s.redo_state : nullptr;
            pc.redo_cap = redo ? s.redo_cap : 0u;
            pc.redo_inline = o.redo_inline ? 1u : 0u;
            pc.redo_lanes = (uint32_t)std::max(1, std::min(64, o.redo_lanes));
            if (redo) TMPT_HIP(hipMemsetAsync(s.redo, 0xFF, sizeof(uint2) * (size_t)s.redo_cap, s.stream));
            TMPT_HIP(hipEventRecord(s.path_ev[2], s.stream));
            fn_main<<<grid_main, kBlk, 0, s.stream>>>(view(s), as, pc, d_out, (uint32_t*)s.ws, d_counters);
            TMPT_HIP(hipGetLastError());
            TMPT_HIP(hipEventRecord(s.path_ev[3], s.stream));
            if (!redo) break;
            TMPT_HIP(hipMemcpyAsync(s.counters_host + kRedoCounter, d_counters + kRedoCounter,
                                    4 * sizeof(unsigned long long), hipMemcpyDeviceToHost, s.stream));
            TMPT_HIP(hipStreamSynchronize(s.stream));
            const unsigned long long n = s.counters_host[kRedoCounter];
            const unsigned long long traced = s.counters_host[kRedoTraced];
            s.redo_samples = (int64_t)n;
            if (n > s.redo_cap && attempt == 0) {
                if (!(n < (1ull << 31) && alloc_redo(s, (int64_t)n))) {
                    redo = false;
                    v_main.ties = 2;
                    if (int rc = find_path_kernel(v_main, "tmpt_render", fn_main)) return rc;
                    grid_main = occupancy_grid((const void*)fn_main, kBlk, 0, s.device);
                    s.redo_samples = 0;
                    s.tie_path = 3;
                }
                TMPT_HIP(hipMemsetAsync(d_counters, 0, kRenderCounters * sizeof(unsigned long long), s.stream));
                TMPT_HIP(hipMemsetAsync(heads, 0, head_words * 4, s.stream));
                continue;
            }
            s.redo_late = (int64_t)(std::min<unsigned long long>(n, s.redo_cap) - std::min(traced, n));
            if (traced < std::min<unsigned long long>(n, s.redo_cap)) {
                TMPT_HIP(hipEventRecord(s.path_ev[0], s.stream));
                k_redo<kBlk, kPathSL><<<grid, kBlk, 0, s.stream>>>(view(s), as, s.redo, s.redo_cap, s.redo_state,
                                                                  pc.sbuf, pc.sb_ss, pc.sb_sp, (uint32_t*)s.ws,
                                                                  d_counters);
                TMPT_HIP(hipGetLastError());
                TMPT_HIP(hipEventRecord(s.path_ev[1], s.stream));
                s.redo_launches = 1;
            }
            break;
        }
        if (pc.sbuf) {
            k_resolve_px<<<(unsigned)((a.slots + 63) / 64), 64, 0, s.stream>>>(
                pc.sbuf, a.slots, a.spp, a.out_recip, d_out, a.smp_begin, a.smp_end, a.prog);
            TMPT_HIP(hipGetLastError());
        }
        return 0;
    }
    s.tie_path = oct ? 1 : 0;
    PathFn fn;
    if (int rc = find_path_kernel(variant(w5, help, flag ? 2 : 0, false), "tmpt_render", fn)) return rc;
    const int grid_px = occupancy_grid((const void*)fn, kBlk, 0, s.device);
    if ((size_t)grid_px * kBlk * (kStackTotal - (waves5p ? kPathSL5 : kPathSL)) > ovf_words) {
        set_error("tmpt_render: internal: stack spill area sized for fewer lanes");
        return -1;
    }
    uint32_t* base = heads + head_words;
    float4* state = reinterpret_cast<float4*>(base);
    uint32_t* cost = base + 4 * (size_t)P;
    uint32_t* keys = cost + P;
    uint32_t* vals = keys + P;
    uint32_t* tkeys = vals + P;
    uint32_t* tvals = tkeys + P;
    uint32_t* hist = tvals + P;
    uint32_t* simd_reg = hist + hist_words;
    RenderArgs a1 = a;
    a1.smp_end = pilot;
    a1.out_recip = 1.0f / (float)pilot;
    a1.prog = state;
    pc.cost_out = cost;
    TMPT_HIP(hipEventRecord(s.path_ev[0], s.stream));
    fn<<<grid_px, kBlk, 0, s.stream>>>(view(s), a1, pc, d_out, (uint32_t*)s.ws, d_counters);
    TMPT_HIP(hipGetLastError());
    TMPT_HIP(hipEventRecord(s.path_ev[1], s.stream));
    k_order_keys<<<(unsigned)((P + 255) / 256), 256, 0, s.stream>>>(cost, a.W, a.tile_rows, keys, vals);
    const int which = radix_sort_pairs(keys, vals, tkeys, tvals, (int32_t)P, 16, hist, s.stream);
    TMPT_HIP(hipMemsetAsync(heads, 0, head_words * 4, s.stream));
    RenderArgs a2 = a;
    a2.smp_begin = pilot;
    a2.prog = state;
    pc.cost_out = nullptr;
    pc.order = which ? tvals : vals;
    int64_t nch = 0;
    {
        int per1024 = 0;
        if (o.pixel_chains >= 0) per1024 = o.pixel_chains;
        nch = std::min<int64_t>(P, (P * per1024 + 1023) / 1024);
    }
    if (nch > 0) {
        const PixelChains ch{pc.order, state, (int)nch, pilot, a.spp - pilot};
        const int rc = render_rowspec(s, a, d_out, d_counters, &ch);
        if (rc < 0) return rc;
        if (rc == 0) {
            pc.order += nch;
            pc.P = P - nch;
            pc.nchunks = (uint32_t)((pc.P + pc.chunk - 1) / pc.chunk);
        }
        s.chain_pixels = rc == 0 ? nch : 0;
    }
    if (pair > 0 && pair < 64 && pc.chunk == 64u) {
        uint32_t* paired = which ? vals : tvals;
        k_pair_order<<<(unsigned)((pc.P + 255) / 256), 256, 0, s.stream>>>(pc.order, pc.P, pair, paired);
        pc.order = paired;
    }
    if (o.balance) {
        int dev_cus = 0;
        if (hipDeviceGetAttribute(&dev_cus, hipDeviceAttributeMultiprocessorCount, s.device) != hipSuccess ||
            dev_cus < 1)
            dev_cus = 256;
        const uint32_t per_cu = (uint32_t)std::max(1, grid_px / dev_cus);
        pc.simd_reg = simd_reg;
        pc.nsimd = (uint32_t)dev_cus * 4u;
        pc.wps = per_cu * (uint32_t)(kBlk / 64) / 4u;
        pc.claim = simd_reg + 2 * (size_t)kSimdKeys + 64;
        TMPT_HIP(hipMemsetAsync(simd_reg, 0, reg_words * 4, s.stream));
    }
    if (ordered && o.dprio && P <= 12 * lanes) {
        pc.dprio[0] = 0.32f;
        pc.dprio[1] = 0.21f;
        pc.dprio[2] = 0.105f;
        pc.dprio_cost = cost;
    }
    TMPT_HIP(hipEventRecord(s.path_ev[2], s.stream));
    fn<<<grid_px, kBlk, 0, s.stream>>>(view(s), a2, pc, d_out, (uint32_t*)s.ws, d_counters);
    TMPT_HIP(hipGetLastError());
    TMPT_HIP(hipEventRecord(s.path_ev[3], s.stream));
    s.path_launches = 2;
    if (a.prog)
        TMPT_HIP(hipMemcpyAsync(a.prog, state, sizeof(float4) * (size_t)P, hipMemcpyDeviceToDevice, s.stream));
    return 0;
}

int ensure_counters(Scene& s)
{
    if (s.counters) return 0;
    TMPT_HIP(hipMalloc(&s.counters, kRenderCounters * sizeof(unsigned long long)));
    TMPT_HIP(hipMemset(s.counters, 0, kRenderCounters * sizeof(unsigned long long)));
    TMPT_HIP(hipHostMalloc((void**)&s.counters_host, kRenderCounters * sizeof(unsigned long long),
                           hipHostMallocDefault));
    for (auto& e : s.render_ev) TMPT_HIP(hipEventCreate(&e));
    s.ties = s.counters + kTieCounter;
#ifdef TMPT_CHECK
    TMPT_HIP(hipMalloc(&s.chk, 4 * sizeof(uint32_t)));
    TMPT_HIP(hipMemset(s.chk, 0, 4 * sizeof(uint32_t)));
#endif
    return 0;
}

int check_report(Scene& s, const char* what)
{
#ifdef TMPT_CHECK
    if (!s.chk) return 0;
    uint32_t h[3] = {0, 0, 0};
    TMPT_HIP(hipDeviceSynchronize());
    TMPT_HIP(hipMemcpy(h, s.chk, sizeof(h), hipMemcpyDeviceToHost));
    if (h[0] == 0) return 0;
    TMPT_HIP(hipMemset(s.chk, 0, 4 * sizeof(uint32_t)));
    char msg[256];
    snprintf(msg, sizeof(msg),
             "%s: device index check failed: codes 0x%x (1 node, 2 leaf, 4 stack, 8 octree skip, 16 octree refs, "
             "32 triangle id), %u times, last value %d",
             what, h[0], h[1], (int)h[2]);
    fprintf(stderr, "tmpt: %s\n", msg);
    set_error(msg);
    return kCheckError;
#else
    (void)s;
    (void)what;
    return 0;
#endif
}

int ensure_sample_tables(Scene& s, int32_t spp, const char* what)
{
    if (s.jt_spp >= spp) return 0;
    std::vector<uint32_t> tab;
    sample_jump_tables(spp, tab);
    uint32_t* nt = nullptr;
    TMPT_HIP(hipMalloc(&nt, tab.size() * sizeof(uint32_t)));
    if (hipMemcpy(nt, tab.data(), tab.size() * sizeof(uint32_t), hipMemcpyHostToDevice) != hipSuccess) {
        (void)hipFree(nt);
        set_error(std::string(what) + ": jump table upload failed");
        return -1;
    }
    if (s.jt) (void)hipFree(s.jt);
    s.jt = nt;
    s.jt_spp = spp;
    return 0;
}

int wait_caller_stream(Scene& s, const tmpt_render_desc* d, const char* what)
{
    if (!(d->flags & TMPT_FLAG_WAIT_STREAM)) return 0;
    if (!s.wait_ev) TMPT_HIP(hipEventCreateWithFlags(&s.wait_ev, hipEventDisableTiming));
    hipError_t e = hipEventRecord(s.wait_ev, reinterpret_cast<hipStream_t>(static_cast<uintptr_t>(d->wait_stream)));
    if (e == hipSuccess) e = hipStreamWaitEvent(s.stream, s.wait_ev, 0);
    if (e != hipSuccess) {
        set_error(std::string(what) + ": wait_stream: " + hipGetErrorString(e));
        return -1;
    }
    return 0;
}

int32_t camera_root_check(const Scene& s, const Camera& cam)
{
    if (!(s.oct && s.opt.tie_rule == 0)) return 0;
    const float o[3] = {cam.origin.x, cam.origin.y, cam.origin.z};
    const float uu[3] = {cam.u.x, cam.u.y, cam.u.z}, vv[3] = {cam.v.x, cam.v.y, cam.v.z};
    bool inside = true;
    for (int c = 0; c < 3; ++c) {
        const double r = (double)cam.lens_radius * (std::fabs((double)uu[c]) + std::fabs((double)vv[c]));
        const double m = 2.0 * kMinT + 1e-4 * ((double)s.oct_hi[c] - (double)s.oct_lo[c]);
        inside = inside && (double)o[c] - r > (double)s.oct_lo[c] + m && (double)o[c] + r < (double)s.oct_hi[c] - m;
    }
    return inside ? 0 : 1;
}

void reset_render_stats(Scene& s)
{
    s.extend_ms = s.shadow_ms = 0;
    s.extend_rays = s.shadow_rays = s.node_visits = s.tri_tests = 0;
    s.shadow_node_visits = s.shadow_tri_tests = 0;
    s.extend_launches = s.shadow_launches = s.iterations = 0;
    s.row_engine = 0;
    s.stream_fallbacks = 0;
    s.chain_pixels = 0;
    s.redo_samples = 0;
    s.redo_late = 0;
    s.redo_launches = 0;
    s.redo_ms = 0.0;
    s.redo_rays = 0;
    s.tie_path = 0;
}

__global__ void __launch_bounds__(256) k_radiance_scale(float4* __restrict__ px, int64_t n, float spp_recip)
{
    const int64_t i = (int64_t)blockIdx.x * 256 + threadIdx.x;
    if (i >= n) return;
    const float4 c = px[i];
    const f3 col = mk(c.x, c.y, c.z) * spp_recip;
    px[i] = make_float4(col.x, col.y, col.z, 1.0f);
}

int render(Scene& s, const tmpt_camera* cam, const tmpt_render_desc* d, uint32_t* d_out,
           uint64_t* ray_count, float4* d_sums)
{
    RenderArgs a = make_args(cam, d);
    bool count = (d->flags & TMPT_FLAG_COUNT_VISITS) != 0;
    s.row_render = d->seed_mode == TMPT_SEED_ROW;
    s.pixel_render = d->seed_mode == TMPT_SEED_PIXEL;
    const bool progressive = a.smp_begin > 0 || a.smp_end < a.spp;
    if (progressive) {
        const int32_t key[6] = {d->width, d->height, d->spp, a.band_rows, a.shard, a.nshards};
        uint64_t cam_key = 1469598103934665603ull;
        const unsigned char* cb = reinterpret_cast<const unsigned char*>(cam);
        for (size_t i = 0; i < sizeof(tmpt_camera); ++i) cam_key = (cam_key ^ cb[i]) * 1099511628211ull;
        cam_key = (cam_key ^ (uint32_t)d->seed_mode) * 1099511628211ull;
        if (a.smp_begin > 0 &&
            (memcmp(key, s.prog_key, sizeof(key)) != 0 || s.prog_key[6] != a.smp_begin || s.prog_cam != cam_key)) {
            set_error("tmpt_render: spp_begin does not continue the previous pass of this shard "
                      "(same camera, size, spp and shard)");
            return -22;
        }
        s.prog_cam = cam_key;
        if (s.prog_slots < (size_t)a.slots) {
            if (s.prog) (void)hipFree(s.prog);
            s.prog = nullptr;
            s.prog_slots = 0;
            TMPT_HIP(hipMalloc(&s.prog, sizeof(float4) * (size_t)a.slots));
            s.prog_slots = (size_t)a.slots;
        }
        a.prog = s.prog;
        memcpy(s.prog_key, key, sizeof(key));
        s.prog_key[6] = -1;
    } else if (d_sums) {
        a.prog = d_sums;
    }
    if (a.seed_mode == TMPT_SEED_SAMPLE) {
        if (int rc = ensure_sample_tables(s, a.spp, "tmpt_render")) return rc;
        a.jt = s.jt;
    }
    if (int rc = wait_caller_stream(s, d, "tmpt_render")) return rc;
    if (ensure_counters(s)) return -1;
    a.root_check = camera_root_check(s, a.cam);
    unsigned long long* d_counters = s.counters;
    TMPT_HIP(hipMemsetAsync(d_counters, 0, kRenderCounters * sizeof(unsigned long long), s.stream));
    hipEvent_t e0 = s.render_ev[0], e1 = s.render_ev[1];
    TMPT_HIP(hipEventRecord(e0, s.stream));
    int rc = 0;
    const bool wave = d->engine == TMPT_ENGINE_WAVEFRONT && a.seed_mode != TMPT_SEED_ROW;
    const bool persistent = d->engine == TMPT_ENGINE_PERSISTENT && a.seed_mode != TMPT_SEED_ROW;
    const bool rowspec = d->engine == TMPT_ENGINE_PERSISTENT && a.seed_mode == TMPT_SEED_ROW && !count &&
                         !progressive && s.opt.rowspec != 0;
    if (progressive && !persistent) {
        set_error("tmpt_render: progressive spp needs the persistent engine");
        return -22;
    }
    reset_render_stats(s);
    if (a.slots > 0) {
        if (wave) rc = render_wavefront(s, a, d_out, count);
        else if (persistent) rc = render_persistent(s, a, d_out, count, d_counters);
        else if (rowspec) {
            rc = s.opt.rowspec_stream != 0 && s.opt.rowspec_noshadow != 0 ? render_rowstream(s, a, d_out, d_counters)
                                                                          : 1;
            s.row_engine = rc == 0 ? 3 : 2;
            if (rc == 2) {
                s.stream_fallbacks = 1;
                TMPT_HIP(hipMemsetAsync(d_counters, 0, kRenderCounters * sizeof(unsigned long long), s.stream));
            }
            if (rc == 1 || rc == 2) rc = render_rowspec(s, a, d_out, d_counters);
        } else {
            rc = render_megakernel(s, a, d_out, count, d_counters);
            if (a.seed_mode == TMPT_SEED_ROW) s.row_engine = 1;
        }
        if (rc == 0 && d_sums) {
            k_radiance_scale<<<(unsigned)((a.slots + 255) / 256), 256, 0, s.stream>>>(d_sums, a.slots, a.spp_recip);
            if (hipGetLastError() != hipSuccess) rc = (set_error("tmpt_render_radiance: scale launch failed"), -1);
        }
    }
    (void)hipEventRecord(e1, s.stream);
    hipError_t se = rc == 0 ? hipMemcpyAsync(s.counters_host, d_counters, kRenderCounters * sizeof(unsigned long long),
                                             hipMemcpyDeviceToHost, s.stream)
                            : hipSuccess;
    const hipError_t se2 = hipStreamSynchronize(s.stream);
    if (se == hipSuccess) se = se2;
    unsigned long long c[kRenderCounters] = {};
    if (rc == 0 && se == hipSuccess) memcpy(c, s.counters_host, sizeof(c));
    float ms = 0;
    (void)hipEventElapsedTime(&ms, e0, e1);
    if (rc) return rc;
    if (se != hipSuccess) {
        set_error(std::string("render: ") + hipGetErrorString(se));
        return -1;
    }
    s.render_ms = ms;
    s.tie_queries = c[kTieCounter];
    s.root_misses = c[kTieCounter + 1];
    s.crack_queries = c[kCrackCounter];
#ifdef TMPT_EXP_WAVETIME
    {
        std::vector<unsigned long long> w(3 * kWaveTimeMax, 0ull);
        if (wavetime_get(w.data())) {
            std::vector<double> st, ml, ex;
            unsigned long long t0 = ~0ull;
            for (int i = 0; i < kWaveTimeMax; ++i)
                if (w[3 * i] && w[3 * i + 2]) t0 = std::min(t0, w[3 * i]);
            for (int i = 0; i < kWaveTimeMax; ++i)
                if (w[3 * i] && w[3 * i + 2]) {
                    st.push_back((w[3 * i] - t0) * 0.01);
                    ml.push_back((w[3 * i + 1] - t0) * 0.01);
                    ex.push_back((w[3 * i + 2] - t0) * 0.01);
                }
            auto pct = [](std::vector<double> v, double q) {
                if (v.empty()) return 0.0;
                std::sort(v.begin(), v.end());
                return v[std::min(v.size() - 1, (size_t)(q * (v.size() - 1)))];
            };
            fprintf(stderr, "waves %zu; start us p0/p50/p100 %.0f/%.0f/%.0f; main loop end p0/p10/p50/p90/p100 "
                            "%.0f/%.0f/%.0f/%.0f/%.0f; exit p0/p50/p99/p100 %.0f/%.0f/%.0f/%.0f\n",
                    st.size(), pct(st, 0), pct(st, 0.5), pct(st, 1), pct(ml, 0), pct(ml, 0.1), pct(ml, 0.5),
                    pct(ml, 0.9), pct(ml, 1), pct(ex, 0), pct(ex, 0.5), pct(ex, 0.99), pct(ex, 1));
            std::fill(w.begin(), w.end(), 0ull);
            wavetime_put(w.data());
        }
    }
#endif
    if (progressive) s.prog_key[6] = a.smp_end < a.spp ? a.smp_end : -1;
    if (persistent) {
        float k1 = 0.0f, k0 = 0.0f;
        (void)hipEventElapsedTime(&k1, s.path_ev[2], s.path_ev[3]);
        if (s.path_launches == 2) (void)hipEventElapsedTime(&k0, s.path_ev[0], s.path_ev[1]);
        s.extend_ms = (double)k0 + (double)k1;
        if (s.redo_launches) {
            float kr = 0.0f;
            (void)hipEventElapsedTime(&kr, s.path_ev[0], s.path_ev[1]);
            s.redo_ms = kr;
            s.redo_rays = c[kRedoRaysCounter];
        }
        s.extend_rays = c[3];
        s.shadow_rays = c[0] - c[3];
        s.node_visits = c[1];
        s.tri_tests = c[2];
        s.shadow_node_visits = c[4];
        s.shadow_tri_tests = c[5];
        s.extend_launches = s.path_launches;
// ... 79 lines not shown
```

Measured before the change: 10960.

## Precompute camera rays in a separate kernel and load them in the path kernel

Adds a k_cam_rays pre-pass that generates each primary ray's origin, direction, RNG state and NaN/root-miss flags into a device buffer. The 5-wave sample path kernel (new CAM template variants) then loads this 32-byte entry with two nontemporal loads instead of computing pixel seeds, camera sampling and the octree root test inline. The goal is to shorten the register- and ALU-heavy camera path inside the persistent megakernel. In exchange it adds an extra launch and a large buffer (slots×spp×32 bytes) that is written and then read back through HBM, with a fallback when memory is short.

```diff
diff --git a/include/tmpt.h b/include/tmpt.h
--- a/include/tmpt.h
+++ b/include/tmpt.h
@@ -148,6 +148,8 @@
 
 int tmpt_fastdiv(uint32_t divisor, const uint32_t* x, uint64_t n, uint32_t* out, uint32_t mul_shift[2]);
 
+int tmpt_camera_rays(tmpt_scene* scene, const tmpt_camera* cam, const tmpt_render_desc* desc, uint32_t* out);
+
 int tmpt_scene_dump_bvh(const tmpt_scene* scene, int32_t layout, uint32_t* nodes, uint64_t node_words,
                         uint32_t* tris, uint64_t tri_words, int32_t info[8]);
 int tmpt_radix_sort(const tmpt_scene* scene, uint32_t* keys, uint32_t* vals, int64_t n, int32_t bits);
diff --git a/toymeshpathtracer_amd/__init__.py b/toymeshpathtracer_amd/__init__.py
--- a/toymeshpathtracer_amd/__init__.py
+++ b/toymeshpathtracer_amd/__init__.py
@@ -157,7 +157,7 @@
            "tmpt_write_png", "tmpt_last_error", "tmpt_abi_version", "tmpt_unit_sincos",
            "tmpt_scene_build_octree", "tmpt_octree_bounds", "tmpt_octree_digest",
            "tmpt_octree_flags", "tmpt_render_aov", "tmpt_render_radiance", "tmpt_denoise", "tmpt_fastdiv",
-           "tmpt_scene_dump_bvh", "tmpt_radix_sort")
+           "tmpt_scene_dump_bvh", "tmpt_radix_sort", "tmpt_camera_rays")
 
 
 def _check(rc: int, what: str) -> None:
@@ -560,6 +560,19 @@
                         img.ctypes.data_as(ctypes.c_void_p)), "denoise")
         return res, img
 
+    def camera_rays(self, camera: Camera, width: int, height: int, spp: int, spp_begin: int = 0,
+                    spp_count: int = 0, band_rows: int = 0, shard: int = 0, num_shards: int = 1) -> np.ndarray:
+        fn = _sig("tmpt_camera_rays", ctypes.c_int, [ctypes.c_void_p, ctypes.c_void_p, ctypes.c_void_p,
+                                                     ctypes.c_void_p])
+        d = _desc(width, height, spp, SEED_SAMPLE, band_rows, shard, num_shards, ENGINE_PERSISTENT, 0,
+                  spp_begin, spp_count)
+        slots = int(_tile_rows(ctypes.byref(d))) * width
+        count = spp_count if spp_count > 0 else spp - spp_begin
+        out = np.zeros((slots, max(count, 0), 8), np.uint32)
+        cam = camera._to_c()
+        _check(fn(self._h, ctypes.byref(cam), ctypes.byref(d), out.ctypes.data_as(ctypes.c_void_p)), "camera_rays")
+        return out
+
     def dump_bvh(self, layout: str = "aos") -> dict:
         if layout not in ("aos", "soa"):
             raise ValueError("dump_bvh: layout is 'aos' or 'soa'")
diff --git a/toymeshpathtracer_amd/csrc/tmpt_api.cpp b/toymeshpathtracer_amd/csrc/tmpt_api.cpp
--- a/toymeshpathtracer_amd/csrc/tmpt_api.cpp
+++ b/toymeshpathtracer_amd/csrc/tmpt_api.cpp
@@ -28,6 +28,7 @@
 int write_png(const char* path, const uint8_t* rgba, int w, int h);
 int render(Scene& s, const tmpt_camera* cam, const tmpt_render_desc* d, uint32_t* d_out,
            uint64_t* ray_count, float4* d_sums = nullptr);
+int camera_rays(Scene& s, const tmpt_camera* cam, const tmpt_render_desc* d, uint32_t* out);
 int intersect_batch(Scene& s, const float* d_rays, int64_t n, float tmin, float tmax, bool any, bool ranged,
                     float* d_hits, int32_t* d_ids);
 
@@ -103,6 +104,8 @@
     {"sample_tail", false, -1, 64, &Options::sample_tail, nullptr, nullptr},
     {"sbuf_max", false, 0, 1e18, nullptr, nullptr, &Options::sbuf_max},
     {"sbuf_pair", false, 0, 1, &Options::sbuf_pair, nullptr, nullptr},
+    {"cam_pre", false, -1, 1, &Options::cam_pre, nullptr, nullptr},
+    {"cam_pre_max", false, 0, 1e18, nullptr, nullptr, &Options::cam_pre_max},
     {"pilot", false, -1, 512, &Options::pilot, nullptr, nullptr},
     {"help", false, -1, 1, &Options::help, nullptr, nullptr},
     {"pair", false, -1, 63, &Options::pair, nullptr, nullptr},
@@ -426,6 +429,7 @@
     if (s.prog) (void)hipFree(s.prog);
     if (s.jt) (void)hipFree(s.jt);
     if (s.sbuf) (void)hipFree(s.sbuf);
+    if (s.cam_rays) (void)hipFree(s.cam_rays);
     if (s.redo) (void)hipFree(s.redo);
     if (s.redo_state) (void)hipFree(s.redo_state);
     if (s.jt2) (void)hipFree(s.jt2);
@@ -598,6 +602,10 @@
     if (!h || !value) return bad("tmpt_scene_get_option: null argument");
     if (key && strcmp(key, "pop_key_bits") == 0) {
         *value = (double)pop_key_bits(h->s.link_bits, h->s.opt.pop_key_cap);
+        return 0;
+    }
+    if (key && strcmp(key, "cam_rays_used") == 0) {
+        *value = (double)h->s.cam_rays_used;
         return 0;
     }
     return options_get(h->s.opt, key, value);
@@ -757,6 +765,24 @@
     }
     if (!dev_out && d_out) (void)hipFree(d_out);
     return rc;
+    TMPT_GUARD_END
+}
+
+int tmpt_camera_rays(tmpt_scene* h, const tmpt_camera* cam, const tmpt_render_desc* d, uint32_t* out)
+{
+    TMPT_GUARD_BEGIN
+    if (!h || !cam || !d || !out) return bad("tmpt_camera_rays: null argument");
+    if (d->width < 1 || d->width > 10000) return bad("tmpt_camera_rays: invalid width");
+    if (d->height < 1 || d->height > 10000) return bad("tmpt_camera_rays: invalid height");
+    if (d->spp < 1 || d->spp > 1024) return bad("tmpt_camera_rays: invalid samplesPerPixel");
+    if (d->num_shards > 1 && (d->shard < 0 || d->shard >= d->num_shards))
+        return bad("tmpt_camera_rays: invalid shard");
+    if (d->spp_begin < 0 || d->spp_begin >= d->spp || d->spp_count < 0 || d->spp_count > d->spp - d->spp_begin)
+        return bad("tmpt_camera_rays: invalid spp_begin / spp_count");
+    (void)hipGetLastError();
+    Scene& s = h->s;
+    TMPT_HIP(hipSetDevice(s.device));
+    return camera_rays(s, cam, d, out);
     TMPT_GUARD_END
 }
 
diff --git a/toymeshpathtracer_amd/csrc/tmpt_internal.h b/toymeshpathtracer_amd/csrc/tmpt_internal.h
--- a/toymeshpathtracer_amd/csrc/tmpt_internal.h
+++ b/toymeshpathtracer_amd/csrc/tmpt_internal.h
@@ -200,6 +200,8 @@
     int sample_tail = -1;
     double sbuf_max = 0.0;
     int sbuf_pair = 1;
+    int cam_pre = -1;
+    double cam_pre_max = 0.0;
     int pilot = -1;
     int help = -1;
     int pair = -1;
@@ -278,6 +280,9 @@
     int32_t jt_spp = 0;
     float4* sbuf = nullptr;
     size_t sbuf_bytes = 0;
+    void* cam_rays = nullptr;
+    size_t cam_bytes = 0;
+    int32_t cam_rays_used = 0;
     uint2* redo = nullptr;
     uint32_t redo_cap = 0;
     float4* redo_state = nullptr;
diff --git a/toymeshpathtracer_amd/csrc/tmpt_path.h b/toymeshpathtracer_amd/csrc/tmpt_path.h
--- a/toymeshpathtracer_amd/csrc/tmpt_path.h
+++ b/toymeshpathtracer_amd/csrc/tmpt_path.h
@@ -38,6 +38,14 @@
     return sample_seed(S.t1, j & 127u, s);
 }
 
+struct alignas(16) CamRay {
+    float ox, oy, oz, dx;
+    float dy, dz;
+    uint32_t rng, flags;
+};
+static_assert(sizeof(CamRay) == 32, "camera entry: two dwordx4 accesses");
+constexpr uint32_t kCamNan = 1u, kCamRootMiss = 2u;
+
 struct PathCtl {
     uint32_t* heads;
     uint32_t nchunks;
@@ -73,6 +81,8 @@
     uint32_t redo_lanes;
     uint32_t oct_shadow;
     uint32_t top_walk;
+    const CamRay* __restrict__ cam_rays;
+    uint32_t cam_count;
 };
 
 struct PathVariant {
@@ -84,6 +94,7 @@
     bool soa;
     int ties;
     bool sums;
+    int cam;
 };
 
 constexpr int kPathSL = 16, kPathSL5 = 12;
diff --git a/toymeshpathtracer_amd/csrc/tmpt_render.hip b/toymeshpathtracer_amd/csrc/tmpt_render.hip
--- a/toymeshpathtracer_amd/csrc/tmpt_render.hip
+++ b/toymeshpathtracer_amd/csrc/tmpt_render.hip
@@ -379,7 +379,7 @@
 
 
 template <bool COUNT, int BLOCK, int SL, int STEPS, int SHADE_MIN, int OCC = 1, int TAIL = 0, int PROF = 0,
-          int HELP = 0, int SAMP = 0, bool SOA = false, int TIES = 0, bool SUMS = false>
+          int HELP = 0, int SAMP = 0, bool SOA = false, int TIES = 0, bool SUMS = false, int CAM = 0>
 __global__ void __launch_bounds__(BLOCK, OCC) k_path(SceneView sv, RenderArgs a, PathCtl pc,
                                                 uint32_t* __restrict__ out,
                                                 uint32_t* __restrict__ ovf,
@@ -387,6 +387,7 @@
 {
     constexpr bool DEFER = TIES == 1, FLAG = TIES != 0;
     static_assert(!SUMS || SAMP == 1, "SUMS: the sample kernel's float sums");
+    static_assert(!CAM || (SAMP == 1 && OCC >= 5 && !COUNT && !SOA && !HELP), "CAM: the 5-wave sample kernels");
     __shared__ uint32_t s_stack[SL * BLOCK];
     __shared__ float s_light[SAMP >= 3 ? 1 : kMaxDepth * BLOCK];
     constexpr bool NEXT3 = OCC >= 5;
@@ -620,7 +621,7 @@
                     } else if (SAMP >= 2) {
                         rng = pc.ustate[cur_unit];
                     } else if (!kFull || a.smp_begin == 0) {
-                        rng = pixel_seed((uint32_t)x, (uint32_t)tile_row_to_y_fd(a, lr), (uint32_t)a.W);
+                        if (!CAM) rng = pixel_seed((uint32_t)x, (uint32_t)tile_row_to_y_fd(a, lr), (uint32_t)a.W);
                         col = mk(0.0f, 0.0f, 0.0f);
                     } else {
                         const float4 pv = a.prog[pix];
@@ -865,7 +866,19 @@
                     pc_cl += (uint64_t)__popcll(cm);
                 }
             }
-            if (cam) {
+            uint32_t cflags = 0;
+            if (CAM && cam) {
+                typedef uint32_t u32x4 __attribute__((ext_vector_type(4)));
+                const u32x4* e = reinterpret_cast<const u32x4*>(
+                    pc.cam_rays + ((size_t)pix * pc.cam_count + (size_t)(smp - (uint32_t)a.smp_begin)));
+                const u32x4 e0 = __builtin_nontemporal_load(e), e1 = __builtin_nontemporal_load(e + 1);
+                so = mk(__uint_as_float(e0.x), __uint_as_float(e0.y), __uint_as_float(e0.z));
+                sd = mk(__uint_as_float(e0.w), __uint_as_float(e1.x), __uint_as_float(e1.y));
+                rng = e1.z;
+                cflags = e1.w;
+                start = true;
+            }
+            if (!CAM && cam) {
                 const int lr = (int)fastdiv(pix, a.div_w);
                 const int x = (int)(pix - (uint32_t)lr * (uint32_t)a.W);
                 const uint32_t y = (uint32_t)tile_row_to_y_fd(a, lr);
@@ -901,7 +914,8 @@
                 qany = sany;
                 if (sany) ++rays_s; else ++rays_e;
                 in_query = sv.n > 0 && !ray_has_nan(so, sd);
-                if (!DEFER && a.root_check && cam && in_query && !octree_root_hit(sv, so, sd, kMinT, kMaxT)) {
+                if (!DEFER && a.root_check && cam && in_query &&
+                    (CAM ? (cflags & kCamRootMiss) != 0u : !octree_root_hit(sv, so, sd, kMinT, kMaxT))) {
                     in_query = false;
                     atomicAdd(&sv.oct->ties[1], 1ull);
                 }
@@ -1154,49 +1168,96 @@
     }
 }
 
+constexpr int kCamBlockSamples = 4;
+__global__ void __launch_bounds__(64 * kCamBlockSamples) k_cam_rays(SceneView sv, RenderArgs a,
+                                                                    CamRay* __restrict__ out, uint32_t count)
+{
+    typedef uint32_t u32x4 __attribute__((ext_vector_type(4)));
+    constexpr uint32_t S = kCamBlockSamples;
+    __shared__ u32x4 s_e[64 * S * 2];
+    const uint32_t l = threadIdx.x & 63u, w = threadIdx.x >> 6;
+    const uint32_t pix0 = blockIdx.x * 64u, rel0 = blockIdx.y * S;
+    const uint32_t pix = min(pix0 + l, (uint32_t)a.slots - 1u);
+    const uint32_t smp = (uint32_t)a.smp_begin + min(rel0 + w, count - 1u);
+    const int lr = (int)fastdiv(pix, a.div_w);
+    const int x = (int)(pix - (uint32_t)lr * (uint32_t)a.W);
+    const uint32_t y = (uint32_t)tile_row_to_y_fd(a, lr);
+    const uint32_t ps = pixel_seed((uint32_t)x, y, (uint32_t)a.W);
+    uint32_t rng = sample_seed(a.jt, smp, ps);
+    f3 so, sd;
+    camera_sample(a.cam, (uint32_t)x, y, a.invW, a.invH, rng, so, sd);
+    uint32_t flags = 0;
+    if (ray_has_nan(so, sd)) flags = kCamNan;
+    else if (a.root_check && !octree_root_hit(sv, so, sd, kMinT, kMaxT)) flags = kCamRootMiss;
+    s_e[(l * S + w) * 2u] = (u32x4){__float_as_uint(so.x), __float_as_uint(so.y), __float_as_uint(so.z),
+                                    __float_as_uint(sd.x)};
+    s_e[(l * S + w) * 2u + 1u] = (u32x4){__float_as_uint(sd.y), __float_as_uint(sd.z), rng, flags};
+    __syncthreads();
+#pragma unroll
+    for (uint32_t h = threadIdx.x; h < 64u * S * 2u; h += 64u * S) {
+        const uint32_t sl = h / (2u * S), r = h % (2u * S);
+        const uint32_t p = pix0 + sl, rel = rel0 + (r >> 1);
+        if (p < (uint32_t)a.slots && rel < count)
+            __builtin_nontemporal_store(s_e[h], reinterpret_cast<u32x4*>(out + ((size_t)p * count + rel)) + (r & 1u));
+    }
+}
+
+static void launch_cam_rays(Scene& s, const RenderArgs& a, CamRay* out)
+{
+    const uint32_t count = (uint32_t)(a.smp_end - a.smp_begin);
+    const dim3 grid((unsigned)((a.slots + 63) / 64), (count + kCamBlockSamples - 1) / kCamBlockSamples);
+    k_cam_rays<<<grid, 64 * kCamBlockSamples, 0, s.stream>>>(view(s), a, out, count);
+}
+
 namespace {
 constexpr bool F = false, T = true;
 constexpr PathVariant kPathVariants[] = {
-    {F, kPathSL, kSampleSteps, kShadeMin, 4, 0, 0, 1, F, 0, F},
-    {F, kPathSL, kSampleSteps, kShadeMin, 4, 0, 0, 1, F, 2, F},
-    {F, kPathSL, kSampleSteps, kShadeMin, 4, 0, 0, 1, F, 1, F},
-    {F, kPathSL, kSampleSteps, kShadeMin, 4, 0, 0, 1, F, 0, T},
-    {F, kPathSL, kSampleSteps, kShadeMin, 4, 0, 0, 1, F, 2, T},
-    {T, kPathSL, kSampleSteps, kShadeMin, 4, 0, 0, 1, F, 0, F},
-    {F, kPathSL, kSampleSteps, kShadeMin, 4, 0, 0, 1, T, 0, F},
-    {F, kPathSL, kSampleSteps, kShadeMin, 4, 0, 0, 1, T, 0, T},
-    {T, kPathSL, kSampleSteps, kShadeMin, 4, 0, 0, 1, T, 0, F},
-    {F, kPathSL5, kSampleSteps, kShadeMin, 5, 0, 0, 1, F, 0, F},
-    {F, kPathSL5, kSampleSteps, kShadeMin, 5, 0, 0, 1, F, 2, F},
-    {F, kPathSL5, kSampleSteps, kShadeMin, 5, 0, 0, 1, F, 1, F},
-    {F, kPathSL5, kSampleSteps, kShadeMin, 5, 0, 0, 1, F, 0, T},
-    {F, kPathSL5, kSampleSteps, kShadeMin, 5, 0, 0, 1, F, 2, T},
-    {F, kPathSL, kPixSteps, kShadeMin, 4, 0, 0, 0, F, 0, F},
-    {F, kPathSL, kPixSteps, kShadeMin, 4, 0, 0, 0, F, 2, F},
-    {F, kPathSL, kPixSteps, kShadeMin, 4, 0, 1, 0, F, 0, F},
-    {F, kPathSL, kPixSteps, kShadeMin, 4, 0, 1, 0, F, 2, F},
-    {T, kPathSL, kPixSteps, kShadeMin, 4, 0, 0, 0, F, 0, F},
-    {F, kPathSL5, kPixSteps, kShadeMin, 5, 0, 0, 0, F, 0, F},
-    {F, kPathSL5, kPixSteps, kShadeMin, 5, 0, 0, 0, F, 2, F},
-    {F, kPathSL5, kPixSteps, kShadeMin, 5, 0, 1, 0, F, 0, F},
-    {F, kPathSL5, kPixSteps, kShadeMin, 5, 0, 1, 0, F, 2, F},
-    {F, kPathSL, kRowIterSteps, kRowIterShadeMin, 4, 0, 0, 2, F, 0, F},
-    {F, kPathSL, kRowIterSteps, kRowIterShadeMin, kRsOcc3, 0, 0, 3, F, 0, F},
-    {F, kPathSL, kRowSteps, kRowShadeMin, 4, 0, 0, 2, F, 0, F},
-    {F, kPathSL, kRowSteps, kRowShadeMin, 4, 0, 0, 2, F, 2, F},
-    {F, kPathSL5, kRowSteps, kRowShadeMin, 5, 0, 0, 2, F, 0, F},
-    {F, kPathSL5, kRowSteps, kRowShadeMin, 5, 0, 0, 2, F, 2, F},
-    {F, kPathSL, kRowSteps, kRowShadeMin, 4, 0, 0, 4, F, 0, F},
-    {F, kPathSL, kRowSteps, kRowShadeMin, 4, 0, 0, 4, F, 2, F},
-    {F, kPathSL, kRowSteps, kRowShadeMin, kRsOcc3, 0, 0, 4, F, 0, F},
-    {F, kPathSL, kRowSteps, kRowShadeMin, kRsOcc3, 0, 0, 4, F, 2, F},
+    {F, kPathSL, kSampleSteps, kShadeMin, 4, 0, 0, 1, F, 0, F, 0},
+    {F, kPathSL, kSampleSteps, kShadeMin, 4, 0, 0, 1, F, 2, F, 0},
+    {F, kPathSL, kSampleSteps, kShadeMin, 4, 0, 0, 1, F, 1, F, 0},
+    {F, kPathSL, kSampleSteps, kShadeMin, 4, 0, 0, 1, F, 0, T, 0},
+    {F, kPathSL, kSampleSteps, kShadeMin, 4, 0, 0, 1, F, 2, T, 0},
+    {T, kPathSL, kSampleSteps, kShadeMin, 4, 0, 0, 1, F, 0, F, 0},
+    {F, kPathSL, kSampleSteps, kShadeMin, 4, 0, 0, 1, T, 0, F, 0},
+    {F, kPathSL, kSampleSteps, kShadeMin, 4, 0, 0, 1, T, 0, T, 0},
+    {T, kPathSL, kSampleSteps, kShadeMin, 4, 0, 0, 1, T, 0, F, 0},
+    {F, kPathSL5, kSampleSteps, kShadeMin, 5, 0, 0, 1, F, 0, F, 0},
+    {F, kPathSL5, kSampleSteps, kShadeMin, 5, 0, 0, 1, F, 2, F, 0},
+    {F, kPathSL5, kSampleSteps, kShadeMin, 5, 0, 0, 1, F, 1, F, 0},
+    {F, kPathSL5, kSampleSteps, kShadeMin, 5, 0, 0, 1, F, 0, T, 0},
+    {F, kPathSL5, kSampleSteps, kShadeMin, 5, 0, 0, 1, F, 2, T, 0},
+    {F, kPathSL5, kSampleSteps, kShadeMin, 5, 0, 0, 1, F, 0, F, 1},
+    {F, kPathSL5, kSampleSteps, kShadeMin, 5, 0, 0, 1, F, 2, F, 1},
+    {F, kPathSL5, kSampleSteps, kShadeMin, 5, 0, 0, 1, F, 1, F, 1},
+    {F, kPathSL5, kSampleSteps, kShadeMin, 5, 0, 0, 1, F, 0, T, 1},
+    {F, kPathSL5, kSampleSteps, kShadeMin, 5, 0, 0, 1, F, 2, T, 1},
+    {F, kPathSL, kPixSteps, kShadeMin, 4, 0, 0, 0, F, 0, F, 0},
+    {F, kPathSL, kPixSteps, kShadeMin, 4, 0, 0, 0, F, 2, F, 0},
+    {F, kPathSL, kPixSteps, kShadeMin, 4, 0, 1, 0, F, 0, F, 0},
+    {F, kPathSL, kPixSteps, kShadeMin, 4, 0, 1, 0, F, 2, F, 0},
+    {T, kPathSL, kPixSteps, kShadeMin, 4, 0, 0, 0, F, 0, F, 0},
+    {F, kPathSL5, kPixSteps, kShadeMin, 5, 0, 0, 0, F, 0, F, 0},
+    {F, kPathSL5, kPixSteps, kShadeMin, 5, 0, 0, 0, F, 2, F, 0},
+    {F, kPathSL5, kPixSteps, kShadeMin, 5, 0, 1, 0, F, 0, F, 0},
+    {F, kPathSL5, kPixSteps, kShadeMin, 5, 0, 1, 0, F, 2, F, 0},
+    {F, kPathSL, kRowIterSteps, kRowIterShadeMin, 4, 0, 0, 2, F, 0, F, 0},
+    {F, kPathSL, kRowIterSteps, kRowIterShadeMin, kRsOcc3, 0, 0, 3, F, 0, F, 0},
+    {F, kPathSL, kRowSteps, kRowShadeMin, 4, 0, 0, 2, F, 0, F, 0},
+    {F, kPathSL, kRowSteps, kRowShadeMin, 4, 0, 0, 2, F, 2, F, 0},
+    {F, kPathSL5, kRowSteps, kRowShadeMin, 5, 0, 0, 2, F, 0, F, 0},
+    {F, kPathSL5, kRowSteps, kRowShadeMin, 5, 0, 0, 2, F, 2, F, 0},
+    {F, kPathSL, kRowSteps, kRowShadeMin, 4, 0, 0, 4, F, 0, F, 0},
+    {F, kPathSL, kRowSteps, kRowShadeMin, 4, 0, 0, 4, F, 2, F, 0},
+    {F, kPathSL, kRowSteps, kRowShadeMin, kRsOcc3, 0, 0, 4, F, 0, F, 0},
+    {F, kPathSL, kRowSteps, kRowShadeMin, kRsOcc3, 0, 0, 4, F, 2, F, 0},
 #ifdef TMPT_DIAG
-    {F, kPathSL, kPixSteps, kShadeMin, 1, 1, 0, 0, F, 0, F},
-    {F, kPathSL, kPixSteps, kShadeMin, 1, 2, 0, 0, F, 0, F},
-    {F, kPathSL, kPixSteps, kShadeMin, 1, 3, 0, 0, F, 0, F},
-    {F, kPathSL, kSampleSteps, kShadeMin, 1, 1, 0, 1, F, 0, F},
-    {F, kPathSL, kSampleSteps, kShadeMin, 1, 2, 0, 1, F, 0, F},
-    {F, kPathSL5, kSampleSteps, kShadeMin, 5, 2, 0, 1, F, 0, F},
+    {F, kPathSL, kPixSteps, kShadeMin, 1, 1, 0, 0, F, 0, F, 0},
+    {F, kPathSL, kPixSteps, kShadeMin, 1, 2, 0, 0, F, 0, F, 0},
+    {F, kPathSL, kPixSteps, kShadeMin, 1, 3, 0, 0, F, 0, F, 0},
+    {F, kPathSL, kSampleSteps, kShadeMin, 1, 1, 0, 1, F, 0, F, 0},
+    {F, kPathSL, kSampleSteps, kShadeMin, 1, 2, 0, 1, F, 0, F, 0},
+    {F, kPathSL5, kSampleSteps, kShadeMin, 5, 2, 0, 1, F, 0, F, 0},
+    {F, kPathSL5, kSampleSteps, kShadeMin, 5, 2, 0, 1, F, 0, F, 1},
 #endif
 };
 constexpr size_t kNumPathVariants = sizeof(kPathVariants) / sizeof(kPathVariants[0]);
@@ -1205,7 +1266,7 @@
 {
     return a.count == b.count && a.sl == b.sl && a.steps == b.steps && a.shade_min == b.shade_min && a.occ == b.occ &&
            a.prof == b.prof && a.help == b.help && a.samp == b.samp && a.soa == b.soa && a.ties == b.ties &&
-           a.sums == b.sums;
+           a.sums == b.sums && a.cam == b.cam;
 }
 
 template <size_t I>
@@ -1213,7 +1274,7 @@
 {
     constexpr PathVariant v = kPathVariants[I];
     return k_path<v.count, kBlk, v.sl, v.steps, v.shade_min, v.occ, path_tail(v.samp), v.prof, v.help, v.samp, v.soa,
-                  v.ties, v.sums>;
+                  v.ties, v.sums, v.cam>;
 }
 
 template <size_t... I>
@@ -1239,7 +1300,8 @@
               std::to_string(v.sl) + ", steps " + std::to_string(v.steps) + ", shade_min " +
               std::to_string(v.shade_min) + ", occ " + std::to_string(v.occ) + ", prof " + std::to_string(v.prof) +
               ", help " + std::to_string(v.help) + ", samp " + std::to_string(v.samp) + ", soa " +
-              std::to_string(v.soa) + ", ties " + std::to_string(v.ties) + ", sums " + std::to_string(v.sums));
+              std::to_string(v.soa) + ", ties " + std::to_string(v.ties) + ", sums " + std::to_string(v.sums) +
+              ", cam " + std::to_string(v.cam));
     return -22;
 }
 
@@ -1470,6 +1532,27 @@
     return 0u;
 }
 
+constexpr int kCamPreDefault = 1;
+
+static bool ensure_cam_rays(Scene& s, size_t need)
+{
+    if (s.opt.cam_pre_max > 0.0 && (double)need > s.opt.cam_pre_max) return false;
+    if (s.cam_bytes >= need) return true;
+    size_t fr = 0, tot = 0;
+    if (hipMemGetInfo(&fr, &tot) != hipSuccess) fr = 0;
+    if (need > (fr + s.cam_bytes) / 2) return false;
+    if (s.cam_rays) (void)hipFree(s.cam_rays);
+    s.cam_rays = nullptr;
+    s.cam_bytes = 0;
+    if (hipMalloc(&s.cam_rays, need) != hipSuccess) {
+        (void)hipGetLastError();
+        s.cam_rays = nullptr;
+        return false;
+    }
+    s.cam_bytes = need;
+    return true;
+}
+
 int render_persistent(Scene& s, const RenderArgs& a, uint32_t* d_out, bool count,
                       unsigned long long* d_counters)
 {
@@ -1488,7 +1571,7 @@
     const bool prof5 = prof == 2 && jt && !soa && o.path_waves != 4;
     const bool waves5 = jt && !count && (!prof || prof5) && !soa && o.path_waves != 4;
     const bool flag = oct && !count && !prof && !soa_kernel;
-    auto variant = [&](bool w5, int help, int ties, bool sums) {
+    auto variant = [&](bool w5, int help, int ties, bool sums, int cam = 0) {
         PathVariant v{};
         v.count = count;
         v.sl = w5 ? kPathSL5 : kPathSL;
@@ -1501,6 +1584,7 @@
         v.soa = soa_kernel;
         v.ties = ties;
         v.sums = sums;
+        v.cam = cam;
         return v;
     };
     PathVariant probe5{};
@@ -1651,7 +1735,18 @@
             set_error("tmpt_render_radiance: no instrumented kernel stores the float sums");
             return -22;
         }
-        PathVariant v_main = variant(w5, help, flag ? (redo ? 1 : 2) : 0, sums);
+        const int cam_pre = o.cam_pre >= 0 ? o.cam_pre : kCamPreDefault;
+        const int64_t cam_n = a.slots * (s1 - s0);
+        const bool cam_on = waves5 && !help && cam_pre != 0 && ensure_cam_rays(s, sizeof(CamRay) * (size_t)cam_n);
+        if (cam_on) {
+            const uint32_t cnt = (uint32_t)(s1 - s0);
+            pc.cam_rays = static_cast<const CamRay*>(s.cam_rays);
+            pc.cam_count = cnt;
+            launch_cam_rays(s, as, static_cast<CamRay*>(s.cam_rays));
+            TMPT_HIP(hipGetLastError());
+            s.cam_rays_used = 1;
+        }
+        PathVariant v_main = variant(w5, help, flag ? (redo ? 1 : 2) : 0, sums, cam_on ? 1 : 0);
         PathFn fn_main;
         if (int rc = find_path_kernel(v_main, "tmpt_render", fn_main)) return rc;
         int grid_main = occupancy_grid((const void*)fn_main, kBlk, 0, s.device);
@@ -1895,6 +1990,34 @@
     s.redo_ms = 0.0;
     s.redo_rays = 0;
     s.tie_path = 0;
+    s.cam_rays_used = 0;
+}
+
+int camera_rays(Scene& s, const tmpt_camera* cam, const tmpt_render_desc* d, uint32_t* out)
+{
+    RenderArgs a = make_args(cam, d);
+    if (int rc = ensure_sample_tables(s, a.spp, "tmpt_camera_rays")) return rc;
+    a.jt = s.jt;
+    a.root_check = camera_root_check(s, a.cam);
+    const uint32_t cnt = (uint32_t)(a.smp_end - a.smp_begin);
+    const int64_t n = a.slots * (int64_t)cnt;
+    if (n <= 0) return 0;
+    CamRay* buf = nullptr;
+    if (hipMalloc(&buf, sizeof(CamRay) * (size_t)n) != hipSuccess) {
+        (void)hipGetLastError();
+        set_error("tmpt_camera_rays: out of device memory");
+        return -12;
+    }
+    launch_cam_rays(s, a, buf);
+    hipError_t e = hipGetLastError();
+    if (e == hipSuccess) e = hipStreamSynchronize(s.stream);
+    if (e == hipSuccess) e = hipMemcpy(out, buf, sizeof(CamRay) * (size_t)n, hipMemcpyDeviceToHost);
+    (void)hipFree(buf);
+    if (e != hipSuccess) {
+        set_error(std::string("tmpt_camera_rays: ") + hipGetErrorString(e));
+        return -1;
+    }
+    return 0;
 }
 
 __global__ void __launch_bounds__(256) k_radiance_scale(float4* __restrict__ px, int64_t n, float spp_recip)
```

After: 11220, median of 6. 1.02x the previous value.
